# haoosz/FFR-Net

Hardware: AMD Instinct MI355X
Metric: face embeddings/sec (IR-SE50 + RecNet forward, 112x112 fp32) at batch 256 per GPU (higher is better)
Workload: dtype f32; 1 GPU; configs[2]: IR-SE50 + RecBlock (spatial+channel) forward, batch 256 per GPU, 112x112x3 fp32 -> f_new,f [512]; + all-gather of embeddings and pair cosine scores (112x96 of the BASELINE label cannot be embedded by the reference: BASELINE.md); batch_per_gpu=256, global_batch=256, parallelism=image-sharded x1, RCCL all-gather of embeddings

## Files before the change

### ffr-net_amd/csrc/conv.cpp

```cpp
#include "engine_internal.h"

namespace ffr_eng {

#ifdef FFR_TRACE
static int trace_igemm(ffr_handle* h, IgemmArgs& a, int tile, int nblocks, long long units, hipStream_t st) {
    unsigned long long* dbuf = nullptr;
    HIPCK(h, hipMalloc((void**)&dbuf, (size_t)nblocks * 8 * sizeof(unsigned long long)));
    a.trace = dbuf;
    HIPCK(h, launch_igemm(a, tile, nblocks, st));
    HIPCK(h, hipStreamSynchronize(st));
    std::vector<unsigned long long> t((size_t)nblocks * 8);
    HIPCK(h, hipMemcpy(t.data(), dbuf, t.size() * 8, hipMemcpyDeviceToHost));
    HIPCK(h, hipFree(dbuf));
    a.trace = nullptr;
    double acc[4] = {0, 0, 0, 0}, segs = 0, e1 = 0, e2 = 0, ghz = 0;
    unsigned long long r0 = ~0ull, r1 = 0, smax = 0;
    for (int b = 0; b < nblocks; ++b) {
        const unsigned long long* q = &t[(size_t)b * 8];
        for (int k = 0; k < 4; ++k) acc[k] += (double)q[k];
        segs += (double)q[4];
        ghz += (double)(q[0] + q[1] + q[2] + q[3]) / ((double)(q[6] - q[5]) * 10.0);
        e1 += (double)(q[7] >> 32); e2 += (double)(q[7] & 0xffffffffull);
        if (q[5] < r0) r0 = q[5];
        if (q[5] > smax) smax = q[5];
        if (q[6] > r1) r1 = q[6];
    }
    fprintf(stderr, "[igemm trace] tile %d blocks %d units %lld nkt %d segs/blk %.2f | per segment: setup %.0f prologue %.0f "
                    "loop %.0f (%.0f per K-tile) epilogue %.0f (first barrier at %.0f, C in LDS at %.0f) cyc | span %.1f us, starts within %.1f us, shader clock %.2f GHz\n",
            tile, nblocks, units, a.nkt, segs / nblocks, acc[0] / segs, acc[1] / segs, acc[2] / segs,
            acc[2] / ((double)units), acc[3] / segs, e1 / segs, e2 / segs, (double)(r1 - r0) / 100.0, (double)(smax - r0) / 100.0, ghz / nblocks);
    return FFR_OK;
}

static int trace_wino_mixed(ffr_handle* h, WinoMixedArgs& f, const ConvW& L, const ConvCall& c, hipStream_t st) {
    const int nbm = wino_mixed_blocks_launched(c.N, c.H, c.W, L.cout_pad, f.xcd_pairs);
    unsigned long long* dbuf = nullptr;
    HIPCK(h, hipMalloc((void**)&dbuf, (size_t)nbm * 12 * sizeof(unsigned long long)));
    HIPCK(h, hipMemsetAsync(dbuf, 0, (size_t)nbm * 12 * sizeof(unsigned long long), st));
    f.trace = dbuf;
    hipEvent_t e0, e1;
    HIPCK(h, hipEventCreate(&e0)); HIPCK(h, hipEventCreate(&e1));
    HIPCK(h, hipEventRecord(e0, st));
    HIPCK(h, launch_wino_fused_mixed(f, st));
    HIPCK(h, hipEventRecord(e1, st));
    HIPCK(h, hipStreamSynchronize(st));
    float ev_ms = 0.f;
    HIPCK(h, hipEventElapsedTime(&ev_ms, e0, e1));
    hipEventDestroy(e0); hipEventDestroy(e1);
    std::vector<unsigned long long> tr((size_t)nbm * 12);
    HIPCK(h, hipMemcpy(tr.data(), dbuf, tr.size() * 8, hipMemcpyDeviceToHost));
    HIPCK(h, hipFree(dbuf));
    double pro[4] = {0, 0, 0, 0}, loop[4] = {0, 0, 0, 0}, ep1[4] = {0, 0, 0, 0}, ep2[4] = {0, 0, 0, 0}, clk[4] = {0, 0, 0, 0};
    int cnt[4] = {0, 0, 0, 0};
    unsigned long long r_first = ~0ull, r_last = 0;
    struct Run { unsigned long long start, end; int tau; };
    std::map<unsigned long long, std::vector<Run>> per_cu;
    for (int b = 0; b < nbm; ++b) {
        const unsigned long long* q = &tr[(size_t)b * 12];
        if (!q[9]) continue;
        const int tau = (int)q[8];
        pro[tau] += (double)(q[1] - q[0]); loop[tau] += (double)(q[2] - q[1]); ep1[tau] += (double)(q[3] - q[2]); ep2[tau] += (double)(q[4] - q[3]);
        clk[tau] += (double)(q[4] - q[0]) / (double)(q[6] - q[5]) * 0.1;
        ++cnt[tau];
        if (q[5] < r_first) r_first = q[5];
        if (q[6] > r_last) r_last = q[6];
        per_cu[q[7]].push_back(Run{q[5], q[6], tau});
    }
    static const char* tname[4] = {"(4,4)", "(4,3)", "(3,4)", "(3,3)"};
    fprintf(stderr, "[wf trace] mixed %dx%d cin %d cout %d, %d images: hipEvent %.1f us, first block start to last block end %.1f us\n",
            c.H, c.W, L.cin_pad, L.cout_pad, c.N, ev_ms * 1e3, (double)(r_last - r_first) / 100.0);
    for (int tau = 0; tau < 4; ++tau) {
        if (!cnt[tau]) continue;
        const int S = wino_mixed_xp(tau) / 4;
        fprintf(stderr, "[wf trace]   type %s: %d blocks of %d slots | per block (wave 0): prologue %.0f loop %.0f (%.0f per K chunk, floor %d) "
                        "epilogue %.0f + %.0f = block %.0f cyc at %.2f GHz = %.1f us\n", tname[tau], cnt[tau], S, pro[tau] / cnt[tau], loop[tau] / cnt[tau],
                loop[tau] / cnt[tau] / f.nkc, S * 8 * 64, ep1[tau] / cnt[tau], ep2[tau] / cnt[tau],
                (pro[tau] + loop[tau] + ep1[tau] + ep2[tau]) / cnt[tau], clk[tau] / cnt[tau],
                (pro[tau] + loop[tau] + ep1[tau] + ep2[tau]) / cnt[tau] / (clk[tau] / cnt[tau]) * 1e-3);
    }
    std::map<std::string, int> hist;
    double busy = 0, gap = 0, tail = 0, lead = 0;
    for (auto& kv : per_cu) {
        auto& v = kv.second;
        std::sort(v.begin(), v.end(), [](const Run& x, const Run& y) { return x.start < y.start; });
        std::string key;
        for (size_t i = 0; i < v.size(); ++i) {
            key += tname[v[i].tau];
            busy += (double)(v[i].end - v[i].start);
            if (i) gap += (double)(v[i].start - v[i - 1].end);
        }
        lead += (double)(v.front().start - r_first);
        tail += (double)(r_last - v.back().end);
        ++hist[key];
    }
    const double ncu = (double)per_cu.size();
    fprintf(stderr, "[wf trace]   %d CUs ran blocks; per CU: busy %.1f us, idle before its first block %.1f, between blocks %.1f, after its last block %.1f us | sequences:",
            (int)per_cu.size(), busy / ncu / 100.0, lead / ncu / 100.0, gap / ncu / 100.0, tail / ncu / 100.0);
    for (auto& kv : hist) fprintf(stderr, "  %s x %d", kv.first.c_str(), kv.second);
    fprintf(stderr, "\n");
    return FFR_OK;
}

static int trace_wino_fused(ffr_handle* h, WinoFusedArgs& f, const ConvW& L, const ConvCall& c, const ConvPlan& p, hipStream_t st) {
    const int nb = wino_fused_blocks(f);
    unsigned long long* dbuf = nullptr;
    HIPCK(h, hipMalloc((void**)&dbuf, (size_t)nb * 40 * sizeof(unsigned long long)));
    HIPCK(h, hipMemsetAsync(dbuf, 0, (size_t)nb * 40 * sizeof(unsigned long long), st));
    f.trace = dbuf;
    HIPCK(h, launch_wino_fused(f, st));
    HIPCK(h, hipStreamSynchronize(st));
    std::vector<unsigned long long> tr((size_t)nb * 40);
    HIPCK(h, hipMemcpy(tr.data(), dbuf, tr.size() * 8, hipMemcpyDeviceToHost));
    HIPCK(h, hipFree(dbuf));
    double pro = 0, loop = 0, epi = 0, ep[5] = {0, 0, 0, 0, 0}; int cnt = 0;
    unsigned long long r0 = ~0ull, r1 = 0;
    for (int b = 0; b < nb; ++b) {
        const unsigned long long* q = &tr[(size_t)b * 40];
        if (!q[3]) continue;
        ep[0] += (double)(q[6] - q[2]); ep[1] += (double)(q[7] - q[6]); ep[2] += (double)(q[8] - q[7]);
        ep[3] += (double)(q[9] - q[8]); ep[4] += (double)(q[3] - q[9]);
        pro += (double)(q[1] - q[0]); loop += (double)(q[2] - q[1]); epi += (double)(q[3] - q[2]); ++cnt;
        if (q[4] > r1) r1 = q[4];
        if (q[4] < r0) r0 = q[4];
    }
    if (p.phased) {
        const int cpp = 4, nph = f.nkc / cpp;
        fprintf(stderr, "[wf trace] %dx%d cin %d cout %d (input transform in the kernel, %d-channel blocks%s): %d live blocks of %d | per block (wave 0): "
                        "prologue %.0f loop %.0f = %d phases x (transform %.0f + barrier %.0f + %d K chunks of %.0f) epilogue %.0f cyc | "
                        "block ends spread over %.1f us\n", c.H, c.W, L.cin_pad, L.cout_pad, p.half_n ? 32 : 64, "", cnt, nb,
                pro / cnt, loop / cnt, nph, ep[0] / cnt, ep[1] / cnt, cpp, (loop / cnt / nph - ep[0] / cnt - ep[1] / cnt) / cpp, epi / cnt,
                (double)(r1 - r0) / 100.0);
    }
    else
        fprintf(stderr, "[wf trace] %dx%d cin %d cout %d: %d live blocks of %d | per block (wave 0): prologue %.0f loop %.0f (%.0f per K chunk) "
                        "epilogue %.0f cyc (to LDS %.0f, transform+store %.0f, barrier+to LDS %.0f, transform+store %.0f, end %.0f) | block ends spread over %.1f us\n",
                c.H, c.W, L.cin_pad, L.cout_pad, cnt, nb, pro / cnt, loop / cnt, loop / cnt / f.nkc, epi / cnt, ep[0] / cnt, ep[1] / cnt,
                ep[2] / cnt, ep[3] / cnt, ep[4] / cnt, (double)(r1 - r0) / 100.0);
    return FFR_OK;
}
#endif

int run_gemm(ffr_handle* h, IgemmArgs& a, const ConvCall& c, double flops, double bytes, hipStream_t st, double fuse) {
    int tile, nblocks;
    int force = c.tile;
    if (force) {
        int fbm, fbn;
        igemm_tile_shape(force, &fbm, &fbn);
        if (a.cout_pad % fbn) return fail(h, FFR_ERR_ARG, "conv: forced tile %d (%d x %d) does not divide cout_pad %d", force, fbm, fbn, a.cout_pad);
    }
    plan_igemm(a.M, a.cout_pad, a.nkt, a.nbatch, force, h->opt.sk_minunits, &tile, &nblocks, &a.granule, a.w3 != nullptr);
    int bm, bn;
    igemm_tile_shape(tile, &bm, &bn);
    a.mtiles = (a.M + bm - 1) / bm;
    a.ntiles = a.cout_pad / bn;
    const long long units = (long long)a.nbatch * a.mtiles * a.ntiles * a.nkt;
    const bool cut = a.granule == 1 && ((units % nblocks) != 0 || ((units / nblocks) % a.nkt) != 0);
    if (cut && (size_t)nblocks * 2 * bm * bn > c.partial_cap) return fail(h, FFR_ERR_NOMEM, "stream-K workspace too small");
    a.partial = c.partial;
    a.tickets = c.tickets;
    if ((size_t)a.nbatch * a.mtiles * a.ntiles > c.tickets_cap) return fail(h, FFR_ERR_NOMEM, "stream-K ticket array too small");
#ifdef FFR_TRACE
    if (h->opt.igemm_trace) return trace_igemm(h, a, tile, nblocks, units, st);
#endif
    const double fexec = 2.0 * a.nbatch * (double)a.mtiles * bm * (double)a.cout_pad * a.KK;
    Scope s(h, st, FFR_KC_CONV_IGEMM, flops, bytes, fexec, fuse);
    HIPCK(h, launch_igemm(a, tile, nblocks, st));
    return FFR_OK;
}

static int conv_mixed(ffr_handle* h, const ConvW& L, const ConvCall& c, double flops, double bytes, hipStream_t st) {
    WinoMixedGeom g;
    wino_mixed_geom(c.H, c.W, &g);
    if (c.wino_stage == 0) {
        Scope s(h, st, FFR_KC_WINO, 0, 4.0 * ((double)c.N * c.H * c.W * L.cin + (double)wino_mixed_v_floats(g, c.N, L.cin_pad, nullptr)));
        HIPCK(h, launch_wino_in_mixed(c.x, c.winoV, c.N, c.H, c.W, c.in_pitch, L.cin_pad, st));
    }
    WinoMixedArgs f{};
    f.V[0] = c.winoV;
    for (int tau = 0; tau < 4; ++tau) f.U[tau] = L.wum[tau];
    f.bias = L.bias; f.slope = L.slope; f.resid = c.resid; f.out = c.out; f.tile_sums = c.tile_sums;
    f.N = c.N; f.H = c.H; f.W = c.W; f.nkc = L.cin_pad / 8;
    f.cout_pad = L.cout_pad; f.cout_store = c.cout_store; f.out_pitch = c.out_pitch; f.out_coff = c.out_coff;
    f.res_pitch = c.res_pitch; f.border_bias = L.border; f.flags = c.flags;
    f.xcd_pairs = 1;
    double fexec = 0.0, fuse = 0.0;
    for (int tau = 0; tau < 4; ++tau) {
        const int nr = tau >= 2 ? g.n3 : g.n4, nc = (tau & 1) ? g.n3 : g.n4;
        const double Tt = (double)c.N * nr * nc;
        fexec += 2.0 * wino_mixed_xp(tau) * std::ceil(Tt / 32.0) * 32.0 * L.cout_pad * L.cin_pad;
        fuse += 2.0 * wino_mixed_x(tau) * Tt * L.cout * L.cin;
    }
#ifdef FFR_TRACE
    if (h->opt.wf_trace) return trace_wino_mixed(h, f, L, c, st);
#endif
    Scope s(h, st, FFR_KC_WINO_FUSED, flops, bytes, fexec, fuse);
    HIPCK(h, launch_wino_fused_mixed(f, st));
    return FFR_OK;
}

static int conv_fused(ffr_handle* h, const ConvW& L, const ConvCall& c, const ConvPlan& p, double flops, double bytes, hipStream_t st) {
    const long long T = (long long)c.N * ((c.H + 3) / 4) * ((c.W + 3) / 4);
    if (!p.phased && c.wino_stage == 0) {
        Scope s(h, st, FFR_KC_WINO, 0, 4.0 * ((double)c.N * c.H * c.W * L.cin + 36.0 * T * L.cin_pad));
        HIPCK(h, launch_wino_in_chunked(c.x, c.winoV, c.N, c.H, c.W, c.in_pitch, L.cin_pad, L.pad_mode, st));
    }
    WinoFusedArgs f{};
    f.Vc = p.phased ? nullptr : c.winoV; f.x = c.x; f.in_pitch = c.in_pitch; f.pad_mode = L.pad_mode;
    f.x_bytes = p.phased ? (unsigned)(4.0 * c.N * c.H * c.W * c.in_pitch) : 0u;
    f.map_v = p.phased ? 2 : 1; f.half_n = p.half_n ? 1 : 0;
    f.Uc = L.wuc; f.bias = L.bias; f.slope = L.slope; f.resid = c.resid; f.out = c.out; f.tile_sums = c.tile_sums;
    f.N = c.N; f.H = c.H; f.W = c.W; f.nkc = L.cin_pad / 8;
    f.cout_pad = L.cout_pad; f.cout_store = c.cout_store; f.out_pitch = c.out_pitch; f.out_coff = c.out_coff;
    f.res_pitch = c.res_pitch; f.border_bias = L.border; f.flags = c.flags;
    const double fexec = 2.0 * 36.0 * (double)((T + 31) / 32 * 32) * (double)L.cout_pad * L.cin_pad;
#ifdef FFR_TRACE
    if (h->opt.wf_trace) return trace_wino_fused(h, f, L, c, p, st);
#endif
    Scope s(h, st, FFR_KC_WINO_FUSED, flops, bytes, fexec, flops / 4.0);
    HIPCK(h, launch_wino_fused(f, st));
    return FFR_OK;
}

static int igemm_batched(ffr_handle* h, const ConvCall& c, const float* A, long long a_bstride, int K_pad, const float* W,
                         long long w_bstride, int N_pad, float* out, int out_pitch, long long out_bstride, int M, int nbatch,
                         double flops, double bytes, double fuse, hipStream_t st) {
    IgemmArgs g{};
    g.x = A; g.w = W; g.bias = h->zero; g.slope = nullptr; g.resid = nullptr; g.out = out; g.zero = h->zero;
    g.N = 1; g.H = 1; g.W = M; g.Ho = 1; g.Wo = M;
    g.in_pitch = K_pad; g.cin_pad = K_pad; g.R = 1; g.S = 1; g.stride = 1; g.pad = 0; g.pad_mode = 0;
    g.M = M; g.KK = K_pad; g.nkt = K_pad / 32;
    g.cout_pad = N_pad; g.cout_store = N_pad; g.out_pitch = out_pitch; g.out_coff = 0; g.res_pitch = 0;
    g.border_bias = 0; g.flags = 0;
    g.nbatch = nbatch; g.x_bstride = a_bstride; g.w_bstride = w_bstride; g.out_bstride = out_bstride;
    return run_gemm(h, g, c, flops, bytes, st, fuse);
}

static int conv_unfused(ffr_handle* h, const ConvW& L, const ConvCall& c, long long M, double flops, double bytes, hipStream_t st) {
    const long long T = (long long)c.N * ((c.H + 3) / 4) * ((c.W + 3) / 4);
    if (c.wino_stage != 2) {
        Scope s(h, st, FFR_KC_WINO, 0, 4.0 * ((double)c.N * c.H * c.W * L.cin + 36.0 * T * L.cin_pad));
        HIPCK(h, launch_wino_in(c.x, c.winoV, c.N, c.H, c.W, c.in_pitch, L.cin_pad, L.pad_mode, st));
    }
    if (h->opt.gemm_stream) {
        int gtile = IGEMM_TILE_128x64, gblocks = 768;
        double best = 1e300;
        for (int tt = IGEMM_TILE_128x128; tt <= IGEMM_TILE_128x64; ++tt) {
            int bm, bn;
            igemm_tile_shape(tt, &bm, &bn);
            if (L.cout_pad % bn) continue;
            const long long tiles = 36LL * ((T + bm - 1) / bm) * (L.cout_pad / bn);
            const long long pmax = 256LL * igemm_resident_blocks(tt);
            const long long p = pmax > tiles ? tiles : pmax;
            const double rounds = (double)((tiles + p - 1) / p);
            const double share = (double)((p + 255) / 256);
            const double cost = rounds * bm * bn * share / (tt == IGEMM_TILE_128x128 ? 1.0 : 0.92);
            if (cost < best) { best = cost; gtile = tt; gblocks = (int)p; }
        }
        GemmStreamArgs g{};
        g.A = c.winoV; g.W = L.wu; g.C = c.winoM; g.M = (int)T; g.K = L.cin_pad; g.Npad = L.cout_pad; g.nbatch = 36;
        int bm, bn;
        igemm_tile_shape(gtile, &bm, &bn);
        const double fexec = 2.0 * 36.0 * (double)((T + bm - 1) / bm) * bm * (double)L.cout_pad * L.cin_pad;
        Scope s(h, st, FFR_KC_CONV_IGEMM, flops, bytes, fexec, flops / 4.0);
        HIPCK(h, launch_gemm_stream(g, gtile, gblocks, st));
    } else {
        RC(igemm_batched(h, c, c.winoV, T * L.cin_pad, L.cin_pad, L.wu, (long long)L.cout_pad * L.cin_pad, L.cout_pad, c.winoM, L.cout_pad,
                         T * L.cout_pad, (int)T, 36, flops, bytes, flops / 4.0, st));
    }
    if (c.wino_stage == 1) return FFR_OK;
    Scope s(h, st, FFR_KC_WINO, 0, 4.0 * (36.0 * T * L.cout_pad + (double)M * L.cout));
    HIPCK(h, launch_wino_out(c.winoM, L.bias, L.slope, c.resid, c.res_pitch, c.out, c.out_pitch, c.out_coff,
                             c.cout_store, L.cout_pad, c.N, c.H, c.W, L.border, c.flags, st, c.tile_sums));
    return FFR_OK;
}

int run_conv(ffr_handle* h, const ConvW& L, const ConvCall& c, hipStream_t st) {
    const int Ho = (c.H + 2 * L.pad - L.R) / L.stride + 1, Wo = (c.W + 2 * L.pad - L.S) / L.stride + 1;
    const long long M = (long long)c.N * Ho * Wo;
    if (M <= 0 || M > 0x7fffffffLL) return fail(h, FFR_ERR_ARG, "conv: bad M");
    if (L.pad_mode == 1 && (c.H < 2 || c.W < 2)) return fail(h, FFR_ERR_UNSUPPORTED, "reflect pad needs H,W >= 2");
    if (L.border && (c.H < 2 || c.W < 2)) return fail(h, FFR_ERR_UNSUPPORTED, "border-class bias needs H,W >= 2");
    const double flops = 2.0 * M * L.cout * (double)L.R * L.S * L.cin;
    const double bytes = 4.0 * ((double)c.N * c.H * c.W * L.cin + (double)M * L.cout + (double)L.cout * L.R * L.S * L.cin);
    const ConvPlan p = plan_conv(h, L, c);
    if (p.refused) return fail(h, FFR_ERR_STATE, "%s", p.refused);
    if (p.path == ConvPlan::Mixed) return conv_mixed(h, L, c, flops, bytes, st);
    if (p.path == ConvPlan::Unfused) return conv_unfused(h, L, c, M, flops, bytes, st);
    if (p.path == ConvPlan::Fused && !p.n_main) return conv_fused(h, L, c, p, flops, bytes, st);
    if (p.path == ConvPlan::Fused) {
        ConvCall c1 = c, c2 = c;
        c1.N = p.n_main; c1.force = p.half_n ? ConvForce::FusedHalf : ConvForce::Fused;
        c2.N = c.N - p.n_main; c2.force = ConvForce::Unfused;
        const size_t px = (size_t)p.n_main * c.H * c.W;
        c2.x = c.x + px * c.in_pitch;
        c2.out = c.out + px * c.out_pitch;
        if (c.resid) c2.resid = c.resid + px * c.res_pitch;
        if (c.tile_sums) c2.tile_sums = c.tile_sums + (size_t)p.n_main * ((c.H + 3) / 4) * ((c.W + 3) / 4) * L.cout_pad;
        if (p.side) {
            HIPCK(h, hipEventRecord(h->ev_fork, st));
            HIPCK(h, hipStreamWaitEvent(p.side, h->ev_fork, 0));
            RC(run_conv(h, L, c2, p.side));
            HIPCK(h, hipEventRecord(h->ev_join, p.side));
            RC(run_conv(h, L, c1, st));
            HIPCK(h, hipStreamWaitEvent(st, h->ev_join, 0));
            return FFR_OK;
        }
        RC(run_conv(h, L, c1, st));
        return run_conv(h, L, c2, st);
    }
    IgemmArgs a{};
    a.x = c.x; a.w = L.w; a.bias = L.bias; a.slope = L.slope; a.resid = c.resid; a.out = c.out; a.zero = h->zero;
    a.N = c.N; a.H = c.H; a.W = c.W; a.Ho = Ho; a.Wo = Wo;
    a.in_pitch = c.in_pitch; a.cin_pad = L.cin_pad; a.R = L.R; a.S = L.S; a.stride = L.stride; a.pad = L.pad; a.pad_mode = L.pad_mode;
    a.M = (int)M; a.KK = L.R * L.S * L.cin_pad; a.nkt = a.KK / 32; a.nbatch = 1;
    a.cout_pad = L.cout_pad; a.cout_store = c.cout_store; a.out_pitch = c.out_pitch; a.out_coff = c.out_coff;
    a.res_pitch = c.res_pitch; a.border_bias = L.border; a.flags = c.flags;
    if (L.w3 && h->opt.igemm_split) { a.w3 = L.w3; a.w3_pstride = (long long)L.cout_pad * a.KK; }
    return run_gemm(h, a, c, flops, bytes, st);
}

int gemm_rows(ffr_handle* h, const Work& w, const float* A, int a_pitch, int K_pad, const float* W, const float* bias,
              int N_pad, float* out, int out_pitch, long long rows, const float* resid, int res_pitch, int flags,
              hipStream_t st) {
    ConvW cw;
    cw.cin = K_pad; cw.cin_pad = K_pad; cw.cout = N_pad; cw.cout_pad = N_pad; cw.R = 1; cw.S = 1; cw.stride = 1; cw.pad = 0;
    cw.pad_mode = 0; cw.border = 0; cw.w = const_cast<float*>(W); cw.bias = bias ? const_cast<float*>(bias) : h->zero;
    cw.slope = nullptr; cw.wu = nullptr;
    ConvCall c = conv_call(w, ConvForce::Direct);
    c.x = A; c.N = 1; c.H = 1; c.W = (int)rows; c.in_pitch = a_pitch; c.resid = resid; c.res_pitch = res_pitch;
    c.out = out; c.out_pitch = out_pitch; c.out_coff = 0; c.cout_store = N_pad; c.flags = flags;
    return run_conv(h, cw, c, st);
}

int gemm_batched(ffr_handle* h, const Work& w, const float* A, long long a_bstride, int K_pad, const float* W,
                 long long w_bstride, int N_pad, float* out, int out_pitch, long long out_bstride, int M, int nbatch,
                 hipStream_t st) {
    const double fl = 2.0 * nbatch * (double)M * N_pad * K_pad;
    return igemm_batched(h, conv_call(w, ConvForce::Direct), A, a_bstride, K_pad, W, w_bstride, N_pad, out, out_pitch, out_bstride, M,
                         nbatch, fl, 4.0 * nbatch * ((double)M * K_pad + (double)N_pad * K_pad + (double)M * N_pad), fl, st);
}

}
```

### ffr-net_amd/csrc/engine.cpp

```cpp
#include "engine_internal.h"

using namespace ffr;
using namespace ffr_eng;

namespace ffr_eng {

std::string g_err = "";

int fail(ffr_handle* h, int code, const char* fmt, ...) {
    char buf[512];
    va_list ap;
    va_start(ap, fmt);
    vsnprintf(buf, sizeof buf, fmt, ap);
    va_end(ap);
    if (h) h->err = buf; else g_err = buf;
    return code;
}

struct PlanLayer { ConvW* L; std::string name; int net; };

std::vector<PlanLayer> plan_layers(const ffr_handle* hc) {
    ffr_handle* h = const_cast<ffr_handle*>(hc);
    std::vector<PlanLayer> v;
    if (h->enc_loaded)
        for (size_t i = 0; i < h->blocks.size(); ++i) {
            Block& b = h->blocks[i];
            const std::string p = "body." + std::to_string(i) + ".res_layer.";
            if (b.c1.wu) v.push_back({&b.c1, p + "1", 0});
            if (b.c2.wu) v.push_back({&b.c2, p + "3", 0});
        }
    if (h->rec_loaded)
        for (int i = 0; i < 15; ++i)
            if (rec_conv(h, i).wu) v.push_back({&rec_conv(h, i), std::string(REC_LAYERS[i].prefix) + ".conv2d", 1});
    return v;
}

void plan_changed(ffr_handle* h) { ++h->generation; h->mixed_ready_n = 0; }
}

extern "C" {

const char* ffr_version(void) { return "ffrnet-hip 0.1 (gfx950)"; }

const char* ffr_last_error(const ffr_handle* h) { return h ? h->err.c_str() : g_err.c_str(); }

int ffr_create(ffr_handle** out, int device) {
    if (!out) return fail(nullptr, FFR_ERR_ARG, "ffr_create: out is null");
    *out = nullptr;
    int count = 0;
    if (hipGetDeviceCount(&count) != hipSuccess || count <= 0)
        return fail(nullptr, FFR_ERR_HIP, "no HIP device available (this library has no CPU fallback)");
    if (device < 0 || device >= count) return fail(nullptr, FFR_ERR_ARG, "device %d out of range (%d devices)", device, count);
    DeviceScope scope(device);
    if (!scope.ok) return fail(nullptr, FFR_ERR_HIP, "hipSetDevice(%d) failed", device);
    hipDeviceProp_t prop;
    if (hipGetDeviceProperties(&prop, device) != hipSuccess) return fail(nullptr, FFR_ERR_HIP, "hipGetDeviceProperties failed");
    if (strncmp(prop.gcnArchName, "gfx950", 6) != 0)
        return fail(nullptr, FFR_ERR_UNSUPPORTED, "device %d is %s; this library is built for gfx950 (MI355X) only", device,
                    prop.gcnArchName);
    ffr_handle* h = new ffr_handle();
    h->device = device;
    h->num_cus = prop.multiProcessorCount > 0 ? prop.multiProcessorCount : 256;
    void* z = nullptr;
    if (hipMalloc(&z, 131072) != hipSuccess) { delete h; return fail(nullptr, FFR_ERR_NOMEM, "hipMalloc failed"); }
    hipMemset(z, 0, 131072);
    h->zero = (float*)z;
    hipError_t e = igemm_init();
    if (e == hipSuccess) e = gemm_stream_init();
    if (e == hipSuccess) e = wino_fused_init();
    if (e == hipSuccess) e = wino_mixed_init();
    if (e == hipSuccess) e = hipStreamCreateWithFlags(&h->side, hipStreamNonBlocking);
    if (e == hipSuccess) e = hipEventCreateWithFlags(&h->ev_fork, hipEventDisableTiming);
    if (e == hipSuccess) e = hipEventCreateWithFlags(&h->ev_join, hipEventDisableTiming);
    if (e != hipSuccess) {
        if (h->ev_fork) hipEventDestroy(h->ev_fork);
        if (h->ev_join) hipEventDestroy(h->ev_join);
        if (h->side) hipStreamDestroy(h->side);
        hipFree(z); delete h;
        return fail(nullptr, FFR_ERR_HIP, "ffr_create: %s", hipGetErrorString(e));
    }
    *out = h;
    return FFR_OK;
}

void ffr_destroy(ffr_handle* h) {
    if (!h) return;
    FFR_DEVICE_SCOPE(h);
    hipDeviceSynchronize();
    train_free(h);
    free_list(h->enc_allocs);
    free_list(h->rec_allocs);
    if (h->ev_fork) hipEventDestroy(h->ev_fork);
    if (h->ev_join) hipEventDestroy(h->ev_join);
    if (h->side) hipStreamDestroy(h->side);
    if (h->arena) hipFree(h->arena);
    if (h->tickets) hipFree(h->tickets);
    if (h->search_buf) hipFree(h->search_buf);
    if (h->align_buf) hipFree(h->align_buf);
    if (h->zero) hipFree(h->zero);
    for (auto& r : h->prof_log) { hipEventDestroy(r.e0); hipEventDestroy(r.e1); }
    for (auto e : h->ev_pool) hipEventDestroy(e);
    delete h;
}

int ffr_memory_stats(const ffr_handle* h, ffr_mem_stats* out) {
    if (!h || !out) return fail(nullptr, FFR_ERR_ARG, "ffr_memory_stats: null argument");
    out->encoder_weight_bytes = h->enc_weight_bytes;
    out->recnet_weight_bytes = h->rec_weight_bytes;
    out->mixed_tile_weight_bytes = h->mixed_weight_bytes;
    out->workspace_bytes = h->arena_bytes;
    out->encoder_load_seconds = h->enc_load_s;
    out->recnet_load_seconds = h->rec_load_s;
    out->mixed_tile_pack_seconds = h->mixed_pack_s;
    out->split_weight_bytes = h->split_weight_bytes;
    return FFR_OK;
}

size_t ffr_workspace_bytes(const ffr_handle* h, int N, int H, int W) {
    if (N <= 0 || H <= 0 || W <= 0) return 0;
    return layout(h ? h->opt : Options(), nullptr, N, H, W).total;
}

int ffr_reserve(ffr_handle* h, int N, int H, int W) {
    FFR_DEVICE_SCOPE(h); RC(check_fwd(h, false, false, N));
    Work w;
    return ensure_arena_encoder(h, N, H, W, &w);
}

static int encoder_forward(ffr_handle* h, const float* x, const U8In* u8, int N, int H, int W, float* featmap_nchw, float* f,
                           void* stream) {
    FFR_DEVICE_SCOPE(h); RC(check_fwd(h, true, false, N));
    if (u8 ? !u8->img : !x) return fail(h, FFR_ERR_ARG, u8 ? "img is null" : "x is null");
    if (H < 32 || W < 32 || (H & 15) || (W & 15)) return fail(h, FFR_ERR_ARG, "H and W must be multiples of 16, >= 32");
    if (f && (H != 112 || W != 112)) return fail(h, FFR_ERR_UNSUPPORTED, "f needs a 112x112 input (Linear(512*7*7,512))");
    hipStream_t st = (hipStream_t)stream;
    Work w;
    RC(ensure_arena_encoder(h, N, H, W, &w));
    RC(run_encoder(h, w, x, N, H, W, featmap_nchw ? w.trunk_bn : nullptr, f, st, u8));
    if (featmap_nchw) {
        Scope s(h, st, FFR_KC_LAYOUT, 0, 8.0 * N * (H / 16) * (W / 16) * 512);
        HIPCK(h, launch_nhwc_to_nchw(w.trunk_bn, 512, featmap_nchw, N, (H / 16) * (W / 16), 512, st));
    }
    return FFR_OK;
}

int ffr_encoder_forward(ffr_handle* h, const float* x, int N, int H, int W, float* featmap_nchw, float* f, void* stream) {
    return encoder_forward(h, x, nullptr, N, H, W, featmap_nchw, f, stream);
}

int ffr_encoder_forward_u8(ffr_handle* h, const uint8_t* img_hwc_rgb, const uint8_t* flip, int N, int H, int W,
                           float* featmap_nchw, float* f, void* stream) {
    const U8In u8{img_hwc_rgb, flip};
    return encoder_forward(h, nullptr, &u8, N, H, W, featmap_nchw, f, stream);
}

int ffr_recnet_forward(ffr_handle* h, const float* featmap_nchw, int N, float* f_new, float* feat_new_nchw, void* stream) {
    FFR_DEVICE_SCOPE(h); RC(check_fwd(h, false, true, N));
    if (!featmap_nchw) return fail(h, FFR_ERR_ARG, "featmap is null");
    hipStream_t st = (hipStream_t)stream;
    Work w;
    RC(ensure_arena(h, N, 112, 112, &w));
    {
        Scope s(h, st, FFR_KC_LAYOUT, 0, 8.0 * N * 49 * 512);
        HIPCK(h, launch_nchw_to_nhwc(featmap_nchw, w.X, 512, N, 49, 512, st));
    }
    RC(run_recnet(h, w, N, f_new, nullptr, st));
    if (feat_new_nchw) {
        Scope s(h, st, FFR_KC_LAYOUT, 0, 8.0 * N * 49 * 512);
        HIPCK(h, launch_nhwc_to_nchw(w.m512c, 512, feat_new_nchw, N, 49, 512, st));
    }
    return FFR_OK;
}

int ffr_embed(ffr_handle* h, const float* x, int N, float* f_new, float* f, void* stream) {
    FFR_DEVICE_SCOPE(h); RC(check_fwd(h, true, true, N));
    if (!x || !f_new) return fail(h, FFR_ERR_ARG, "x / f_new is null");
    hipStream_t st = (hipStream_t)stream;
    Work w;
    RC(ensure_arena_encoder(h, N, 112, 112, &w));
    RC(run_encoder(h, w, x, N, 112, 112, w.X, f, st));
    return run_recnet(h, w, N, f_new, nullptr, st);
}

int ffr_embed_u8(ffr_handle* h, const uint8_t* img_hwc_rgb, const uint8_t* flip, int N, float* f_new, float* f,
                 void* stream) {
    FFR_DEVICE_SCOPE(h); RC(check_fwd(h, true, true, N));
    if (!img_hwc_rgb || !f_new) return fail(h, FFR_ERR_ARG, "img / f_new is null");
    hipStream_t st = (hipStream_t)stream;
    Work w;
    RC(ensure_arena_encoder(h, N, 112, 112, &w));
    U8In u8{img_hwc_rgb, flip};
    RC(run_encoder(h, w, nullptr, N, 112, 112, w.X, f, st, &u8));
    return run_recnet(h, w, N, f_new, nullptr, st);
}

int ffr_cosine_scores(ffr_handle* h, const float* a, const float* b, int n, int dim, float* score, void* stream) {
    FFR_DEVICE_SCOPE(h); RC(check_fwd(h, false, false, n));
    if (!a || !b || !score || dim <= 0) return fail(h, FFR_ERR_ARG, "ffr_cosine_scores: bad arguments");
    hipStream_t st = (hipStream_t)stream;
    Scope s(h, st, FFR_KC_SCORE, 6.0 * n * dim, 8.0 * n * dim);
    HIPCK(h, launch_cosine(a, b, n, dim, score, st));
    return FFR_OK;
}

int ffr_lfw_fold_accuracy(ffr_handle* h, const float* score, const int32_t* label, int n, int n_folds, double* best_thr,
                          double* test_acc, void* stream) {
    FFR_DEVICE_SCOPE(h); RC(check_fwd(h, false, false, n));
    if (!score || !label || !best_thr || !test_acc || n_folds < 1 || n_folds > 32 || n < n_folds)
        return fail(h, FFR_ERR_ARG, "ffr_lfw_fold_accuracy: bad arguments");
    hipStream_t st = (hipStream_t)stream;
    Work w;
    RC(ensure_arena(h, 8, 112, 112, &w));
    Scope s(h, st, FFR_KC_SCORE, 400.0 * n, 8.0 * 400 * n);
    HIPCK(h, launch_fold_protocol(score, (const int*)label, n, n_folds, (int*)w.partial, best_thr, test_acc, st));
    return FFR_OK;
}

unsigned long long ffr_generation(const ffr_handle* h) { return h ? h->generation : 0; }

static bool misaligned16(const void* p) { return ((uintptr_t)p & 15) != 0; }

int ffr_row_norms(ffr_handle* h, const float* x, long long n, int dim, float* norms, void* stream) {
    FFR_DEVICE_SCOPE(h); RC(check_fwd(h, false, false, 1));
    if (dim != 512) return fail(h, FFR_ERR_UNSUPPORTED, "ffr_row_norms: dim must be 512, got %d", dim);
    if (!x || !norms || n < 1) return fail(h, FFR_ERR_ARG, "ffr_row_norms: bad arguments");
    hipStream_t st = (hipStream_t)stream;
    Scope s(h, st, FFR_KC_SCORE, 2.0 * n * dim, 4.0 * n * (dim + 1));
    HIPCK(h, launch_row_norms(x, n, norms, st));
    return FFR_OK;
}

int ffr_search_topk(ffr_handle* h, const float* query, int Q, const float* gallery, const float* gallery_norms, long long G,
                    int dim, int k, long long index_base, float* top_score, int64_t* top_index, void* stream) {
    FFR_DEVICE_SCOPE(h); RC(check_fwd(h, false, false, 1));
    if (dim != 512) return fail(h, FFR_ERR_UNSUPPORTED, "ffr_search_topk: dim must be 512, got %d", dim);
    if (!query || !top_score || !top_index || Q < 1 || k < 1 || k > 128 || G < 0 || (G > 0 && (!gallery || !gallery_norms)))
        return fail(h, FFR_ERR_ARG, "ffr_search_topk: bad arguments (Q >= 1, 1 <= k <= 128, G >= 0, non-null pointers)");
    if (misaligned16(query) || (G > 0 && misaligned16(gallery)))
        return fail(h, FFR_ERR_ARG, "ffr_search_topk: query and gallery rows must be 16-byte aligned");
    hipStream_t st = (hipStream_t)stream;
    if (G == 0) {
        Scope s(h, st, FFR_KC_SCORE, 0.0, 12.0 * Q * k);
        HIPCK(h, launch_topk_merge(nullptr, nullptr, 0, Q, k, top_score, top_index, st));
        return FFR_OK;
    }
    int T = 0, S = 0;
    long long chunk_rows = 0;
    search_plan(Q, G, h->num_cus, &T, &S, &chunk_rows);
    const size_t norm_bytes = ((size_t)Q * 4 + 255) & ~(size_t)255;
    const size_t list_s = S > 1 ? (((size_t)S * Q * k * 4 + 255) & ~(size_t)255) : 0;
    const size_t need = norm_bytes + list_s + (S > 1 ? (size_t)S * Q * k * 8 : 0);
    if (need > h->search_bytes) {
        if (h->search_buf) { hipDeviceSynchronize(); hipFree(h->search_buf); h->search_buf = nullptr; h->search_bytes = 0; }
        void* p = nullptr;
        if (hipMalloc(&p, need) != hipSuccess) return fail(h, FFR_ERR_NOMEM, "hipMalloc of %zu search bytes failed", need);
        h->search_buf = (char*)p;
        h->search_bytes = need;
        ++h->generation;
    }
    float* qnorm = (float*)h->search_buf;
    float* part_s = S > 1 ? (float*)(h->search_buf + norm_bytes) : top_score;
    int64_t* part_i = S > 1 ? (int64_t*)(h->search_buf + norm_bytes + list_s) : top_index;
    Scope s(h, st, FFR_KC_SCORE, 2.0 * Q * (double)G * dim, 4.0 * (double)G * (dim + 1) + 4.0 * Q * dim + 12.0 * Q * k);
    HIPCK(h, launch_row_norms(query, Q, qnorm, st));
    HIPCK(h, launch_search_topk(query, qnorm, Q, gallery, gallery_norms, G, k, index_base, T, S, chunk_rows, part_s, part_i,
                                st));
    if (S > 1) HIPCK(h, launch_topk_merge(part_s, part_i, S, Q, k, top_score, top_index, st));
// ... 108 lines not shown
    out->arith = v[i].L->direct ? FFR_ARITH_DIRECT : FFR_ARITH_WINOGRAD;
    out->sensitivity = v[i].L->sensitivity;
    return FFR_OK;
}

int ffr_layer_set_arith(ffr_handle* h, int i, int arith) {
    if (!h) return fail(nullptr, FFR_ERR_ARG, "null handle");
    if (arith != FFR_ARITH_DIRECT && arith != FFR_ARITH_WINOGRAD) return fail(h, FFR_ERR_ARG, "ffr_layer_set_arith: arith %d is neither 0 (direct) nor 1 (Winograd)", arith);
    const std::vector<PlanLayer> v = plan_layers(h);
    if (i < 0 || i >= (int)v.size()) return fail(h, FFR_ERR_ARG, "ffr_layer_set_arith: index %d outside [0, %d)", i, (int)v.size());
    const bool direct = arith == FFR_ARITH_DIRECT;
    if (v[i].L->direct != direct) { v[i].L->direct = direct; plan_changed(h); }
    return FFR_OK;
}

int ffr_calibrate(ffr_handle* h, const float* x, const float* featmap, int N, int H, int W, double tol, double* achieved,
                  void* stream) {
    if (!h) return fail(nullptr, FFR_ERR_ARG, "null handle");
    hipStream_t st = (hipStream_t)stream;
    {
        FFR_DEVICE_SCOPE(h);
        hipStreamCaptureStatus cs = hipStreamCaptureStatusNone;
        HIPCK(h, hipStreamIsCapturing(st, &cs));
        if (cs != hipStreamCaptureStatusNone) return fail(h, FFR_ERR_ARG, "ffr_calibrate: the stream is capturing (the call synchronises)");
    }
    if (!(tol > 0.0)) return fail(h, FFR_ERR_ARG, "ffr_calibrate: tol must be > 0 (got %g)", tol);
    if ((x != nullptr) == (featmap != nullptr)) return fail(h, FFR_ERR_ARG, "ffr_calibrate: pass images (x) or a featmap, exactly one of them");
    const bool enc = x != nullptr;
    FFR_DEVICE_SCOPE(h); RC(check_fwd(h, enc, !enc, N));
    if (enc && (H < 32 || W < 32 || (H & 15) || (W & 15))) return fail(h, FFR_ERR_ARG, "H and W must be multiples of 16, >= 32");
    if (!enc && (H != 7 || W != 7)) return fail(h, FFR_ERR_ARG, "ffr_calibrate: a featmap is [N,512,7,7] (H = W = 7)");
    const bool is112 = enc && H == 112 && W == 112;
    const bool rec = !enc || (h->rec_loaded && is112);
    const int P = enc ? (H / 16) * (W / 16) : 49;

    std::vector<ConvW*> cand;
    for (const PlanLayer& pl : plan_layers(h))
        if ((pl.net == 0 && enc) || (pl.net == 1 && rec)) cand.push_back(pl.L);
    const int L = (int)cand.size();
    struct Saved {
        ffr_handle* h; std::vector<std::pair<ConvW*, bool>> plan; bool prof; void* buf = nullptr; bool keep = false;
        ~Saved() {
            if (buf) { hipDeviceSynchronize(); hipFree(buf); }
            h->prof = prof;
            if (!keep) for (auto& p : plan) p.first->direct = p.second;
        }
    } sv{h, {}, h->prof};
    for (ConvW* c : cand) sv.plan.push_back({c, c->direct});
    h->prof = false;

    for (ConvW* c : cand) c->direct = false;
    h->mixed_ready_n = 0;
    Work w;
    if (enc) RC(ensure_arena_encoder(h, N, H, W, &w));
    else RC(ensure_arena(h, N, 112, 112, &w));

    const bool have[4] = {is112, enc, rec, rec};
    const size_t rows[4] = {(size_t)N, (size_t)N * P, (size_t)N, (size_t)N * 49};
    float* featmap_nhwc = rec ? w.X : w.trunk_bn;
    const int max_trials = 2 * L + 4;
    const size_t scratch = (size_t)absdiff_scratch_floats();
    size_t floats = scratch + (size_t)max_trials * 4 * 2 + 2 * (size_t)N * 512;
    size_t off_anchor[4];
    for (int t = 0; t < 4; ++t) { off_anchor[t] = floats; floats += have[t] ? rows[t] * 512 : 0; }
    HIPCK(h, hipMalloc(&sv.buf, floats * sizeof(float)));
    float* base = (float*)sv.buf;
    float* part = base;
    float* table = base + scratch;
    float* f_cur = table + (size_t)max_trials * 8;
    float* fnew_cur = f_cur + (size_t)N * 512;
    const float* cur[4] = {f_cur, featmap_nhwc, fnew_cur, w.m512c};
    float* anchor[4];
    for (int t = 0; t < 4; ++t) anchor[t] = base + off_anchor[t];
    HIPCK(h, hipMemsetAsync(table, 0, (size_t)max_trials * 8 * sizeof(float), st));

    auto forward = [&]() -> int {
        if (enc) {
            RC(run_encoder(h, w, x, N, H, W, featmap_nhwc, is112 ? f_cur : nullptr, st));
        } else {
            HIPCK(h, launch_nchw_to_nhwc(featmap, w.X, 512, N, 49, 512, st));
        }
        if (rec) RC(run_recnet(h, w, N, fnew_cur, nullptr, st));
        return FFR_OK;
    };
    auto compare = [&](int slot) -> int {
        for (int t = 0; t < 4; ++t)
            if (have[t]) HIPCK(h, launch_absdiff_max(cur[t], 512, anchor[t], 512, (int)rows[t], 512, part, table + ((size_t)slot * 4 + t) * 2, st));
        return FFR_OK;
    };
    std::vector<float> host((size_t)max_trials * 8);
    auto read = [&]() -> int {
        HIPCK(h, hipMemcpyAsync(host.data(), table, host.size() * sizeof(float), hipMemcpyDeviceToHost, st));
        HIPCK(h, hipStreamSynchronize(st));
        return FFR_OK;
    };
    auto rel = [&](int slot, int t) { const float* q = &host[((size_t)slot * 4 + t) * 2]; return q[1] > 0.f ? (double)q[0] / q[1] : (double)q[0]; };
    auto err = [&](int slot) { double e = 0.0; for (int t = 0; t < 4; ++t) if (have[t]) e = std::max(e, rel(slot, t)); return e; };
    auto set_plan = [&](const std::vector<char>& wino) { for (int k = 0; k < L; ++k) cand[k]->direct = !wino[k]; };

    set_plan(std::vector<char>(L, 0));
    RC(forward());
    for (int t = 0; t < 4; ++t)
        if (have[t]) HIPCK(h, hipMemcpyAsync(anchor[t], cur[t], rows[t] * 512 * sizeof(float), hipMemcpyDeviceToDevice, st));
    set_plan(std::vector<char>(L, 1));
    RC(forward()); RC(compare(0));
    for (int k = 0; k < L; ++k) {
        std::vector<char> one(L, 0);
        one[k] = 1;
        set_plan(one);
        RC(forward()); RC(compare(1 + k));
    }
    RC(read());
    const double half = 0.5 * tol;
    for (int k = 0; k < L; ++k) cand[k]->sensitivity = err(1 + k);
    std::vector<int> order(L);
    for (int k = 0; k < L; ++k) order[k] = k;
    std::stable_sort(order.begin(), order.end(), [&](int a, int b) { return cand[a]->sensitivity < cand[b]->sensitivity; });
    auto prefix_plan = [&](int p) { std::vector<char> v(L, 0); for (int i = 0; i < p; ++i) v[order[i]] = 1; return v; };

    std::vector<int> passing;
    if (err(0) <= half) passing.push_back(L);
    else if (L > 1) {
        for (int p = 1; p < L; ++p) { set_plan(prefix_plan(p)); RC(forward()); RC(compare(p)); }
        RC(read());
        int pmax = 0;
        while (pmax + 1 < L && err(pmax + 1) <= half) ++pmax;
        for (int p = pmax; p >= 1; --p) passing.push_back(p);
    }
    passing.push_back(0);

    for (int p : passing) {
        set_plan(prefix_plan(p));
        RC(forward()); RC(compare(0));
        RC(read());
        if (err(0) <= half || p == 0) break;
    }
    if (achieved) for (int t = 0; t < 4; ++t) achieved[t] = have[t] ? rel(0, t) : -1.0;
    sv.keep = true;
    bool changed = false;
    for (auto& pr : sv.plan) changed |= pr.first->direct != pr.second;
    if (changed) plan_changed(h);
    else h->mixed_ready_n = 0;
    return FFR_OK;
}

namespace {
struct OptEntry { const char* name; int ffr_eng::Options::*i; long long ffr_eng::Options::*l; long long lo, hi; };
const OptEntry OPTIONS[] = {
    {"wino", &Options::wino, nullptr, 0, 1}, {"wino_mincin", &Options::wino_mincin, nullptr, 0, 1 << 20},
    {"wino_fused", &Options::wino_fused, nullptr, 0, 1},
    {"wf_phased_maxk", &Options::wf_phased_maxk, nullptr, 0, 1 << 20}, {"wf_minblocks", nullptr, &Options::wf_minblocks, 0, 1LL << 40},
    {"se_maxtiles", &Options::se_maxtiles, nullptr, 0, 1 << 20}, {"wf_tailsplit", &Options::wf_tailsplit, nullptr, 0, 1},
    {"gemm_stream", &Options::gemm_stream, nullptr, 0, 1}, {"sk_minunits", &Options::sk_minunits, nullptr, 1, 1 << 20},
    {"combine_v", &Options::combine_v, nullptr, 0, 1}, {"wf_mixed", &Options::wf_mixed, nullptr, 0, 1},
    {"channel_rows", &Options::channel_rows, nullptr, 0, 4}, {"igemm_split", &Options::igemm_split, nullptr, 0, 1},
    {"wf_trace", &Options::wf_trace, nullptr, 0, 1}, {"igemm_trace", &Options::igemm_trace, nullptr, 0, 1},
};
const OptEntry* find_option(const char* name) {
    if (name) for (const OptEntry& e : OPTIONS) if (!strcmp(e.name, name)) return &e;
    return nullptr;
}
}

int ffr_set_option(ffr_handle* h, const char* name, long long value) {
    if (!h) return fail(nullptr, FFR_ERR_ARG, "null handle");
    const OptEntry* e = find_option(name);
    if (!e) return fail(h, FFR_ERR_ARG, "ffr_set_option: unknown option '%s'", name ? name : "(null)");
    if (value < e->lo || value > e->hi) return fail(h, FFR_ERR_ARG, "ffr_set_option: %s = %lld is outside [%lld, %lld]", name, value, e->lo, e->hi);
    if (e->i == &Options::channel_rows && value == 3) return fail(h, FFR_ERR_ARG, "ffr_set_option: channel_rows is 0 (auto), 1, 2 or 4");
#ifndef FFR_TRACE
    if ((e->i == &Options::wf_trace || e->i == &Options::igemm_trace) && value)
        return fail(h, FFR_ERR_UNSUPPORTED, "ffr_set_option: %s needs a -DFFR_TRACE build of the library (tools/trace_build.py)", name);
#endif
    const long long old = e->i ? (long long)(h->opt.*(e->i)) : h->opt.*(e->l);
    if (old != value) ++h->generation;
    if (e->i) h->opt.*(e->i) = (int)value; else h->opt.*(e->l) = value;
    return FFR_OK;
}

int ffr_get_option(const ffr_handle* h, const char* name, long long* value) {
    if (!h || !value) return fail(nullptr, FFR_ERR_ARG, "ffr_get_option: bad arguments");
    const OptEntry* e = find_option(name);
    if (!e) return fail(const_cast<ffr_handle*>(h), FFR_ERR_ARG, "ffr_get_option: unknown option '%s'", name ? name : "(null)");
    *value = e->i ? (long long)(h->opt.*(e->i)) : h->opt.*(e->l);
    return FFR_OK;
}

int ffr_probe_mfma_peak(ffr_handle* h, int iters, double* tflops, double* clock_ghz, void* stream) {
    FFR_DEVICE_SCOPE(h); RC(check_fwd(h, false, false, 1));
    if (iters <= 0 || !tflops) return fail(h, FFR_ERR_ARG, "ffr_probe_mfma_peak: bad arguments");
    hipStream_t st = (hipStream_t)stream;
    const int blocks = h->num_cus * 2;
    struct Res {
        unsigned long long* stamps = nullptr; float* sink = nullptr; hipEvent_t e0 = nullptr, e1 = nullptr;
        ~Res() { if (e0) hipEventDestroy(e0); if (e1) hipEventDestroy(e1); if (stamps) hipFree(stamps); if (sink) hipFree(sink); }
    } r;
    HIPCK(h, hipMalloc((void**)&r.stamps, (size_t)blocks * 4 * sizeof(unsigned long long)));
    HIPCK(h, hipMalloc((void**)&r.sink, (size_t)blocks * 256 * sizeof(float)));
    HIPCK(h, hipEventCreate(&r.e0)); HIPCK(h, hipEventCreate(&r.e1));
    for (int rep = 0; rep < 3; ++rep) HIPCK(h, launch_mfma_probe(iters, blocks, r.stamps, r.sink, st));
    HIPCK(h, hipEventRecord(r.e0, st));
    HIPCK(h, launch_mfma_probe(iters, blocks, r.stamps, r.sink, st));
    HIPCK(h, hipEventRecord(r.e1, st));
    HIPCK(h, hipEventSynchronize(r.e1));
    float ms = 0.f;
    HIPCK(h, hipEventElapsedTime(&ms, r.e0, r.e1));
    std::vector<unsigned long long> sv((size_t)blocks * 4);
    HIPCK(h, hipMemcpy(sv.data(), r.stamps, sv.size() * 8, hipMemcpyDeviceToHost));
    double ghz = 0;
    for (int b = 0; b < blocks; ++b) ghz += (double)(sv[b * 4 + 1] - sv[b * 4 + 0]) / ((double)(sv[b * 4 + 3] - sv[b * 4 + 2]) * 10.0);
    *tflops = (double)blocks * 4.0 * iters * 16.0 * 4096.0 / ((double)ms * 1e-3) / 1e12;
    if (clock_ghz) *clock_ghz = ghz / blocks;
    return FFR_OK;
}

int ffr_profile_enable(ffr_handle* h, int on) {
    if (!h) return fail(nullptr, FFR_ERR_ARG, "null handle");
    h->prof = on != 0;
    return FFR_OK;
}

int ffr_profile_read(ffr_handle* h, ffr_kclass_stat* out) {
    if (!h || !out) return fail(h, FFR_ERR_ARG, "ffr_profile_read: bad arguments");
    for (int i = 0; i < FFR_KC_COUNT; ++i) out[i] = ffr_kclass_stat{0, 0.0, 0.0, 0.0, 0.0, 0.0};
    for (auto& r : h->prof_log) {
        HIPCK(h, hipEventSynchronize(r.e1));
        float ms = 0.f;
        HIPCK(h, hipEventElapsedTime(&ms, r.e0, r.e1));
        out[r.kc].launches += 1;
        if (!r.side) {
            out[r.kc].ms += ms;
            out[r.kc].flops += r.flops;
            out[r.kc].bytes += r.bytes;
            out[r.kc].flops_executed += r.fexec;
            out[r.kc].flops_useful += r.fuse;
        }
        h->ev_pool.push_back(r.e0);
        h->ev_pool.push_back(r.e1);
    }
    h->prof_log.clear();
    return FFR_OK;
}

int ffr_op_conv(ffr_handle* h, const ffr_conv_desc* d, void* stream) {
    if (!d) return fail(h, FFR_ERR_ARG, "desc is null");
    FFR_DEVICE_SCOPE(h); RC(check_fwd(h, false, false, d->N));
    if (!d->x || !d->w || !d->bias || !d->out) return fail(h, FFR_ERR_ARG, "ffr_op_conv: null tensor");
    if (d->cin_pad % 32 || d->cout_pad % 64 || d->cin_pad <= 0) return fail(h, FFR_ERR_ARG, "ffr_op_conv: bad padding");
    Work w;
    RC(ensure_arena(h, d->N > 8 ? d->N : 8, 112, 112, &w));
    ConvW L;
    L.cin = L.cin_pad = d->cin_pad; L.cout = d->cout_store; L.cout_pad = d->cout_pad; L.R = d->R; L.S = d->S;
    L.stride = d->stride; L.pad = d->pad; L.pad_mode = d->pad_mode; L.border = d->border_bias;
    L.w = (float*)d->w; L.bias = (float*)d->bias; L.slope = (float*)d->slope;
    struct Planes { void* p = nullptr; ~Planes() { if (p) hipFree(p); } } planes;
    if (d->flags & 2) {
        if (!h->opt.igemm_split) return fail(h, FFR_ERR_STATE, "ffr_op_conv: flags bit1 asks for the split form, but option igemm_split is 0");
        const size_t nw = (size_t)d->cout_pad * d->R * d->S * d->cin_pad;
        HIPCK(h, hipMalloc(&planes.p, nw * 3 * sizeof(unsigned short)));
        HIPCK(h, launch_split_weights(d->w, (unsigned short*)planes.p, nw, (hipStream_t)stream));
        L.w3 = (unsigned short*)planes.p;
    }
    ConvCall c = conv_call(w);
    c.x = d->x; c.N = d->N; c.H = d->H; c.W = d->W; c.in_pitch = d->in_pitch; c.resid = d->resid; c.res_pitch = d->res_pitch;
    c.out = d->out; c.out_pitch = d->out_pitch; c.out_coff = d->out_coff; c.cout_store = d->cout_store; c.flags = d->flags & 1;
    c.tile = d->tile;
    const int rc = run_conv(h, L, c, (hipStream_t)stream);
    if (planes.p) hipStreamSynchronize((hipStream_t)stream);
    return rc;
}

int ffr_op_conv3x3(ffr_handle* h, const float* x, int N, int H, int W, int cin, const float* w_host,
                   const float* bias_host, const float* slope_host, int cout, int pad_mode, int use_wino,
                   const float* resid, float* out, void* stream) {
    FFR_DEVICE_SCOPE(h); RC(check_fwd(h, false, false, N));
    if (!x || !w_host || !bias_host || !out || cin % 32 || cout % 4 || cin <= 0 || cout <= 0)
        return fail(h, FFR_ERR_ARG, "ffr_op_conv3x3: bad arguments (cin %% 32, cout %% 4)");
    if (use_wino < 0 || use_wino > 4) return fail(h, FFR_ERR_ARG, "ffr_op_conv3x3: use_wino must be 0..4");
    hipStream_t st = (hipStream_t)stream;
    Work w;
    RC(ensure_arena(h, N > 8 ? N : 8, 112, 112, &w));
    std::vector<void*> own;
    BNFold ob;
    ob.s.assign(cout, 1.0);
    ob.t.assign(bias_host, bias_host + cout);
    ConvW L;
    int rc = pack_conv(h, own, w_host, cout, cin, 3, 3, nullptr, &ob, slope_host, 1, 1, pad_mode, &L);
    if (rc == FFR_OK && use_wino && !L.wu) rc = fail(h, FFR_ERR_UNSUPPORTED, "layer not eligible for the Winograd path (cin < FFR_WINO_MINCIN)");
    if (rc == FFR_OK && use_wino == 4) {
        if (!wino_mixed_eligible(h, L, N, H, W, cin, w.wino_cap, ConvForce::Mixed)) rc = fail(h, FFR_ERR_UNSUPPORTED, "layer / map not eligible for the mixed-tile path");
        else rc = ensure_mixed_weights(h, L, own, true);
    }
    if (rc == FFR_OK) {
        ConvCall c = conv_call(w, (ConvForce)use_wino);
        c.x = x; c.N = N; c.H = H; c.W = W; c.in_pitch = cin; c.resid = resid; c.res_pitch = cout;
        c.out = out; c.out_pitch = cout; c.out_coff = 0; c.cout_store = cout;
        rc = run_conv(h, L, c, st);
        if (rc == FFR_OK && use_wino && (size_t)36 * N * ((H + 3) / 4) * ((W + 3) / 4) * (L.cin_pad > L.cout_pad ? L.cin_pad : L.cout_pad) > w.wino_cap)
            rc = fail(h, FFR_ERR_NOMEM, "Winograd scratch too small for this test shape");
    }
    hipStreamSynchronize(st);
    free_list(own);
    return rc;
}

int ffr_encoder_trunk_nhwc(ffr_handle* h, const float* x, int N, int H, int W, int n_blocks, float* out, void* stream) {
    FFR_DEVICE_SCOPE(h); RC(check_fwd(h, true, false, N));
    if (!x || !out || n_blocks < 0 || n_blocks > (int)h->blocks.size()) return fail(h, FFR_ERR_ARG, "ffr_encoder_trunk_nhwc: bad arguments");
    if (H < 32 || W < 32 || (H & 15) || (W & 15)) return fail(h, FFR_ERR_ARG, "H and W must be multiples of 16, >= 32");
    hipStream_t st = (hipStream_t)stream;
    Work w;
    RC(ensure_arena_encoder(h, N, H, W, &w));
    float* t; int oh, ow, oc;
    RC(run_trunk(h, w, x, N, H, W, n_blocks, st, &t, &oh, &ow, &oc));
    HIPCK(h, hipMemcpyAsync(out, t, (size_t)N * oh * ow * oc * sizeof(float), hipMemcpyDeviceToDevice, st));
    return FFR_OK;
}

int ffr_recnet_debug(ffr_handle* h, const float* featmap_nchw, int N, float* ss_space, float* M_space, float* feat_space,
                     float* feat_channel_raw, float* feat_channel, float* ss_channel0, float* M_channel0, void* stream) {
    FFR_DEVICE_SCOPE(h); RC(check_fwd(h, false, true, N));
    if (!featmap_nchw) return fail(h, FFR_ERR_ARG, "featmap is null");
    hipStream_t st = (hipStream_t)stream;
    Work w;
    RC(ensure_arena(h, N, 112, 112, &w));
    HIPCK(h, launch_nchw_to_nhwc(featmap_nchw, w.X, 512, N, 49, 512, st));
    RecDebug d{ss_space, M_space, feat_space, feat_channel_raw, feat_channel, ss_channel0, M_channel0};
    return run_recnet(h, w, N, nullptr, &d, st);
}

}
```

### ffr-net_amd/csrc/engine_internal.h

```cpp
#pragma once
#include <hip/hip_runtime.h>

#include <algorithm>
#include <chrono>
#include <cmath>
#include <cstdarg>
#include <cstdio>
#include <cstdlib>
#include <cstring>
#include <initializer_list>
#include <map>
#include <string>
#include <vector>

#include "../../include/ffrnet.h"
#include "../../include/ffrnet_train.h"
#include "ffr_kernels.h"

namespace ffr_eng {

using namespace ffr;

struct TrainState;

struct ConvW {
    int cin = 0, cin_pad = 0, cout = 0, cout_pad = 0, R = 1, S = 1, stride = 1, pad = 0, pad_mode = 0, border = 0;
    float* w = nullptr;
    float* bias = nullptr;
    float* slope = nullptr;
    float* wu = nullptr;
    float* wum[4] = {nullptr, nullptr, nullptr, nullptr};
    bool wum_gave_up = false;
    unsigned short* w3 = nullptr;
    float* wuc = nullptr;
    bool direct = false;
    double sensitivity = -1.0;
};

struct Block {
    int cin = 0, depth = 0, stride = 1;
    bool has_sc = false;
    ConvW c1, c2, sc;
    float* fc1 = nullptr;
    float* fc2 = nullptr;
};

struct Options {
    int wino = 1;
    int wino_mincin = 64;
    int wino_fused = 1;
    int wf_phased_maxk = 128;
    long long wf_minblocks = 200;
    int se_maxtiles = 256;
    int wf_tailsplit = 1;
    int gemm_stream = 1;
    int sk_minunits = 18;
    int wf_mixed = 1;
    int channel_rows = 0;
    int igemm_split = 1;
    int combine_v = 1;
    int wf_trace = 0, igemm_trace = 0;
};

struct ProfRec {
    hipEvent_t e0, e1;
    int kc;
    double flops, bytes, fexec, fuse;
    bool side;
};

}

struct ffr_handle {
    int device = 0;
    int num_cus = 256;
    hipStream_t side = nullptr;
    hipEvent_t ev_fork = nullptr, ev_join = nullptr;
    std::string err;
    float* zero = nullptr;
    std::vector<void*> enc_allocs, rec_allocs;
    bool enc_loaded = false, rec_loaded = false;
    size_t enc_weight_bytes = 0, rec_weight_bytes = 0;
    size_t mixed_weight_bytes = 0;
    double enc_load_s = 0.0, rec_load_s = 0.0, mixed_pack_s = 0.0;
    size_t split_weight_bytes = 0;
    bool mixed_gave_up_logged = false, split_gave_up_logged = false;
    int mixed_ready_n = 0, mixed_ready_h = 0, mixed_ready_w = 0;
    float *stem_w = nullptr, *stem_b = nullptr, *stem_s = nullptr;
    std::vector<ffr_eng::Block> blocks;
    float *bn_s = nullptr, *bn_t = nullptr;
    ffr_eng::ConvW fc;
    ffr_eng::ConvW sp[9], fm[3], mg[3];
    ffr::ChannelPathWeights cw{};
    char* arena = nullptr;
    size_t arena_bytes = 0;
    int* tickets = nullptr;
    size_t tickets_cap = 0;
    ffr_eng::Options opt;
    bool prof = false;
    std::vector<ffr_eng::ProfRec> prof_log;
    std::vector<hipEvent_t> ev_pool;
    ffr_eng::TrainState* train = nullptr;
    std::vector<ffr_wgrad_launch> wgrad_log;
    char* search_buf = nullptr;
    size_t search_bytes = 0;
    char* align_buf = nullptr;
    size_t align_bytes = 0;
    unsigned long long generation = 1;
};

namespace ffr_eng {

int fail(ffr_handle* h, int code, const char* fmt, ...);

#define HIPCK(h, expr)                                                                          \
    do {                                                                                        \
        hipError_t _e = (expr);                                                                 \
        if (_e != hipSuccess)                                                                   \
            return fail(h, FFR_ERR_HIP, "%s failed: %s (%s:%d)", #expr, hipGetErrorString(_e), __FILE__, __LINE__); \
    } while (0)

#define RC(expr)                  \
    do {                          \
        int _rc = (expr);         \
        if (_rc != FFR_OK) return _rc; \
    } while (0)

inline int round_up(int v, int m) { return (v + m - 1) / m * m; }

struct DeviceScope {
    int prev = -1;
    bool switched = false, ok = true;
    explicit DeviceScope(int dev) {
        if (dev < 0) return;
        if (hipGetDevice(&prev) != hipSuccess) prev = -1;
        if (prev != dev) { ok = hipSetDevice(dev) == hipSuccess; switched = ok && prev >= 0; }
    }
    ~DeviceScope() { if (switched) hipSetDevice(prev); }
};
#define FFR_DEVICE_SCOPE(h) ffr_eng::DeviceScope _dev_scope((h) ? (h)->device : -1)

struct Scope {
    ffr_handle* h;
    hipStream_t st;
    ProfRec r;
    bool on;
    Scope(ffr_handle* h_, hipStream_t st_, int kc, double flops, double bytes, double fexec = -1.0, double fuse = -1.0)
        : h(h_), st(st_), on(h_->prof) {
        if (!on) return;
        auto get = [&]() {
            hipEvent_t e;
            if (!h->ev_pool.empty()) { e = h->ev_pool.back(); h->ev_pool.pop_back(); }
            else hipEventCreate(&e);
            return e;
        };
        r.e0 = get(); r.e1 = get(); r.kc = kc; r.flops = flops; r.bytes = bytes; r.fexec = fexec < 0 ? flops : fexec; r.fuse = fuse < 0 ? flops : fuse;
        r.side = h->side && st == h->side;
        hipEventRecord(r.e0, st);
    }
    ~Scope() {
        if (!on) return;
        hipEventRecord(r.e1, st);
        h->prof_log.push_back(r);
    }
};

struct SD {
    std::map<std::string, const ffr_tensor_desc*> m;
    ffr_handle* h;
    int rc = FFR_OK;
    const float* get(const std::string& name, std::initializer_list<int64_t> shape) {
        auto it = m.find(name);
        if (it == m.end()) { rc = fail(h, FFR_ERR_KEY, "state_dict entry '%s' is missing", name.c_str()); return nullptr; }
        const ffr_tensor_desc* d = it->second;
        bool ok = d->data && d->ndim == (int)shape.size();
        int i = 0;
        for (int64_t s : shape) { if (ok && d->shape[i] != s) ok = false; ++i; }
        if (!ok) { rc = fail(h, FFR_ERR_KEY, "state_dict entry '%s' has an unexpected shape", name.c_str()); return nullptr; }
        return d->data;
    }
};

struct BNFold { std::vector<double> s, t; };
bool bn_fold(SD& sd, const std::string& p, int C, BNFold& o);
int upload(ffr_handle* h, std::vector<void*>& owner, const std::vector<float>& v, float** out);
int pack_conv(ffr_handle* h, std::vector<void*>& owner, const float* W, int cout, int cin, int R, int S,
              const BNFold* in_bn, const BNFold* out_bn, const float* slope, int stride, int pad, int pad_mode, ConvW* L);
void free_list(std::vector<void*>& v);
int ensure_mixed_weights(ffr_handle* h, ConvW& L, std::vector<void*>& owner, bool strict);
int prepare_mixed_weights(ffr_handle* h, int N, int H, int W, size_t wino_cap);
struct RecLayer { const char* prefix; int cin, cout; };
extern const RecLayer REC_LAYERS[15];
inline ConvW& rec_conv(ffr_handle* h, int i) { return i < 9 ? h->sp[i] : i < 12 ? h->fm[i - 9] : h->mg[i - 12]; }

enum class ConvForce { Auto = -1, Direct = 0, Fused = 1, Unfused = 2, FusedHalf = 3, Mixed = 4 };

struct ConvCall {
    const float* x; int N, H, W, in_pitch;
    const float* resid; int res_pitch;
    float* out; int out_pitch, out_coff, cout_store;
    int flags; int tile;
    float* partial; size_t partial_cap;
    int* tickets; size_t tickets_cap;
    float* winoV; float* winoM; size_t wino_cap;
    ConvForce force = ConvForce::Auto;
    int wino_stage = 0;
    bool v_mixed = false;
    bool v_chunked = false;
    float* tile_sums = nullptr;
};

struct ConvPlan {
    enum Path { Direct, Mixed, Fused, Unfused } path = Direct;
    bool half_n = false;
    bool phased = false;
    int n_main = 0;
    hipStream_t side = nullptr;
    bool takes_v = false;
    const char* refused = nullptr;
};

inline bool layer_wino(const ffr_handle* h, const ConvW& L) { return h->opt.wino != 0 && !L.direct; }
ConvForce wino_fused_form(const ffr_handle* h, int cin_pad, int cout_pad, long long T, double x_bytes, ConvForce ask);
bool wino_mixed_eligible(const ffr_handle* h, const ConvW& L, int N, int H, int W, int in_pitch, size_t wino_cap, ConvForce force);
ConvPlan plan_conv(const ffr_handle* h, const ConvW& L, const ConvCall& c);
void plan_igemm(long long M, int cout_pad, int nkt, int nbatch, int force_tile, int min_units, int* tile, int* nblocks, int* granule,
                bool split = false);
int run_gemm(ffr_handle* h, IgemmArgs& a, const ConvCall& c, double flops, double bytes, hipStream_t st, double fuse = -1.0);
int run_conv(ffr_handle* h, const ConvW& L, const ConvCall& c, hipStream_t st);

struct Arena {
    char* base; size_t off = 0, cap;
    Arena(char* b, size_t c) : base(b), cap(c) {}
    float* take(size_t floats) {
        size_t bytes = (floats * 4 + 255) & ~(size_t)255;
        float* p = base ? (float*)(base + off) : nullptr;
        off += bytes;
        return p;
    }
};

struct Work {
    float *bufA, *bufB, *t1, *res, *sc, *scale, *se_part, *trunk_bn;
    float* partial; size_t partial_cap;
    int* tickets; size_t tickets_cap;
    float *winoV, *winoM; size_t wino_cap;
    float *X, *bufS, *bufF, *bufM, *s256a, *s256b, *s256c, *ms, *m512a, *m512b, *m512c, *dbg;
    size_t total;
};

Work layout(const Options& opt, char* base, int N, int H, int W);
inline ConvCall conv_call(const Work& w, ConvForce force = ConvForce::Auto) {
    ConvCall c{};
    c.partial = w.partial; c.partial_cap = w.partial_cap; c.tickets = w.tickets; c.tickets_cap = w.tickets_cap;
    c.winoV = w.winoV; c.winoM = w.winoM; c.wino_cap = w.wino_cap; c.force = force;
    return c;
}
int ensure_arena(ffr_handle* h, int N, int H, int W, Work* w);
int ensure_arena_encoder(ffr_handle* h, int N, int H, int W, Work* w);
struct U8In { const unsigned char* img; const unsigned char* flip; const unsigned char* img2 = nullptr; };
int run_trunk(ffr_handle* h, const Work& w, const float* x_nchw, int N, int H, int W, int n_blocks, hipStream_t st,
              float** out_ptr, int* oh, int* ow, int* oc, const U8In* u8 = nullptr, const float* x2 = nullptr, int n_split = 0);
int run_encoder(ffr_handle* h, const Work& w, const float* x, int N, int H, int W, float* featmap_nhwc, float* f,
                hipStream_t st, const U8In* u8 = nullptr, const float* x2 = nullptr, int n_split = 0);
struct RecDebug { float *ss_space, *M_space, *feat_space, *feat_channel_raw, *feat_channel, *ss_channel0, *M_channel0; };
int conv_rec(ffr_handle* h, const Work& w, const ConvW& L, const float* x, int in_pitch, const float* resid,
             int res_pitch, float* out, int out_pitch, int out_coff, int flags, int N, hipStream_t st);
int run_recnet(ffr_handle* h, const Work& w, int N, float* f_new, const RecDebug* dbg, hipStream_t st);
int check_fwd(ffr_handle* h, bool need_enc, bool need_rec, int N);
int gemm_rows(ffr_handle* h, const Work& w, const float* A, int a_pitch, int K_pad, const float* W, const float* bias,
              int N_pad, float* out, int out_pitch, long long rows, const float* resid, int res_pitch, int flags,
              hipStream_t st);
int gemm_batched(ffr_handle* h, const Work& w, const float* A, long long a_bstride, int K_pad, const float* W,
                 long long w_bstride, int N_pad, float* out, int out_pitch, long long out_bstride, int M, int nbatch,
                 hipStream_t st);
void train_free(ffr_handle* h);

}
```

### ffr-net_amd/csrc/ffr_kernels.h

```cpp
#pragma once
#include <hip/hip_runtime.h>
#include <stdint.h>

#ifdef FFR_TRACE
#define FFR_TRACE_ON(p) ((p) != nullptr)
#else
#define FFR_TRACE_ON(p) false
#endif

namespace ffr {

struct IgemmArgs {
    const float* x;
    const float* w;
    const float* bias;
    const float* slope;
    const float* resid;
    float* out;
    const float* zero;
    float* partial;
    int* tickets;
    unsigned long long* trace;
    int N, H, W, Ho, Wo, in_pitch, cin_pad, R, S, stride, pad, pad_mode;
    int M, KK, nkt, granule;
    int nbatch;
    long long x_bstride, w_bstride, out_bstride;
    int cout_pad, cout_store, out_pitch, out_coff, res_pitch;
    int border_bias, flags;
    int mtiles, ntiles;
    const unsigned short* w3;
    long long w3_pstride;
};
enum { IGEMM_TILE_128x128 = 1, IGEMM_TILE_128x64 = 2, IGEMM_TILE_64x64 = 3, IGEMM_TILE_256x64 = 4,
       IGEMM_NTILES = 4 };
void igemm_tile_shape(int tile, int* bm, int* bn);
hipError_t igemm_init();
int igemm_resident_blocks(int tile, bool split = false);
hipError_t launch_split_weights(const float* w, unsigned short* planes, size_t n, hipStream_t stream);
hipError_t launch_igemm(const IgemmArgs& a, int tile, int nblocks, hipStream_t stream);

struct GemmStreamArgs {
    const float* A; const float* W; float* C;
    int M, K, Npad, nbatch;
    int mtiles, ntiles;
};
hipError_t gemm_stream_init();
hipError_t launch_gemm_stream(GemmStreamArgs a, int tile, int nblocks, hipStream_t stream);

hipError_t launch_wino_in(const float* x, float* V, int N, int H, int W, int pitch, int cin_pad, int pad_mode,
                          hipStream_t stream);
hipError_t launch_wino_weights(const float* W, float* U, int out_pad, int in_pad, hipStream_t stream, int chunked = 0);
hipError_t launch_wino_dout(const float* dy, float* dM, int N, int H, int W, int Cp, hipStream_t stream);
hipError_t launch_wino_dweights(const float* dU, float* grad, int out_pad, int in_pad, int accumulate, hipStream_t stream);
bool wino_out_in_supported(int H, int W, int C);
hipError_t launch_wino_out_in(const float* M, const float* bias, const float* slope, float* V, int N, int H, int W, int C,
                              int border_bias, hipStream_t stream);
hipError_t launch_wino_out(const float* M, const float* bias, const float* slope, const float* resid, int res_pitch,
                           float* out, int out_pitch, int out_coff, int cout_store, int cout_pad, int N, int H, int W,
                           int border_bias, int flags, hipStream_t stream, float* tile_sums = nullptr);

hipError_t launch_wino_in_chunked(const float* x, float* Vc, int N, int H, int W, int pitch, int cin_pad, int pad_mode,
                                  hipStream_t stream);
struct WinoFusedArgs {
    const float* Vc; const float* Uc;
    const float* x;
    unsigned x_bytes;
    int in_pitch, pad_mode;
    const float* bias; const float* slope; const float* resid; float* out; float* tile_sums;
    int N, H, W, nkc;
    int cout_pad, cout_store, out_pitch, out_coff, res_pitch, border_bias, flags;
    int half_n;
    int map_v;
    int th, tw, mbn, nbn;
    long long T;
    unsigned long long* trace;
};
bool combine_in_c_supported(int H, int W, int C);
hipError_t launch_combine_in_c(const float* res, const float* scale, const float* sh, float* out, float* Vc, int N, int H,
                               int W, int C, hipStream_t stream);
int wino_fused_blocks(const WinoFusedArgs& a);
hipError_t wino_fused_init();
hipError_t launch_wino_fused(WinoFusedArgs a, hipStream_t stream);
inline size_t wino_chunked_floats(long long T, int cin_pad) { return (size_t)((T + 31) / 32) * 32 * 36 * cin_pad; }

struct WinoMixedGeom { int n4, o4[2], n3, o3[2]; };
struct WinoInMixedArgs {
    const float* x; float* V[4];
    int N, H, W, pitch, nkc;
    WinoMixedGeom g;
    int goff[4];
    long long T[4];
};
struct WinoMixedArgs {
    const float* V[4];
    const float* U[4];
    const float* bias; const float* slope; const float* resid; float* out; float* tile_sums;
    int N, H, W, nkc;
    int cout_pad, cout_store, out_pitch, out_coff, res_pitch, border_bias, flags;
    WinoMixedGeom g;
    int xcd_pairs;
    int mbn[4], boff[4], nbn, tpi_off[4], tpi_total;
    long long T[4];
    unsigned long long* trace;
};
bool wino_mixed_geom(int H, int W, WinoMixedGeom* g);
int wino_mixed_x(int tau);
int wino_mixed_xp(int tau);
size_t wino_mixed_v_floats(const WinoMixedGeom& g, int N, int cin_pad, size_t off[4]);
int wino_mixed_blocks(int N, int H, int W, int cout_pad);
size_t wino_mixed_u_floats(int tau, int cout_pad, int cin_pad);
int wino_mixed_blocks_launched(int N, int H, int W, int cout_pad, int xcd_pairs);
hipError_t launch_wino_weights_mixed(const float* w, float* um, int cout_pad, int cin_pad, int tau, hipStream_t stream);
hipError_t wino_mixed_init();
hipError_t launch_wino_in_mixed(const float* x, float* V, int N, int H, int W, int pitch, int cin_pad, hipStream_t stream);
hipError_t launch_wino_fused_mixed(WinoMixedArgs a, hipStream_t stream);
hipError_t launch_combine_in_mixed(const float* res, const float* scale, const float* sh, float* out, float* V, int N, int H, int W,
                                   int C, hipStream_t stream);

hipError_t launch_mfma_probe(int iters, int blocks, unsigned long long* stamps, float* sink, hipStream_t stream);

hipError_t launch_stem(const float* x_nchw, const unsigned char* xu8, const unsigned char* flip, const float* w27x64,
                       const float* bias, const float* slope, float* out, int N, int H, int W, hipStream_t stream,
                       const float* x2 = nullptr, int n_split = 0, const unsigned char* xu8b = nullptr);
int se_slices(int N, int HW);
hipError_t launch_se(const float* res, int N, int HW, int C, const float* fc1, const float* fc2,
                     float* scale, float* part, hipStream_t stream);
hipError_t launch_se_fc(const float* part, int N, int S, int HW, int C, const float* fc1, const float* fc2, float* scale,
                        hipStream_t stream);
hipError_t launch_combine(const float* res, const float* scale, const float* sc, const float* x,
                          float* out, int N, int Ho, int Wo, int C, int stride, hipStream_t stream);
hipError_t launch_affine(const float* x, const float* s, const float* t, float* y, int M, int C,
                         hipStream_t stream);
hipError_t launch_head_finish(const float* partial, int splits, int N, int C, const float* bias,
                              float* f, hipStream_t stream);
hipError_t launch_nhwc_to_nchw(const float* in, int in_pitch, float* out, int N, int P, int C,
                               hipStream_t stream);
hipError_t launch_nchw_to_nhwc(const float* in, float* out, int out_pitch, int N, int P, int C,
                               hipStream_t stream);
hipError_t launch_copy_slice(const float* in, float* out, int M, int C, int pitch, int coff,
                             hipStream_t stream);
hipError_t launch_cosine(const float* a, const float* b, int n, int dim, float* score,
                         hipStream_t stream);
int absdiff_scratch_floats();
hipError_t launch_absdiff_max(const float* a, int a_pitch, const float* b, int b_pitch, int rows, int cols, float* part,
                              float* out, hipStream_t stream);

hipError_t launch_row_norms(const float* x, long long n, float* norms, hipStream_t stream);
long long search_max_chunk_rows();
void search_plan(int Q, long long G, int num_cus, int* ntiles, int* nchunks, long long* chunk_rows);
hipError_t launch_search_topk(const float* query, const float* qnorm, int Q, const float* gallery, const float* gnorm,
                              long long G, int k, long long index_base, int ntiles, int nchunks, long long chunk_rows,
                              float* out_s, int64_t* out_i, hipStream_t stream);
hipError_t launch_topk_merge(const float* score, const int64_t* index, int S, int Q, int k, float* out_s, int64_t* out_i,
                             hipStream_t stream);

hipError_t launch_align_tfm(const float* landmarks, const float* tmpl, int N, int K, const int* frame_index, int F, double* A,
                            uint8_t* valid, hipStream_t stream);
hipError_t launch_align_warp(const uint8_t* frames, int F, int H, int W, int pitch, const int* frame_index, const double* A,
                             const uint8_t* valid, int N, int oh, int ow, uint8_t* crop, hipStream_t stream);

hipError_t launch_fold_protocol(const float* score, const int* label, int n, int nf, int* scratch, double* best_thr,
                                double* test_acc, hipStream_t stream);

hipError_t launch_selfsim_space(const float* X, float* bufS, int pitchS, float* ss_out, int N,
                                hipStream_t stream);
struct ChannelPathWeights {
    const float* w1a;
    const float* w1b;
    const float* b1;
    const float* a1;
    const float* A2;
    const float* d2;
    const float* a4;
    const float* A3;
    const float* d3;
    const float* a7;
    const float* w8;
    const float* b8;
    const float* w8a;
    const float* b8a;
};
hipError_t launch_channel_path(const float* X, const ChannelPathWeights& w, float* bufF, int pitchF, int N, hipStream_t stream,
                               float* dbg_ss, float* dbg_M, int num_cus, int row_blocks ,
                               unsigned long long* trace = nullptr , int* row_blocks_used = nullptr);
hipError_t launch_space_apply(const float* X, const float* ms, int ms_pitch, float* out, int out_pitch,
                              int out_coff, int N, hipStream_t stream);
hipError_t launch_avgpool49(const float* feat, float* f_new, int N, int C, hipStream_t stream);

}
```

### ffr-net_amd/csrc/igemm.hip

```cpp
#include "ffr_kernels.h"

#include <utility>

namespace ffr {

typedef float f32x16 __attribute__((ext_vector_type(16)));
typedef float f32x4 __attribute__((ext_vector_type(4)));
typedef unsigned u32x4 __attribute__((ext_vector_type(4)));
typedef __bf16 bf16x8 __attribute__((ext_vector_type(8)));

#define LDS_PTR(p) ((__attribute__((address_space(3))) void*)(p))
#define GLB_PTR(p) ((const __attribute__((address_space(1))) void*)(p))

__device__ __forceinline__ unsigned cvt_pk_bf16(float lo, float hi) {
    unsigned r;
    asm("v_cvt_pk_bf16_f32 %0, %1, %2" : "=v"(r) : "v"(lo), "v"(hi));
    return r;
}

template <int BM, int BN, int WARPS_M, int WARPS_N, int PAD_MODE, bool SPLIT = false>
__global__ __launch_bounds__(256) void k_igemm(const IgemmArgs a) {
    constexpr int WM = BM / WARPS_M, WN = BN / WARPS_N;
    constexpr int TM = WM / 32, TN = WN / 32;
    constexpr int A_PT = BM / 32;
    constexpr int B_PT = SPLIT ? 3 * (BN / 64) : BN / 32;
    constexpr int STAGE_FLOATS = SPLIT ? BM * 32 + BN * 48 : (BM + BN) * 32;
    static_assert(WARPS_M * WARPS_N == 4, "4 waves");
    extern __shared__ __attribute__((aligned(16))) float smem[];
    constexpr int MAIN_FLOATS = (2 * STAGE_FLOATS > BM * (BN + 4)) ? 2 * STAGE_FLOATS : BM * (BN + 4);
    int* s_cls = reinterpret_cast<int*>(smem + MAIN_FLOATS);
    float* s_bias = smem + MAIN_FLOATS + BM + 4;

    const int wave = __builtin_amdgcn_readfirstlane(threadIdx.x >> 6);
    const int wm = wave / WARPS_N, wn = wave % WARPS_N;
    const int HoWo = a.Ho * a.Wo;

    const long long U = (long long)a.nbatch * a.mtiles * a.ntiles * a.nkt;
    const long long G = U / a.granule;
    long long u = (long long)blockIdx.x * G / gridDim.x * a.granule;
    const long long uend = (long long)(blockIdx.x + 1) * G / gridDim.x * a.granule;
    unsigned long long tr_acc[6] = {0, 0, 0, 0, 0, 0}, tr_seg = 0, tr_t = 0, tr_rt0 = 0;
    if (FFR_TRACE_ON(a.trace)) tr_rt0 = __builtin_amdgcn_s_memrealtime();
    while (u < uend) {
    const int tile_id = (int)(u / a.nkt);
    const int kb = (int)(u - (long long)tile_id * a.nkt);
    const int nk = (uend - u < (long long)(a.nkt - kb)) ? (int)(uend - u) : a.nkt - kb;
    u += nk;
    const int tpb = a.mtiles * a.ntiles;
    const int batch = tile_id / tpb;
    const int tile_b = tile_id - batch * tpb;
    const int nt = tile_b % a.ntiles, mt = tile_b / a.ntiles;
    const float* const xb = a.x + (long long)batch * a.x_bstride;
    const float* const wb = a.w + (long long)batch * a.w_bstride;
    float* const ob = a.out + (long long)batch * a.out_bstride;
    const int m0 = mt * BM, n0 = nt * BN;
    __syncthreads();
    __builtin_amdgcn_s_setprio(2);
    int tid = threadIdx.x;
    asm volatile("" : "+v"(tid));
    if (FFR_TRACE_ON(a.trace)) { tr_t = __builtin_amdgcn_s_memtime(); ++tr_seg; }
    const int lane = tid & 63;

    const int srow = tid >> 3;
    const int lch = (tid & 7) ^ ((srow >> 1) & 7);
    int a_pix[A_PT], a_h0[A_PT], a_w0[A_PT];
#pragma unroll
    for (int i = 0; i < A_PT; ++i) {
        int m = m0 + srow + 32 * i;
        if (m >= a.M) m = 0;
        if (a.H == 1 && a.N == 1) {
            a_pix[i] = 0;
            a_h0[i] = -a.pad;
            a_w0[i] = m * a.stride - a.pad;
        } else {
            const int n = m / HoWo;
            const int rem = m - n * HoWo;
            const int ho = rem / a.Wo;
            const int wo = rem - ho * a.Wo;
            a_pix[i] = n * a.H * a.W;
            a_h0[i] = ho * a.stride - a.pad;
            a_w0[i] = wo * a.stride - a.pad;
        }
    }
    if (a.border_bias && tid < BM) {
        int m = m0 + tid;
        if (m >= a.M) m = 0;
        const int n = m / HoWo;
        const int rem = m - n * HoWo;
        const int ho = rem / a.Wo;
        const int wo = rem - ho * a.Wo;
        const int h0 = ho * a.stride - a.pad, w0 = wo * a.stride - a.pad;
        const int rc = (h0 < 0) ? 0 : ((h0 + a.R - 1 >= a.H) ? 2 : 1);
        const int cc = (w0 < 0) ? 0 : ((w0 + a.S - 1 >= a.W) ? 2 : 1);
        s_cls[tid] = rc * 3 + cc;
    }
    if (a.border_bias) {
        for (int idx = tid; idx < 9 * BN; idx += 256) s_bias[idx] = a.bias[(idx / BN) * a.cout_pad + n0 + (idx % BN)];
    }

    const int kbase0 = kb * 32;
    int tap = kbase0 / a.cin_pad;
    int c0 = kbase0 - tap * a.cin_pad;
    int tr = tap / a.S, ts = tap - tr * a.S;

    const float* a_ptr[A_PT];
    const float* b_ptr[B_PT];
#pragma unroll
    for (int i = 0; i < B_PT; ++i) {
        if constexpr (SPLIT) {
            const int brow = tid >> 2, bch = (tid & 3) ^ ((brow >> 2) & 3);
            const int plane = i / (BN / 64), piece = i % (BN / 64);
            b_ptr[i] = reinterpret_cast<const float*>(a.w3 + (size_t)plane * a.w3_pstride + (size_t)(n0 + brow + 64 * piece) * a.KK + kbase0 + bch * 8);
        } else {
            b_ptr[i] = wb + (size_t)(n0 + srow + 32 * i) * a.KK + kbase0 + lch * 4;
        }
    }

    auto set_tap = [&]() {
#pragma unroll
        for (int i = 0; i < A_PT; ++i) {
            int hi = a_h0[i] + tr, wi = a_w0[i] + ts;
            bool ok = true;
            if (PAD_MODE == 1) {
                hi = hi < 0 ? -hi : (hi >= a.H ? 2 * a.H - 2 - hi : hi);
                wi = wi < 0 ? -wi : (wi >= a.W ? 2 * a.W - 2 - wi : wi);
            } else {
                ok = ((unsigned)hi < (unsigned)a.H) && ((unsigned)wi < (unsigned)a.W);
            }
            const float* src = xb + (size_t)(a_pix[i] + hi * a.W + wi) * a.in_pitch;
            a_ptr[i] = (ok ? src : a.zero) + c0 + lch * 4;
        }
    };
    set_tap();

    auto dma_piece = [&](int buf, int d) {
        float* sA = smem + buf * STAGE_FLOATS;
        if (d < A_PT) {
            __builtin_amdgcn_global_load_lds(GLB_PTR(a_ptr[d]), LDS_PTR(sA + (32 * d + 8 * wave) * 32), 16, 0, 0);
            a_ptr[d] += 32;
        } else {
            const int i = d - A_PT;
            if constexpr (SPLIT) {
                __builtin_amdgcn_global_load_lds(GLB_PTR(b_ptr[i]), LDS_PTR(sA + BM * 32 + (i / (BN / 64)) * BN * 16 + (64 * (i % (BN / 64)) + 16 * wave) * 16), 16, 0, 0);
                b_ptr[i] += 16;
            } else {
                __builtin_amdgcn_global_load_lds(GLB_PTR(b_ptr[i]), LDS_PTR(sA + (BM + 32 * i + 8 * wave) * 32), 16, 0, 0);
                b_ptr[i] += 32;
            }
        }
    };
    auto advance_tile = [&]() {
        c0 += 32;
        if (c0 == a.cin_pad) {
            c0 = 0;
            if (++ts == a.S) { ts = 0; ++tr; }
            set_tap();
        }
    };

    f32x16 acc[TM][TN];
#pragma unroll
    for (int i = 0; i < TM; ++i)
#pragma unroll
        for (int j = 0; j < TN; ++j)
#pragma unroll
            for (int r = 0; r < 16; ++r) acc[i][j][r] = 0.f;

    const int frow = lane & 31;
    const int fh = lane >> 5;
    const int fswz = (lane >> 1) & 7;
    int pc[4];
// ... 411 lines not shown
```

### ffr-net_amd/csrc/pack.cpp

```cpp
#include "engine_internal.h"

using namespace ffr_eng;

namespace ffr_eng {

const double BN_EPS = 1e-5;


bool bn_fold(SD& sd, const std::string& p, int C, BNFold& o) {
    const float* g = sd.get(p + ".weight", {C});
    const float* b = sd.get(p + ".bias", {C});
    const float* mu = sd.get(p + ".running_mean", {C});
    const float* var = sd.get(p + ".running_var", {C});
    if (!g || !b || !mu || !var) return false;
    o.s.resize(C); o.t.resize(C);
    for (int c = 0; c < C; ++c) {
        o.s[c] = (double)g[c] / std::sqrt((double)var[c] + BN_EPS);
        o.t[c] = (double)b[c] - (double)mu[c] * o.s[c];
    }
    return true;
}

int upload(ffr_handle* h, std::vector<void*>& owner, const std::vector<float>& v, float** out) {
    void* p = nullptr;
    if (hipMalloc(&p, v.size() * sizeof(float)) != hipSuccess)
        return fail(h, FFR_ERR_NOMEM, "hipMalloc of %zu weight bytes failed", v.size() * sizeof(float));
    owner.push_back(p);
    if (h && &owner == &h->enc_allocs) h->enc_weight_bytes += v.size() * sizeof(float);
    if (h && &owner == &h->rec_allocs) h->rec_weight_bytes += v.size() * sizeof(float);
    HIPCK(h, hipMemcpy(p, v.data(), v.size() * sizeof(float), hipMemcpyHostToDevice));
    *out = (float*)p;
    return FFR_OK;
}

static double round_bf16(double d) {
    if (d == 0.0 || !std::isfinite(d)) return d;
    if (std::fabs(d) >= 1.2e-38) {
        unsigned long long u;
        memcpy(&u, &d, 8);
        u += 0x00000fffffffffffull + ((u >> 45) & 1);
        u &= ~((1ull << 45) - 1);
        memcpy(&d, &u, 8);
        return d;
    }
    int e;
    std::frexp(d, &e);
    int q = e - 8;
    if (q < -133) q = -133;
    return std::nearbyint(std::ldexp(d, -q)) * std::ldexp(1.0, q);
}

int upload_split(ffr_handle* h, std::vector<void*>& owner, const std::vector<double>& wd, unsigned short** out) {
    *out = nullptr;
    const size_t n = wd.size();
    std::vector<unsigned short> pl(3 * n);
    for (size_t i = 0; i < n; ++i) {
        double r = wd[i];
        for (int p = 0; p < 3; ++p) {
            const double b = round_bf16(r);
            const float bf = (float)b;
            unsigned u;
            memcpy(&u, &bf, 4);
            pl[(size_t)p * n + i] = (unsigned short)(u >> 16);
            r -= b;
        }
    }
    void* p = nullptr;
    const size_t bytes = pl.size() * sizeof(unsigned short);
    hipError_t e = hipMalloc(&p, bytes);
    if (e == hipSuccess) e = hipMemcpy(p, pl.data(), bytes, hipMemcpyHostToDevice);
    if (e != hipSuccess) {
        if (p) hipFree(p);
        (void)hipGetLastError();
        if (!h->split_gave_up_logged) {
            h->split_gave_up_logged = true;
            fprintf(stderr, "ffrnet: no room for the split-operand weight planes (%zu bytes: %s); the layers concerned keep the fp32 kernel\n",
                    bytes, hipGetErrorString(e));
        }
        return FFR_OK;
    }
    owner.push_back(p);
    if (&owner == &h->enc_allocs) { h->enc_weight_bytes += bytes; h->split_weight_bytes += bytes; }
    if (&owner == &h->rec_allocs) h->rec_weight_bytes += bytes;
    *out = (unsigned short*)p;
    return FFR_OK;
}

int pack_conv(ffr_handle* h, std::vector<void*>& owner, const float* W, int cout, int cin, int R, int S,
              const BNFold* in_bn, const BNFold* out_bn, const float* slope, int stride, int pad, int pad_mode,
              ConvW* L) {
    L->cin = cin; L->cout = cout; L->R = R; L->S = S; L->stride = stride; L->pad = pad; L->pad_mode = pad_mode;
    L->cin_pad = round_up(cin, 32);
    L->cout_pad = round_up(cout, 64);
    L->border = in_bn ? 1 : 0;
    const int KK = R * S * L->cin_pad;
    std::vector<float> wp((size_t)L->cout_pad * KK, 0.f);
    const int wino_min_cin = h->opt.wino_mincin;
    const bool wino = R == 3 && S == 3 && stride == 1 && pad == 1 && L->cin_pad >= wino_min_cin && wino_min_cin > 0;
    std::vector<double> wd;
    if (!wino) wd.assign(wp.size(), 0.0);
    const int ncls = L->border ? 9 : 1;
    std::vector<float> bias((size_t)ncls * L->cout_pad, 0.f);
    std::vector<double> tap(R * S);
    for (int co = 0; co < cout; ++co) {
        const double g = out_bn ? out_bn->s[co] : 1.0;
        const double b = out_bn ? out_bn->t[co] : 0.0;
        for (int r = 0; r < R; ++r)
            for (int s = 0; s < S; ++s) {
                double tsum = 0.0;
                for (int ci = 0; ci < cin; ++ci) {
                    const double wv = W[(((size_t)co * cin + ci) * R + r) * S + s];
                    const double si = in_bn ? in_bn->s[ci] : 1.0;
                    wp[(size_t)co * KK + (size_t)(r * S + s) * L->cin_pad + ci] = (float)(wv * si * g);
                    if (!wino) wd[(size_t)co * KK + (size_t)(r * S + s) * L->cin_pad + ci] = wv * si * g;
                    if (in_bn) tsum += wv * in_bn->t[ci];
                }
                tap[r * S + s] = tsum;
            }
        if (L->border) {
            for (int rc = 0; rc < 3; ++rc)
                for (int cc = 0; cc < 3; ++cc) {
                    double acc = 0.0;
                    for (int r = 0; r < R; ++r) {
                        if ((rc == 0 && r == 0) || (rc == 2 && r == R - 1)) continue;
                        for (int s = 0; s < S; ++s) {
                            if ((cc == 0 && s == 0) || (cc == 2 && s == S - 1)) continue;
                            acc += tap[r * S + s];
                        }
                    }
                    bias[(size_t)(rc * 3 + cc) * L->cout_pad + co] = (float)(g * acc + b);
                }
        } else {
            bias[co] = (float)b;
        }
    }
    RC(upload(h, owner, wp, &L->w));
    RC(upload(h, owner, bias, &L->bias));
    L->w3 = nullptr;
    if (!wino) RC(upload_split(h, owner, wd, &L->w3));
    L->wu = nullptr;
    L->wuc = nullptr;
    for (int tau = 0; tau < 4; ++tau) L->wum[tau] = nullptr;
    L->direct = false;
    L->sensitivity = -1.0;
    if (wino) {
        static const double G[6][3] = {{0.25, 0, 0}, {-1.0 / 6, -1.0 / 6, -1.0 / 6}, {-1.0 / 6, 1.0 / 6, -1.0 / 6},
                                       {1.0 / 24, 1.0 / 12, 1.0 / 6}, {1.0 / 24, -1.0 / 12, 1.0 / 6}, {0, 0, 1}};
        std::vector<float> wu((size_t)36 * L->cout_pad * L->cin_pad, 0.f);
        for (int co = 0; co < cout; ++co) {
            const double g = out_bn ? out_bn->s[co] : 1.0;
            for (int ci = 0; ci < cin; ++ci) {
                const float* gk = W + ((size_t)co * cin + ci) * 9;
                const double sc = (in_bn ? in_bn->s[ci] : 1.0) * g;
                double tmp[6][3];
                for (int i = 0; i < 6; ++i)
                    for (int c = 0; c < 3; ++c) tmp[i][c] = G[i][0] * gk[0 * 3 + c] + G[i][1] * gk[1 * 3 + c] + G[i][2] * gk[2 * 3 + c];
                for (int i = 0; i < 6; ++i)
                    for (int j = 0; j < 6; ++j) {
                        const double u = tmp[i][0] * G[j][0] + tmp[i][1] * G[j][1] + tmp[i][2] * G[j][2];
                        wu[((size_t)(i * 6 + j) * L->cout_pad + co) * L->cin_pad + ci] = (float)(u * sc);
                    }
            }
        }
        RC(upload(h, owner, wu, &L->wu));
        const int nkc = L->cin_pad / 8, nbn = L->cout_pad / 64;
        std::vector<float> wuc(wu.size());
        for (int nb = 0; nb < nbn; ++nb)
            for (int kc = 0; kc < nkc; ++kc)
                for (int xi = 0; xi < 36; ++xi)
                    for (int nl = 0; nl < 64; ++nl)
                        for (int hf = 0; hf < 2; ++hf) {
                            const int piece = (nl >> 5) * 64 + hf * 32 + (nl & 31);
                            float* dst = &wuc[((((size_t)nb * nkc + kc) * 36 + xi) * 128 + piece) * 4];
                            const float* src = &wu[((size_t)xi * L->cout_pad + nb * 64 + nl) * L->cin_pad + kc * 8 + 4 * hf];
                            for (int e = 0; e < 4; ++e) dst[e] = src[e];
                        }
        RC(upload(h, owner, wuc, &L->wuc));
    }
    L->slope = nullptr;
    if (slope) {
        std::vector<float> sl(L->cout_pad, 0.f);
        for (int co = 0; co < cout; ++co) sl[co] = slope[co];
        RC(upload(h, owner, sl, &L->slope));
    }
    return FFR_OK;
}

void free_list(std::vector<void*>& v) {
    for (void* p : v) hipFree(p);
    v.clear();
}

const int STAGE_CH[4][2] = {{64, 64}, {64, 128}, {128, 256}, {256, 512}};
const int UNITS[3][4] = {{3, 4, 14, 3}, {3, 13, 30, 3}, {3, 8, 36, 3}};

static bool block_table(int n_blocks, std::vector<int>& cin, std::vector<int>& depth, std::vector<int>& stride) {
    for (auto& units : UNITS) {
        if (units[0] + units[1] + units[2] + units[3] != n_blocks) continue;
        for (int s = 0; s < 4; ++s)
            for (int u = 0; u < units[s]; ++u) {
                cin.push_back(u == 0 ? STAGE_CH[s][0] : STAGE_CH[s][1]);
                depth.push_back(STAGE_CH[s][1]);
                stride.push_back(u == 0 ? 2 : 1);
            }
        return true;
    }
    return false;
}

const RecLayer REC_LAYERS[15] = {
    {"Conv4Space.0", 561, 256}, {"Conv4Space.1.conv1", 256, 256}, {"Conv4Space.1.conv2", 256, 256}, {"Conv4Space.2", 256, 128},
    {"Conv4Space.3.conv1", 128, 128}, {"Conv4Space.3.conv2", 128, 128}, {"Conv4Space.4", 128, 49}, {"Conv4Space.5.conv1", 49, 49},
    {"Conv4Space.5.conv2", 49, 49}, {"ChannelFlipMerge.0", 1024, 512}, {"ChannelFlipMerge.1.conv1", 512, 512},
    {"ChannelFlipMerge.1.conv2", 512, 512}, {"Conv4Merge.0", 1536, 512}, {"Conv4Merge.1.conv1", 512, 512}, {"Conv4Merge.1.conv2", 512, 512}};

int ensure_mixed_weights(ffr_handle* h, ConvW& L, std::vector<void*>& owner, bool strict) {
    if (L.wum[1]) return FFR_OK;
    if (L.wum_gave_up && !strict) return FFR_OK;
    if (!L.wuc || !L.w) return fail(h, FFR_ERR_STATE, "mixed-tile weights asked for a layer without Winograd weights");
    float* um[4] = {L.wuc, nullptr, nullptr, nullptr};
    const auto t0 = std::chrono::steady_clock::now();
    size_t total = 0;
    for (int tau = 1; tau < 4; ++tau) {
        void* p = nullptr;
        const size_t bytes = wino_mixed_u_floats(tau, L.cout_pad, L.cin_pad) * sizeof(float);
        hipError_t e = hipMalloc(&p, bytes);
        if (e == hipSuccess) {
            um[tau] = (float*)p;
            e = launch_wino_weights_mixed(L.w, um[tau], L.cout_pad, L.cin_pad, tau, nullptr);
        }
        if (e != hipSuccess) {
            hipDeviceSynchronize();
            for (int k = 1; k <= tau; ++k) if (um[k]) hipFree(um[k]);
            (void)hipGetLastError();
            if (strict) return fail(h, e == hipErrorOutOfMemory ? FFR_ERR_NOMEM : FFR_ERR_HIP, "mixed-tile weights (%zu bytes): %s", bytes, hipGetErrorString(e));
            L.wum_gave_up = true;
            if (!h->mixed_gave_up_logged) {
                h->mixed_gave_up_logged = true;
                fprintf(stderr, "ffrnet: no room for the exact-tiling weight sets (%zu bytes: %s); the layers concerned stay on padded F(4x4) tiles\n",
                        bytes, hipGetErrorString(e));
            }
            return FFR_OK;
        }
        total += bytes;
    }
    HIPCK(h, hipDeviceSynchronize());
    for (int tau = 1; tau < 4; ++tau) owner.push_back(um[tau]);
    if (&owner == &h->enc_allocs) { h->mixed_weight_bytes += total; h->enc_weight_bytes += total; }
    h->mixed_pack_s += std::chrono::duration<double>(std::chrono::steady_clock::now() - t0).count();
    for (int tau = 0; tau < 4; ++tau) L.wum[tau] = um[tau];
    return FFR_OK;
}

int prepare_mixed_weights(ffr_handle* h, int N, int H, int W, size_t wino_cap) {
    if (!h->enc_loaded || !h->opt.wf_mixed || !h->opt.wino || !h->opt.wino_fused) return FFR_OK;
    if (h->mixed_ready_n >= N && h->mixed_ready_h == H && h->mixed_ready_w == W) return FFR_OK;
    int ch = H, cw = W;
    for (Block& b : h->blocks) {
        if (wino_mixed_eligible(h, b.c1, N, ch, cw, b.cin, wino_cap, ConvForce::Auto)) RC(ensure_mixed_weights(h, b.c1, h->enc_allocs, false));
        if (b.stride == 1 && wino_mixed_eligible(h, b.c2, N, ch, cw, b.depth, wino_cap, ConvForce::Auto)) RC(ensure_mixed_weights(h, b.c2, h->enc_allocs, false));
        ch /= b.stride; cw /= b.stride;
    }
    h->mixed_ready_n = N; h->mixed_ready_h = H; h->mixed_ready_w = W;
    return FFR_OK;
}

}

extern "C" {

int ffr_load_encoder(ffr_handle* h, const ffr_tensor_desc* t, int n) {
    if (!h || !t || n <= 0) return fail(h, FFR_ERR_ARG, "ffr_load_encoder: bad arguments");
    FFR_DEVICE_SCOPE(h); RC(check_fwd(h, false, false, 1));
    hipDeviceSynchronize();
    free_list(h->enc_allocs);
    ++h->generation;
    h->enc_loaded = false;
    h->mixed_ready_n = 0; h->mixed_weight_bytes = 0; h->enc_weight_bytes = 0; h->mixed_pack_s = 0.0; h->split_weight_bytes = 0;
    const auto load_t0 = std::chrono::steady_clock::now();
    SD sd; sd.h = h;
    for (int i = 0; i < n; ++i) if (t[i].name) sd.m[t[i].name] = &t[i];
    auto& own = h->enc_allocs;

    {
        const float* W = sd.get("input_layer.0.weight", {64, 3, 3, 3});
        BNFold bn;
        if (!W || !bn_fold(sd, "input_layer.1", 64, bn)) return sd.rc;
        const float* sl = sd.get("input_layer.2.weight", {64});
        if (!sl) return sd.rc;
        std::vector<float> w(27 * 64), b(64), s(64);
        for (int co = 0; co < 64; ++co) {
            for (int k = 0; k < 27; ++k) w[k * 64 + co] = (float)((double)W[co * 27 + k] * bn.s[co]);
            b[co] = (float)bn.t[co];
            s[co] = sl[co];
        }
        RC(upload(h, own, w, &h->stem_w));
        RC(upload(h, own, b, &h->stem_b));
        RC(upload(h, own, s, &h->stem_s));
    }
    int n_blocks = 0;
    while (sd.m.count("body." + std::to_string(n_blocks) + ".res_layer.1.weight")) ++n_blocks;
    std::vector<int> cin, depth, stride;
    if (!block_table(n_blocks, cin, depth, stride))
        return fail(h, FFR_ERR_KEY, "the state_dict holds %d bottlenecks; Backbone has 24, 49 or 50 (num_layers 50, 100, 152)", n_blocks);
    const bool has_se = sd.m.count("body.0.res_layer.5.fc1.weight") != 0;
    h->blocks.assign(n_blocks, Block());
    for (int i = 0; i < n_blocks; ++i) {
        Block& b = h->blocks[i];
        b.cin = cin[i]; b.depth = depth[i]; b.stride = stride[i];
        const std::string p = "body." + std::to_string(i);
        BNFold bn1, bn2;
        if (!bn_fold(sd, p + ".res_layer.0", b.cin, bn1) || !bn_fold(sd, p + ".res_layer.4", b.depth, bn2)) return sd.rc;
        const float* W1 = sd.get(p + ".res_layer.1.weight", {b.depth, b.cin, 3, 3});
        const float* sl = sd.get(p + ".res_layer.2.weight", {b.depth});
        const float* W2 = sd.get(p + ".res_layer.3.weight", {b.depth, b.depth, 3, 3});
        const float* f1 = has_se ? sd.get(p + ".res_layer.5.fc1.weight", {b.depth / 16, b.depth, 1, 1}) : nullptr;
        const float* f2 = has_se ? sd.get(p + ".res_layer.5.fc2.weight", {b.depth, b.depth / 16, 1, 1}) : nullptr;
        if (!W1 || !sl || !W2 || (has_se && (!f1 || !f2))) return sd.rc;
        RC(pack_conv(h, own, W1, b.depth, b.cin, 3, 3, &bn1, nullptr, sl, 1, 1, 0, &b.c1));
        RC(pack_conv(h, own, W2, b.depth, b.depth, 3, 3, nullptr, &bn2, nullptr, b.stride, 1, 0, &b.c2));
        if (has_se) {
            RC(upload(h, own, std::vector<float>(f1, f1 + (size_t)b.depth / 16 * b.depth), &b.fc1));
            RC(upload(h, own, std::vector<float>(f2, f2 + (size_t)b.depth / 16 * b.depth), &b.fc2));
        }
        b.has_sc = b.cin != b.depth;
        if (b.has_sc) {
            BNFold bns;
            const float* Ws = sd.get(p + ".shortcut_layer.0.weight", {b.depth, b.cin, 1, 1});
            if (!Ws || !bn_fold(sd, p + ".shortcut_layer.1", b.depth, bns)) return sd.rc;
            RC(pack_conv(h, own, Ws, b.depth, b.cin, 1, 1, nullptr, &bns, nullptr, b.stride, 0, 0, &b.sc));
        }
    }
    {
        BNFold bn;
        if (!bn_fold(sd, "bn", 512, bn)) return sd.rc;
        std::vector<float> s(512), tt(512);
        for (int c = 0; c < 512; ++c) { s[c] = (float)bn.s[c]; tt[c] = (float)bn.t[c]; }
        RC(upload(h, own, s, &h->bn_s));
        RC(upload(h, own, tt, &h->bn_t));
    }
    {
        BNFold b0, b4;
        if (!bn_fold(sd, "output_layer.0", 512, b0) || !bn_fold(sd, "output_layer.4", 512, b4)) return sd.rc;
        const float* W = sd.get("output_layer.3.weight", {512, 25088});
        const float* bias = sd.get("output_layer.3.bias", {512});
        if (!W || !bias) return sd.rc;
        ConvW& L = h->fc;
        L = ConvW();
        L.cin = L.cin_pad = 25088; L.cout = L.cout_pad = 512; L.R = L.S = 1; L.stride = 1; L.pad = 0;
        std::vector<float> wp((size_t)512 * 25088), bb(512);
        std::vector<double> wd(wp.size());
        for (int o = 0; o < 512; ++o) {
            double acc = bias[o];
            for (int c = 0; c < 512; ++c)
                for (int p = 0; p < 49; ++p) {
                    const double wv = W[(size_t)o * 25088 + c * 49 + p];
                    wp[(size_t)o * 25088 + p * 512 + c] = (float)(wv * b0.s[c] * b4.s[o]);
                    wd[(size_t)o * 25088 + p * 512 + c] = wv * b0.s[c] * b4.s[o];
                    acc += wv * b0.t[c];
                }
            bb[o] = (float)(b4.s[o] * acc + b4.t[o]);
        }
        RC(upload(h, own, wp, &L.w));
        RC(upload(h, own, bb, &L.bias));
        RC(upload_split(h, own, wd, &L.w3));
    }
    h->enc_loaded = true;
    h->enc_load_s = std::chrono::duration<double>(std::chrono::steady_clock::now() - load_t0).count();
    return FFR_OK;
}

int ffr_load_recnet(ffr_handle* h, const ffr_tensor_desc* t, int n) {
    if (!h || !t || n <= 0) return fail(h, FFR_ERR_ARG, "ffr_load_recnet: bad arguments");
    FFR_DEVICE_SCOPE(h); RC(check_fwd(h, false, false, 1));
    hipDeviceSynchronize();
    free_list(h->rec_allocs);
    ++h->generation;
    h->rec_loaded = false;
    h->rec_weight_bytes = 0;
    const auto load_t0 = std::chrono::steady_clock::now();
    SD sd; sd.h = h;
    for (int i = 0; i < n; ++i) if (t[i].name) sd.m[t[i].name] = &t[i];
    auto& own = h->rec_allocs;

    auto conv_layer = [&](const std::string& p, int cin, int cout, ConvW* L) -> int {
        const float* W = sd.get(p + ".conv2d.weight", {cout, cin, 3, 3});
        const float* sl = sd.get(p + ".relu.func.weight", {cout});
        BNFold bn;
        if (!W || !sl || !bn_fold(sd, p + ".norm.norm", cout, bn)) return sd.rc;
        return pack_conv(h, own, W, cout, cin, 3, 3, nullptr, &bn, sl, 1, 1, 1, L);
    };
    for (int i = 0; i < 15; ++i) RC(conv_layer(REC_LAYERS[i].prefix, REC_LAYERS[i].cin, REC_LAYERS[i].cout, &rec_conv(h, i)));

    const float* W1 = sd.get("Conv4Channel.0.weight", {32, 561});
    const float* b1 = sd.get("Conv4Channel.0.bias", {32});
    const float* a1 = sd.get("Conv4Channel.1.func.weight", {512});
    const float* W2 = sd.get("Conv4Channel.2.weight", {512, 32});
    const float* b2 = sd.get("Conv4Channel.2.bias", {512});
    const float* W3 = sd.get("Conv4Channel.3.weight", {32, 512});
    const float* b3 = sd.get("Conv4Channel.3.bias", {32});
    const float* a4 = sd.get("Conv4Channel.4.func.weight", {512});
    const float* W5 = sd.get("Conv4Channel.5.weight", {512, 32});
    const float* b5 = sd.get("Conv4Channel.5.bias", {512});
    const float* W6 = sd.get("Conv4Channel.6.weight", {32, 512});
    const float* b6 = sd.get("Conv4Channel.6.bias", {32});
    const float* a7 = sd.get("Conv4Channel.7.func.weight", {512});
    const float* W8 = sd.get("Conv4Channel.8.weight", {512, 32});
    const float* b8 = sd.get("Conv4Channel.8.bias", {512});
    if (!W1 || !b1 || !a1 || !W2 || !b2 || !W3 || !b3 || !a4 || !W5 || !b5 || !W6 || !b6 || !a7 || !W8 || !b8) return sd.rc;
    std::vector<float> w1a(32 * 49), w1bT(512 * 32);
    for (int j = 0; j < 32; ++j) {
        for (int p = 0; p < 49; ++p) w1a[j * 49 + p] = W1[j * 561 + p];
        for (int c = 0; c < 512; ++c) w1bT[c * 32 + j] = W1[j * 561 + 49 + c];
    }
    auto fold = [](const float* Wb , const float* bb, const float* Wa , const float* ba,
                   std::vector<float>& A, std::vector<float>& d) {
        A.assign(32 * 32, 0.f); d.assign(32, 0.f);
        for (int j = 0; j < 32; ++j) {
            double dd = bb[j];
            for (int k = 0; k < 512; ++k) dd += (double)Wb[j * 512 + k] * ba[k];
            d[j] = (float)dd;
            for (int i = 0; i < 32; ++i) {
                double s = 0;
                for (int k = 0; k < 512; ++k) s += (double)Wb[j * 512 + k] * Wa[k * 32 + i];
                A[j * 32 + i] = (float)s;
            }
        }
    };
    std::vector<float> A2, d2, A3, d3;
    fold(W3, b3, W2, b2, A2, d2);
    fold(W6, b6, W5, b5, A3, d3);
// ... 33 lines not shown
```

### ffr-net_amd/csrc/plan.cpp

```cpp
#include "engine_internal.h"

namespace ffr_eng {

static bool wino_phased(const ffr_handle* h, int cin_pad, double x_bytes) {
    return cin_pad <= h->opt.wf_phased_maxk && x_bytes <= 1073741824.0;
}

static bool short_last_round(const ffr_handle* h, long long block_tiles) {
    const long long full = block_tiles / h->num_cus * h->num_cus, rem = block_tiles - full;
    return h->opt.wf_tailsplit != 0 && !h->opt.wf_trace && full > 0 && rem > 0 && rem * 4 <= h->num_cus;
}

ConvForce wino_fused_form(const ffr_handle* h, int cin_pad, int cout_pad, long long T, double x_bytes, ConvForce ask) {
    if (!h->opt.wino_fused || ask == ConvForce::Direct || ask == ConvForce::Unfused) return ConvForce::Unfused;
    if (ask == ConvForce::Fused || ask == ConvForce::FusedHalf) return ask;
    const long long min_blocks = h->opt.wf_minblocks;
    const long long mbn = (T + 31) / 32;
    const long long bt_full = mbn * (cout_pad / 64);
    auto fit = [&](long long bt) {
        const long long full = bt / h->num_cus * h->num_cus, rem = bt - full;
        if (rem == 0 || short_last_round(h, bt)) return 1.0;
        return (double)bt / (double)(full + h->num_cus);
    };
    bool half_n = false;
    if (!wino_phased(h, cin_pad, x_bytes)) {
        if (bt_full < min_blocks) half_n = 2 * bt_full >= min_blocks;
        else half_n = 0.92 * fit(2 * bt_full) > fit(bt_full);
    }
    if (mbn * (cout_pad / (half_n ? 32 : 64)) < min_blocks) return ConvForce::Unfused;
    return half_n ? ConvForce::FusedHalf : ConvForce::Fused;
}

bool wino_mixed_eligible(const ffr_handle* h, const ConvW& L, int N, int H, int W, int in_pitch, size_t wino_cap, ConvForce force) {
    if (!L.wuc || !L.w || L.R != 3 || L.S != 3 || L.stride != 1 || L.pad_mode != 0 || in_pitch != L.cin_pad) return false;
    if (!(H == 14 && W == 14) && !(force == ConvForce::Mixed && H == 7 && W == 7)) return false;
    WinoMixedGeom g;
    if (!wino_mixed_geom(H, W, &g) || wino_mixed_v_floats(g, N, L.cin_pad, nullptr) > wino_cap) return false;
    if (force == ConvForce::Mixed) return true;
    if (force != ConvForce::Auto || !layer_wino(h, L) || !h->opt.wino_fused || !h->opt.wf_mixed) return false;
    return wino_mixed_blocks(N, H, W, L.cout_pad) >= 2 * h->num_cus;
}

ConvPlan plan_conv(const ffr_handle* h, const ConvW& L, const ConvCall& c) {
    ConvPlan p;
    if (c.wino_stage == 2 && c.v_chunked) {
        ConvCall whole = c;
        whole.wino_stage = 0; whole.v_chunked = false;
        p = plan_conv(h, L, whole);
        if (!p.takes_v) { p = ConvPlan{}; p.refused = "a ready V was announced for a convolution that cannot take it"; }
        return p;
    }
    const ConvForce f = c.force;
    if (L.wum[1] && wino_mixed_eligible(h, L, c.N, c.H, c.W, c.in_pitch, c.wino_cap, f) && c.winoV && c.tile == 0 &&
        (c.wino_stage == 0 || (c.wino_stage == 2 && c.v_mixed)) && ((c.out_pitch | c.out_coff | c.res_pitch | c.cout_store) & 3) == 0)
        { p.path = ConvPlan::Mixed; return p; }
    if (!L.wu || !c.winoV || c.tile != 0 || (f == ConvForce::Auto ? !layer_wino(h, L) : f == ConvForce::Direct)) return p;
    const int tiles_img = ((c.H + 3) / 4) * ((c.W + 3) / 4);
    const long long T = (long long)c.N * tiles_img;
    const double x_bytes = 4.0 * c.N * c.H * c.W * c.in_pitch;
    const bool phased = wino_phased(h, L.cin_pad, x_bytes);
    const ConvForce form = wino_fused_form(h, L.cin_pad, L.cout_pad, T, x_bytes, f);
    if (form != ConvForce::Unfused && L.wuc && c.wino_stage == 0 && (phased || wino_chunked_floats(T, L.cin_pad) <= c.wino_cap) &&
        T < 0x7fffffffLL) {
        p.path = ConvPlan::Fused;
        p.phased = phased;
        p.half_n = form == ConvForce::FusedHalf;
        const int nbn = L.cout_pad / (p.half_n ? 32 : 64);
        const long long block_tiles = (T + 31) / 32 * nbn;
        if (f == ConvForce::Auto && short_last_round(h, block_tiles)) {
            const long long full = block_tiles / h->num_cus * h->num_cus;
            const int n_main = (int)((full / nbn) * 32 / tiles_img);
            const size_t rem_floats = (size_t)36 * (c.N - n_main) * tiles_img * (L.cin_pad > L.cout_pad ? L.cin_pad : L.cout_pad);
            if (n_main >= 1 && n_main < c.N && rem_floats <= c.wino_cap) {
                p.n_main = n_main;
                p.side = phased ? h->side : nullptr;
            }
        }
        p.takes_v = !phased && p.n_main == 0 && L.pad_mode == 0 && c.in_pitch == L.cin_pad;
        return p;
    }
    if (L.wu == L.wuc) p.refused = "Winograd weights exist in the fused kernel's order only, but this launch cannot run fused";
    else if ((size_t)36 * T * L.cin_pad <= c.wino_cap && (size_t)36 * T * L.cout_pad <= c.wino_cap && T < 0x7fffffffLL) p.path = ConvPlan::Unfused;
    return p;
}

void plan_igemm(long long M, int cout_pad, int nkt, int nbatch, int force_tile, int min_units, int* tile, int* nblocks, int* granule, bool split) {
    auto ntiles = [&](int t) {
        int bm, bn;
        igemm_tile_shape(t, &bm, &bn);
        return ((M + bm - 1) / bm) * (long long)(cout_pad / bn) * nbatch;
    };
    int best = (cout_pad % 128 == 0) ? IGEMM_TILE_128x128 : IGEMM_TILE_128x64;
    if (split && nkt < 16) best = IGEMM_TILE_128x64;
    const long long big_units = ntiles(best) * nkt;
    const bool large = big_units / (256LL * igemm_resident_blocks(best, split)) >= (nkt + 3) / 4 && M * nbatch >= 1024;
    if (!large) best = IGEMM_TILE_64x64;
    bool exact = false;
    if (large) {
        for (int t = IGEMM_TILE_128x128; t <= IGEMM_TILE_128x64; ++t) {
            int bm, bn;
            igemm_tile_shape(t, &bm, &bn);
            if (cout_pad % bn || (split && nkt < 16 && t == IGEMM_TILE_128x128)) continue;
            if (ntiles(t) % (256LL * igemm_resident_blocks(t, split)) == 0) { best = t; exact = true; break; }
        }
    }
    if (force_tile >= 1 && force_tile <= IGEMM_NTILES) { best = force_tile; exact = false; }
    const long long tiles = ntiles(best);
    const long long units = tiles * (long long)nkt;
    const long long pmax = 256LL * igemm_resident_blocks(best, split);
    long long p;
    *granule = 1;
    if (exact || (nkt < 16 && tiles >= pmax && (nkt <= 4 || tiles >= pmax * 8))) {
        *granule = nkt;
        p = pmax;
    } else if (large) {
        p = pmax;
        if (p > units / 4) p = units / 4;
    } else if (tiles >= 160 && tiles <= pmax) {
        *granule = nkt;
        p = tiles;
    } else {
        p = units / min_units;
        if (p > pmax) p = pmax;
    }
    if (p < 1) p = 1;
    *tile = best;
    *nblocks = (int)p;
}

}
```

### ffr-net_amd/csrc/wino_fused.hip

```cpp
#include "ffr_kernels.h"
#include "wino_math.h"

namespace ffr {

template <int PAD_MODE>
__global__ __launch_bounds__(256) void k_wino_in_c(const float* __restrict__ x, float* __restrict__ Vc, int H, int W, int pitch,
                                                  int nkc, int th, int tw, long long T) {
    const int lane = threadIdx.x & 63, wave = threadIdx.x >> 6;
    const int mb = blockIdx.x, kc = blockIdx.y * 4 + wave;
    const int tl = lane >> 1;
    const int hh = lane & 1;
    const long long t = (long long)mb * 32 + tl;
    const int c4 = kc * 8 + hh * 4;
    float* vout = Vc + (((size_t)mb * nkc + kc) * 36) * 256 + (hh * 32 + tl) * 4;
    if (t >= T) {
#pragma unroll
        for (int xi = 0; xi < 36; ++xi) *reinterpret_cast<f32x4*>(vout + xi * 256) = (f32x4){0.f, 0.f, 0.f, 0.f};
        return;
    }
    const unsigned tu = (unsigned)t, tpi = (unsigned)(tw * th);
    const int n = (int)(tu / tpi);
    const unsigned tr = tu - (unsigned)n * tpi;
    const int ty = (int)(tr / (unsigned)tw);
    const int tx = (int)(tr - (unsigned)ty * (unsigned)tw);
    const int h0 = ty * 4 - 1, w0 = tx * 4 - 1;
    const float* xn = x + (size_t)n * H * W * pitch + c4;
    f32x4 tmp[6][6];
#pragma unroll
    for (int j = 0; j < 6; ++j) {
        f32x4 d[6], v[6];
        int wi = w0 + j;
        bool okw = true;
        if (PAD_MODE == 1) wi = wi < 0 ? -wi : (wi >= W ? 2 * W - 2 - wi : wi);
        else okw = (unsigned)wi < (unsigned)W;
        if (PAD_MODE == 1 && wi < 0) wi = 0;
#pragma unroll
        for (int i = 0; i < 6; ++i) {
            int hi = h0 + i;
            bool ok = okw;
            if (PAD_MODE == 1) { hi = hi < 0 ? -hi : (hi >= H ? 2 * H - 2 - hi : hi); if (hi < 0) hi = 0; }
            else ok = ok && ((unsigned)hi < (unsigned)H);
            d[i] = (f32x4){0.f, 0.f, 0.f, 0.f};
            if (ok) d[i] = *reinterpret_cast<const f32x4*>(xn + ((size_t)hi * W + wi) * pitch);
        }
        bt6v(d, v);
#pragma unroll
        for (int i = 0; i < 6; ++i) tmp[i][j] = v[i];
    }
#pragma unroll
    for (int i = 0; i < 6; ++i) {
        f32x4 v[6];
        bt6v(tmp[i], v);
#pragma unroll
        for (int j = 0; j < 6; ++j) *reinterpret_cast<f32x4*>(vout + (i * 6 + j) * 256) = v[j];
    }
}

hipError_t launch_wino_in_chunked(const float* x, float* Vc, int N, int H, int W, int pitch, int cin_pad, int pad_mode,
                                  hipStream_t stream) {
    if (cin_pad % 32) return hipErrorInvalidValue;
    const int th = (H + 3) / 4, tw = (W + 3) / 4;
    const long long T = (long long)N * th * tw;
    const int mbn = (int)((T + 31) / 32);
    const dim3 grid(mbn, cin_pad / 32);
    if (pad_mode == 1) hipLaunchKernelGGL(k_wino_in_c<1>, grid, dim3(256), 0, stream, x, Vc, H, W, pitch, cin_pad / 8, th, tw, T);
    else hipLaunchKernelGGL(k_wino_in_c<0>, grid, dim3(256), 0, stream, x, Vc, H, W, pitch, cin_pad / 8, th, tw, T);
    return hipGetLastError();
}

constexpr int CIC_MAXPX = 392;
__global__ __launch_bounds__(256) void k_combine_in_c(const float* __restrict__ res, const float* __restrict__ scale,
                                                     const float* __restrict__ sh, float* __restrict__ out,
                                                     float* __restrict__ Vc, int N, int H, int W, int C, int nkc, int th, int tw) {
    __shared__ __attribute__((aligned(16))) float s_x[CIC_MAXPX * 32];
    const int tid = threadIdx.x, lane = tid & 63, wave = tid >> 6;
    const int mb = blockIdx.x;
    const int tiles_img = th * tw, ipg = 32 / tiles_img, HW = H * W;
    const int n_first = mb * ipg;
    const int n_imgs = N - n_first < ipg ? N - n_first : ipg;
    const int cb = blockIdx.y * 32;
    {
        const int q4 = (tid & 7) * 4;
        const int npx = n_imgs * HW;
        for (int p = tid >> 3; p < npx; p += 32) {
            const int il = p / HW;
            const size_t off = ((size_t)n_first * HW + p) * C + cb + q4;
            const f32x4 sv = scale ? *reinterpret_cast<const f32x4*>(scale + (size_t)(n_first + il) * C + cb + q4) : (f32x4){1.f, 1.f, 1.f, 1.f};
            const f32x4 x = *reinterpret_cast<const f32x4*>(res + off) * sv + *reinterpret_cast<const f32x4*>(sh + off);
            *reinterpret_cast<f32x4*>(out + off) = x;
            *reinterpret_cast<f32x4*>(s_x + p * 32 + q4) = x;
        }
    }
    __syncthreads();
    const int tl = 8 * wave + (lane >> 3), quad = lane & 7;
    const int kc = blockIdx.y * 4 + (quad >> 1), hf = quad & 1;
    float* vout = Vc + (((size_t)mb * nkc + kc) * 36) * 256 + (hf * 32 + tl) * 4;
    const int il = tl / tiles_img, tr = tl - il * tiles_img;
    const f32x4 zero4 = {0.f, 0.f, 0.f, 0.f};
    if (il >= n_imgs) {
#pragma unroll
        for (int xi = 0; xi < 36; ++xi) *reinterpret_cast<f32x4*>(vout + xi * 256) = zero4;
        return;
    }
    const int ty = tr / tw, tx = tr - ty * tw;
    const int h0 = ty * 4 - 1, w0 = tx * 4 - 1;
    const float* xi_base = s_x + il * HW * 32 + quad * 4;
    f32x4 d[6][6];
#pragma unroll
    for (int i = 0; i < 6; ++i) {
        const int hi = h0 + i;
        const bool okh = (unsigned)hi < (unsigned)H;
#pragma unroll
        for (int j = 0; j < 6; ++j) {
            const int wi = w0 + j;
            d[i][j] = zero4;
            if (okh && (unsigned)wi < (unsigned)W) d[i][j] = *reinterpret_cast<const f32x4*>(xi_base + (hi * W + wi) * 32);
        }
    }
#pragma unroll
    for (int j = 0; j < 6; ++j) {
        f32x4 col[6], v[6];
#pragma unroll
        for (int i = 0; i < 6; ++i) col[i] = d[i][j];
        bt6v(col, v);
#pragma unroll
        for (int i = 0; i < 6; ++i) d[i][j] = v[i];
    }
#pragma unroll
    for (int i = 0; i < 6; ++i) {
        f32x4 v[6];
        bt6v(d[i], v);
#pragma unroll
        for (int j = 0; j < 6; ++j) *reinterpret_cast<f32x4*>(vout + (i * 6 + j) * 256) = v[j];
    }
}

bool combine_in_c_supported(int H, int W, int C) {
    const int tiles_img = ((H + 3) / 4) * ((W + 3) / 4);
    return C % 32 == 0 && tiles_img <= 32 && 32 % tiles_img == 0 && (32 / tiles_img) * H * W <= CIC_MAXPX;
}

hipError_t launch_combine_in_c(const float* res, const float* scale, const float* sh, float* out, float* Vc, int N, int H,
                               int W, int C, hipStream_t stream) {
    if (!combine_in_c_supported(H, W, C)) return hipErrorInvalidValue;
    const int th = (H + 3) / 4, tw = (W + 3) / 4;
    const long long T = (long long)N * th * tw;
    const dim3 grid((unsigned)((T + 31) / 32), C / 32);
    hipLaunchKernelGGL(k_combine_in_c, grid, dim3(256), 0, stream, res, scale, sh, out, Vc, N, H, W, C, C / 8, th, tw);
    return hipGetLastError();
}

__device__ __forceinline__ void wait_vmcnt(int n) {
    switch (n) {
        case 0: asm volatile("s_waitcnt vmcnt(0)" ::: "memory"); break;
        case 3: asm volatile("s_waitcnt vmcnt(3)" ::: "memory"); break;
        case 6: asm volatile("s_waitcnt vmcnt(6)" ::: "memory"); break;
        case 9: asm volatile("s_waitcnt vmcnt(9)" ::: "memory"); break;
        case 12: asm volatile("s_waitcnt vmcnt(12)" ::: "memory"); break;
        case 15: asm volatile("s_waitcnt vmcnt(15)" ::: "memory"); break;
        case 18: asm volatile("s_waitcnt vmcnt(18)" ::: "memory"); break;
        case 21: asm volatile("s_waitcnt vmcnt(21)" ::: "memory"); break;
        default: asm volatile("s_waitcnt vmcnt(24)" ::: "memory"); break;
    }
}

constexpr int WF_EPI_FLOATS = 36 * 32 * 32;
constexpr int WF_LDS_BYTES = (WF_EPI_FLOATS + 9 * 64 + 32 * 8 + 32 * 12) * 4;

template <int MODE, int NT>
__global__ __launch_bounds__(256, 1) void k_wino_fused(const WinoFusedArgs a) {
    constexpr bool PHASED = MODE != 0;
    extern __shared__ __attribute__((aligned(16))) float smem[];
    const int wave = __builtin_amdgcn_readfirstlane(threadIdx.x >> 6);
    const int lane = threadIdx.x & 63;
    const int xcd = blockIdx.x & 7, idx = blockIdx.x >> 3;
    int nb, mb;
    if (a.map_v == 2) {
        nb = idx % a.nbn; mb = xcd * ((a.mbn + 7) >> 3) + idx / a.nbn;
        if (idx / a.nbn >= ((a.mbn + 7) >> 3)) return;
    } else if (a.map_v == 3) {
        const int hn = a.nbn >> 1;
        nb = (xcd >> 2) * hn + idx % hn; mb = (idx / hn) * 4 + (xcd & 3);
    } else if (a.map_v) {
        nb = idx % a.nbn; mb = (idx / a.nbn) * 8 + xcd;
    } else if (a.nbn % 8 == 0) {
        const int r = a.nbn >> 3;
        nb = xcd * r + idx % r; mb = idx / r;
    } else if (8 % a.nbn == 0) {
        const int per = 8 / a.nbn;
        nb = xcd % a.nbn; mb = xcd / a.nbn + per * idx;
    } else {
        nb = idx % a.nbn; mb = (idx / a.nbn) * 8 + xcd;
    }
    if (mb >= a.mbn) return;
    const int nkc = a.nkc;
    unsigned long long st0 = 0, st1 = 0, st2 = 0, se[4] = {0, 0, 0, 0};
    if (FFR_TRACE_ON(a.trace)) st0 = __builtin_amdgcn_s_memtime();
    const int tid = threadIdx.x;
    const int n0 = nb * (32 * NT);
    float* const s_bias = smem + WF_EPI_FLOATS;
    int* const s_tile = reinterpret_cast<int*>(s_bias + 9 * 64);
    for (int i = tid; i < (a.border_bias ? 9 : 1) * 64; i += 256)
        if ((i & 63) < 32 * NT) s_bias[i] = a.bias[(size_t)(i >> 6) * a.cout_pad + n0 + (i & 63)];
    if (tid < 32) {
        const long long t = (long long)mb * 32 + tid;
        int pix0 = 0, vrc = 0, br = 0, bc = 0, ibase = 0, h0 = 0, w0 = 0;
        if (t < a.T) {
            const unsigned tiles_img = (unsigned)(a.th * a.tw);
            const int n = (int)((unsigned)t / tiles_img);
            const int tr = (int)((unsigned)t - (unsigned)n * tiles_img);
            const int ty = (int)((unsigned)tr / (unsigned)a.tw), tx = tr - ty * a.tw;
            pix0 = (n * a.H + ty * 4) * a.W + tx * 4;
            ibase = n * a.H * a.W; h0 = ty * 4 - 1; w0 = tx * 4 - 1;
            const int vr = a.H - ty * 4 < 4 ? a.H - ty * 4 : 4, vc = a.W - tx * 4 < 4 ? a.W - tx * 4 : 4;
            vrc = vr | (vc << 8);
            br = (ty == 0 ? 1 : 0) | ((a.H - 1 - ty * 4) & 0xff) << 8;
            bc = (tx == 0 ? 1 : 0) | ((a.W - 1 - tx * 4) & 0xff) << 8;
        }
        s_tile[tid * 8 + 0] = pix0; s_tile[tid * 8 + 1] = vrc; s_tile[tid * 8 + 2] = br; s_tile[tid * 8 + 3] = bc;
        s_tile[tid * 8 + 4] = ibase; s_tile[tid * 8 + 5] = h0; s_tile[tid * 8 + 6] = w0;
        if constexpr (PHASED) {
            unsigned* const so = reinterpret_cast<unsigned*>(s_tile + 32 * 8) + tid * 12;
#pragma unroll
            for (int i = 0; i < 6; ++i) {
                int hi = h0 + i, wi = w0 + i;
                bool rok, cok;
                if (a.pad_mode == 1) {
                    hi = hi < 0 ? -hi : (hi >= a.H ? 2 * a.H - 2 - hi : hi); if (hi < 0) hi = 0;
                    wi = wi < 0 ? -wi : (wi >= a.W ? 2 * a.W - 2 - wi : wi); if (wi < 0) wi = 0;
                    rok = vrc != 0; cok = true;
                } else {
                    rok = vrc != 0 && (unsigned)hi < (unsigned)a.H;
                    cok = (unsigned)wi < (unsigned)a.W;
                }
                so[i] = rok ? (unsigned)((ibase + hi * a.W) * a.in_pitch) * 4u : 0x40000000u;
                so[6 + i] = cok ? (unsigned)(wi * a.in_pitch) * 4u : 0x40000000u;
            }
        }
    }

    const __amdgpu_buffer_rsrc_t vrs = __builtin_amdgcn_make_buffer_rsrc((void*)(PHASED ? a.Uc : a.Vc + (size_t)mb * nkc * 36 * 256), 0,
                                                                         PHASED ? 0u : (unsigned)nkc * 36u * 1024u, 0x00020000);
    const __amdgpu_buffer_rsrc_t urs = __builtin_amdgcn_make_buffer_rsrc((void*)a.Uc, 0, (unsigned)((size_t)a.cout_pad * nkc * 8 * 36 * 4), 0x00020000);
    const unsigned lane16 = (unsigned)lane * 16u;
    unsigned vp = (unsigned)(9 * wave) * 1024u;
    unsigned up = NT == 2 ? (unsigned)(nb * nkc * 36 + 9 * wave) * 2048u
                          : (unsigned)((nb >> 1) * nkc * 36 + 9 * wave) * 2048u + (unsigned)(nb & 1) * 1024u;
    auto ldfrag = [&](const __amdgpu_buffer_rsrc_t& rs, unsigned so) {
        return __builtin_bit_cast(f32x4, __builtin_amdgcn_raw_buffer_load_b128(rs, lane16, so, 0));
    };
    const int rowl = lane & 31;

    f32x16 acc[8][NT], accv[NT];
#pragma unroll
    for (int nt = 0; nt < NT; ++nt)
#pragma unroll
        for (int r = 0; r < 16; ++r) {
            accv[nt][r] = 0.f;
#pragma unroll
            for (int j = 0; j < 8; ++j) acc[j][nt][r] = 0.f;
        }

#define FFR_PIN __builtin_amdgcn_sched_barrier(0)
    if constexpr (MODE == 0) {
    f32x4 fv[9], fu[9][NT];
    auto load = [&](int j, int part, unsigned v, unsigned u) {
        if (part == 0) fv[j] = ldfrag(vrs, v + j * 1024u);
        else fu[j][part - 1] = ldfrag(urs, u + j * 2048u + (part - 1) * 1024u);
    };
#pragma unroll
    for (int j = 0; j < 8; ++j) {
#pragma unroll
        for (int part = 0; part <= NT; ++part) load(j, part, vp, up);
        FFR_PIN;
    }
    FFR_PIN;
    if (FFR_TRACE_ON(a.trace)) st1 = __builtin_amdgcn_s_memtime();

    auto chunk = [&]<bool LAST>() {
#pragma unroll
        for (int j = 0; j < 9; ++j) {
            const f32x4 av = fv[j], b0 = fu[j][0], b1 = fu[j][NT - 1];
#pragma unroll
            for (int g = 0; g < 4 * NT; ++g) {
                const int e = g / NT, nt = g % NT;
                if (j < 8) acc[j][nt] = __builtin_amdgcn_mfma_f32_32x32x2f32(nt ? b1[e] : b0[e], av[e], acc[j][nt], 0, 0, 0);
                else asm volatile("v_mfma_f32_32x32x2_f32 %0, %1, %2, %0" : "+v"(accv[nt]) : "v"(nt ? b1[e] : b0[e]), "v"(av[e]));
                if (g == 1) {
#pragma unroll
                    for (int part = 0; part <= NT; ++part) {
                        if (j == 0) load(8, part, vp, up);
                        else if (!LAST) load(j - 1, part, vp + 36 * 1024u, up + 36 * 2048u);
                    }
                }
                FFR_PIN;
            }
        }
    };
#pragma unroll 1
    for (int kc = 0; kc + 1 < nkc; ++kc) {
        chunk.template operator()<false>();
        vp += 36 * 1024u;
        up += 36 * 2048u;
    }
    chunk.template operator()<true>();
    } else if constexpr (MODE == 1) {
    f32x4 fu[9][NT];
    auto loadu = [&](int j, int part, unsigned u) {
        fu[j][part] = ldfrag(urs, u + j * 2048u + part * 1024u);
    };
    f32x4 af[2];
    int aoff[4];
#pragma unroll
    for (int c = 0; c < 4; ++c) aoff[c] = ((lane & 32) + (lane & 24) + ((lane + 2 * c + (lane >> 5)) & 7)) * 4;
    auto reada = [&](int buf, int c, int j) {
        af[buf] = *reinterpret_cast<const f32x4*>(smem + (c * 36 + 9 * wave + j) * 256 + aoff[c]);
    };
    __syncthreads();
    constexpr unsigned OOB = 0x40000000u;
    const __amdgpu_buffer_rsrc_t xrsrc = __builtin_amdgcn_make_buffer_rsrc((void*)a.x, 0, a.x_bytes, 0x00020000);
    const int nph = nkc >> 2;
    const int ttl = 8 * wave + (lane >> 3), tq = lane & 7;
    unsigned ro[6], co[6];
    const unsigned* const s_off = reinterpret_cast<const unsigned*>(s_tile + 32 * 8) + ttl * 12;
    auto offsets = [&]() {
#pragma unroll
        for (int i = 0; i < 6; ++i) {
            ro[i] = s_off[i] + (unsigned)tq * 16u;
            co[i] = s_off[6 + i];
        }
    };
    offsets();
    constexpr int NPRE = 16;
    f32x4 pre[NPRE];
    auto load_px = [&](int idx, unsigned so) {
        return __builtin_bit_cast(f32x4, __builtin_amdgcn_raw_buffer_load_b128(xrsrc, ro[idx % 6] + co[idx / 6], so, 0));
    };
#pragma unroll
    for (int k = 0; k < NPRE; ++k) pre[k] = load_px(k, 0u);
    if (FFR_TRACE_ON(a.trace)) st1 = __builtin_amdgcn_s_memtime();
#pragma unroll 1
    for (int ph = 0; ph < nph; ++ph) {
        unsigned long long tp0 = 0;
        if (FFR_TRACE_ON(a.trace)) tp0 = __builtin_amdgcn_s_memtime();
        const unsigned soff = (unsigned)(ph * 32) * 4u;
        const unsigned soff_next = ph + 1 < nph ? soff + 128u : soff;
        {
        f32x4 d[6][6];
#pragma unroll
        for (int j = 0; j < 6; ++j)
#pragma unroll
            for (int i = 0; i < 6; ++i) d[i][j] = j * 6 + i < NPRE ? pre[j * 6 + i] : load_px(j * 6 + i, soff);
#pragma unroll
        for (int j = 0; j < 6; ++j) {
            f32x4 col[6], v[6];
#pragma unroll
            for (int i = 0; i < 6; ++i) col[i] = d[i][j];
            bt6t(col, v);
#pragma unroll
            for (int i = 0; i < 6; ++i) d[i][j] = v[i];
        }
        float* vout = smem + (((tq >> 1) * 36) * 64 + (tq & 1) * 32 + (ttl & 24) + ((ttl + tq) & 7)) * 4;
#pragma unroll
        for (int i = 0; i < 6; ++i) {
            f32x4 v[6];
            bt6t(d[i], v);
#pragma unroll
            for (int j = 0; j < 6; ++j) *reinterpret_cast<f32x4*>(vout + (i * 6 + j) * 256) = v[j];
            if (i >= 2) {
#pragma unroll
                for (int q = 0; q < 2; ++q)
#pragma unroll
                    for (int part = 0; part < NT; ++part) loadu((i - 2) * 2 + q, part, up);
            }
        }
        }
        if (FFR_TRACE_ON(a.trace)) se[0] += __builtin_amdgcn_s_memtime() - tp0;
        __syncthreads();
        if (FFR_TRACE_ON(a.trace)) se[1] += __builtin_amdgcn_s_memtime() - tp0;
        reada(0, 0, 0);
#pragma unroll
        for (int c = 0; c < 4; ++c) {
#pragma unroll
            for (int j = 0; j < 9; ++j) {
                const int cur = (c * 9 + j) & 1;
                const f32x4 av = af[cur], b0 = fu[j][0], b1 = fu[j][NT - 1];
                const bool has_next = !(c == 3 && j == 8);
#pragma unroll
                for (int g = 0; g < 4 * NT; ++g) {
                    const int e = g / NT, nt = g % NT;
                    if (j < 8) acc[j][nt] = __builtin_amdgcn_mfma_f32_32x32x2f32(nt ? b1[e] : b0[e], av[e], acc[j][nt], 0, 0, 0);
                    else asm volatile("v_mfma_f32_32x32x2_f32 %0, %1, %2, %0" : "+v"(accv[nt]) : "v"(nt ? b1[e] : b0[e]), "v"(av[e]));
                    if (c == 3 && j == 0 && g == 0) offsets();
                    if (g == 1) {
#pragma unroll
                        for (int part = 0; part < NT; ++part) {
                            if (j == 0) loadu(8, part, up);
                            else if (c < 3) loadu(j - 1, part, up + 36 * 2048u);
                        }
                        if (c == 3 && j >= 1) {
#pragma unroll
                            for (int q = 0; q < NPRE / 8; ++q) pre[(NPRE / 8) * (j - 1) + q] = load_px((NPRE / 8) * (j - 1) + q, soff_next);
                        }
                    }
                    if (g == 2 * NT && has_next) reada(cur ^ 1, j == 8 ? c + 1 : c, j == 8 ? 0 : j + 1);
                    FFR_PIN;
                }
            }
            up += 36 * 2048u;
        }
        __syncthreads();
    }
    }
#undef FFR_PIN
    if (FFR_TRACE_ON(a.trace)) st2 = __builtin_amdgcn_s_memtime();

    asm volatile("s_nop 15\n\ts_nop 15" ::: "memory");
    const int hsel = lane >> 5;
    const int cq = lane & 7;
    const bool vec4 = ((a.out_pitch | a.out_coff | a.res_pitch) & 3) == 0;
#pragma unroll
    for (int nt = 0; nt < NT; ++nt) {
#pragma unroll
        for (int j = 0; j < 9; ++j)
#pragma unroll
            for (int q = 0; q < 4; ++q) {
                const f32x16& t16 = j < 8 ? acc[j < 8 ? j : 0][nt] : accv[nt];
                *reinterpret_cast<f32x4*>(smem + ((9 * wave + j) * 32 + rowl) * 32 + (((2 * q + hsel) ^ (rowl & 7)) * 4)) =
                    (f32x4){t16[4 * q], t16[4 * q + 1], t16[4 * q + 2], t16[4 * q + 3]};
            }
        __syncthreads();
        if (FFR_TRACE_ON(a.trace) && !PHASED) se[2 * nt] = __builtin_amdgcn_s_memtime();
        const int tl = (lane >> 3) + 8 * wave;
        const int vrc = s_tile[tl * 8 + 1];
        if (vrc != 0) {
            const int pix0 = s_tile[tl * 8 + 0];
            const int vr = vrc & 0xff, vc = vrc >> 8;
            const f32x4* e = reinterpret_cast<const f32x4*>(smem + tl * 32 + 4 * (cq ^ (tl & 7)));
            f32x4 y[4][4];
            {
                f32x4 tmp[4][6];
#pragma unroll
                for (int j = 0; j < 6; ++j) {
                    f32x4 mc[6], yc[4];
#pragma unroll
                    for (int i = 0; i < 6; ++i) mc[i] = e[(i * 6 + j) * 256];
                    at6q(mc, yc);
#pragma unroll
                    for (int i = 0; i < 4; ++i) tmp[i][j] = yc[i];
                }
#pragma unroll
                for (int i = 0; i < 4; ++i) at6q(tmp[i], y[i]);
            }
            const int cl = nt * 32 + 4 * cq;
            const int cg = n0 + cl;
            f32x4 slope = {1.f, 1.f, 1.f, 1.f};
            if (a.slope) slope = *reinterpret_cast<const f32x4*>(a.slope + cg);
            f32x4 bs[4][4];
            if (!a.border_bias) {
                const f32x4 b0 = *reinterpret_cast<const f32x4*>(s_bias + cl);
#pragma unroll
                for (int i = 0; i < 4; ++i)
#pragma unroll
                    for (int jj = 0; jj < 4; ++jj) bs[i][jj] = b0;
            } else {
                const int br = s_tile[tl * 8 + 2], bc = s_tile[tl * 8 + 3];
                int rc[4], cc[4];
#pragma unroll
                for (int i = 0; i < 4; ++i) {
                    rc[i] = ((i == 0 && (br & 1)) ? 0 : (i == (br >> 8) ? 2 : 1)) * 3 * 64;
                    cc[i] = ((i == 0 && (bc & 1)) ? 0 : (i == (bc >> 8) ? 2 : 1)) * 64;
                }
#pragma unroll
                for (int i = 0; i < 4; ++i)
#pragma unroll
                    for (int jj = 0; jj < 4; ++jj) bs[i][jj] = *reinterpret_cast<const f32x4*>(s_bias + rc[i] + cc[jj] + cl);
            }
            f32x4 psum = {0.f, 0.f, 0.f, 0.f};
            if (vec4 && cg + 3 < a.cout_store) {
                int ro[4], co[4];
#pragma unroll
                for (int i = 0; i < 4; ++i) {
                    ro[i] = (i < vr ? i : vr - 1) * a.W;
                    co[i] = i < vc ? i : vc - 1;
                }
                float* const ob = a.out + (size_t)pix0 * a.out_pitch + a.out_coff + cg;
                const float* const rb = a.resid ? a.resid + (size_t)pix0 * a.res_pitch + cg : nullptr;
                f32x4 rs[4][4];
                if (rb) {
#pragma unroll
                    for (int i = 0; i < 4; ++i)
#pragma unroll
                        for (int jj = 0; jj < 4; ++jj) rs[i][jj] = *reinterpret_cast<const f32x4*>(rb + (ro[i] + co[jj]) * a.res_pitch);
                }
                float mr[4], mc[4];
#pragma unroll
                for (int i = 0; i < 4; ++i) { mr[i] = i < vr ? 1.f : 0.f; mc[i] = i < vc ? 1.f : 0.f; }
#pragma unroll
                for (int i = 3; i >= 0; --i)
#pragma unroll
                    for (int jj = 3; jj >= 0; --jj) {
                        f32x4 v = y[i][jj] + bs[i][jj];
#pragma unroll
                        for (int c = 0; c < 4; ++c) v[c] = fmaxf(v[c], 0.f) + slope[c] * fminf(v[c], 0.f);
                        if (rb) v += rs[i][jj];
                        if (a.flags & 1) {
#pragma unroll
                            for (int c = 0; c < 4; ++c) v[c] = 1.0f / (1.0f + __expf(-v[c]));
                        }
                        *reinterpret_cast<f32x4*>(ob + (ro[i] + co[jj]) * a.out_pitch) = v;
                        if (a.tile_sums) psum += v * (mr[i] * mc[jj]);
                    }
            } else {
#pragma unroll
                for (int i = 0; i < 4; ++i)
#pragma unroll
                    for (int jj = 0; jj < 4; ++jj) {
                        if (!(i < vr && jj < vc)) continue;
                        const size_t m = (size_t)pix0 + i * a.W + jj;
#pragma unroll
                        for (int c = 0; c < 4; ++c) {
                            if (cg + c >= a.cout_store) continue;
                            float v = y[i][jj][c] + bs[i][jj][c];
                            v = fmaxf(v, 0.f) + slope[c] * fminf(v, 0.f);
                            if (a.resid) v += a.resid[m * a.res_pitch + cg + c];
                            if (a.flags & 1) v = 1.0f / (1.0f + __expf(-v));
                            a.out[m * a.out_pitch + a.out_coff + cg + c] = v;
                            psum[c] += v;
                        }
                    }
            }
            if (a.tile_sums) {
                const long long t = (long long)mb * 32 + tl;
                *reinterpret_cast<f32x4*>(a.tile_sums + (size_t)t * a.cout_pad + cg) = psum;
            }
        }
        if (FFR_TRACE_ON(a.trace) && !PHASED) se[2 * nt + 1] = __builtin_amdgcn_s_memtime();
        __syncthreads();
    }
    if (FFR_TRACE_ON(a.trace) && lane == 0) {
        unsigned long long* tr = a.trace + ((size_t)blockIdx.x * 4 + wave) * 10;
        tr[0] = st0; tr[1] = st1; tr[2] = st2; tr[3] = __builtin_amdgcn_s_memtime();
        tr[6] = se[0]; tr[7] = se[1];
        tr[8] = NT == 2 ? se[2] : se[1]; tr[9] = NT == 2 ? se[3] : se[1];
        if (PHASED) {
            tr[6] = st2 + se[0] / (nkc >> 2); tr[7] = tr[6] + (se[1] - se[0]) / (nkc >> 2); tr[8] = tr[7]; tr[9] = tr[7];
        }
        tr[4] = __builtin_amdgcn_s_memrealtime();
        unsigned xcc;
        asm volatile("s_getreg_b32 %0, hwreg(HW_REG_XCC_ID)" : "=s"(xcc));
        tr[5] = xcc & 0xf;
    }
}

hipError_t wino_fused_init() {
    const void* fns[4] = {(const void*)k_wino_fused<0, 2>, (const void*)k_wino_fused<1, 2>,
                          (const void*)k_wino_fused<0, 1>, (const void*)k_wino_fused<1, 1>};
    for (const void* f : fns) {
        hipError_t e = hipFuncSetAttribute(f, hipFuncAttributeMaxDynamicSharedMemorySize, WF_LDS_BYTES);
        if (e != hipSuccess) return e;
    }
    return hipSuccess;
}

static int wf_grid(int mbn, int nbn, int map_v) {
    if (map_v == 3) return (mbn + 3) / 4 * 8 * (nbn >> 1);
    if (map_v) return (mbn + 7) / 8 * 8 * nbn;
    if (nbn % 8 == 0) return mbn * nbn;
    if (8 % nbn == 0) { const int per = 8 / nbn; return 8 * ((mbn + per - 1) / per); }
    return (mbn + 7) / 8 * 8 * nbn;
}

int wino_fused_blocks(const WinoFusedArgs& a) {
    const long long T = (long long)a.N * ((a.H + 3) / 4) * ((a.W + 3) / 4);
    return wf_grid((int)((T + 31) / 32), a.cout_pad / (a.half_n ? 32 : 64), a.map_v);
}

hipError_t launch_wino_fused(WinoFusedArgs a, hipStream_t stream) {
    if (a.cout_pad % 64 || a.nkc < 2) return hipErrorInvalidValue;
    a.th = (a.H + 3) / 4; a.tw = (a.W + 3) / 4;
    a.T = (long long)a.N * a.th * a.tw;
    a.mbn = (int)((a.T + 31) / 32);
    a.nbn = a.cout_pad / (a.half_n ? 32 : 64);
    const dim3 grid(wf_grid(a.mbn, a.nbn, a.map_v));
    if (a.Vc) {
        if (a.half_n) hipLaunchKernelGGL((k_wino_fused<0, 1>), grid, dim3(256), WF_LDS_BYTES, stream, a);
        else hipLaunchKernelGGL((k_wino_fused<0, 2>), grid, dim3(256), WF_LDS_BYTES, stream, a);
    } else {
        if (!a.x || a.nkc % 4 || a.x_bytes == 0 || a.x_bytes > 0x40000000u) return hipErrorInvalidValue;
        if (a.half_n) hipLaunchKernelGGL((k_wino_fused<1, 1>), grid, dim3(256), WF_LDS_BYTES, stream, a);
        else hipLaunchKernelGGL((k_wino_fused<1, 2>), grid, dim3(256), WF_LDS_BYTES, stream, a);
    }
    return hipGetLastError();
}

}
```

### ffr-net_amd/native.py

```python
import ctypes as C
import os

import torch

from . import align as _align

_HERE = os.path.dirname(os.path.abspath(__file__))
_LIB = None

KCLASS_NAMES = ['conv_igemm', 'stem', 'se', 'combine', 'head', 'selfsim', 'channel',
                'space', 'layout', 'score', 'wino', 'wino_fused', 'wgrad',
                'train_bn', 'train_loss', 'train_optim', 'train_xform', 'train_elem']


class NativeLibraryMissing(RuntimeError):
    pass


class TensorDesc(C.Structure):
    _fields_ = [('name', C.c_char_p), ('data', C.c_void_p), ('ndim', C.c_int32),
                ('shape', C.c_int64 * 4)]


class MemStats(C.Structure):
    _fields_ = [('encoder_weight_bytes', C.c_size_t), ('recnet_weight_bytes', C.c_size_t), ('mixed_tile_weight_bytes', C.c_size_t),
                ('workspace_bytes', C.c_size_t), ('encoder_load_seconds', C.c_double), ('recnet_load_seconds', C.c_double),
                ('mixed_tile_pack_seconds', C.c_double), ('split_weight_bytes', C.c_size_t)]


class KClassStat(C.Structure):
    _fields_ = [('launches', C.c_int64), ('ms', C.c_double), ('flops', C.c_double),
                ('bytes', C.c_double), ('flops_executed', C.c_double), ('flops_useful', C.c_double)]


class ConvDesc(C.Structure):
    _fields_ = [('x', C.c_void_p), ('N', C.c_int), ('H', C.c_int), ('W', C.c_int),
                ('in_pitch', C.c_int), ('cin_pad', C.c_int),
                ('w', C.c_void_p), ('bias', C.c_void_p), ('slope', C.c_void_p),
                ('resid', C.c_void_p), ('res_pitch', C.c_int),
                ('out', C.c_void_p), ('out_pitch', C.c_int), ('out_coff', C.c_int),
                ('cout_store', C.c_int), ('cout_pad', C.c_int),
                ('R', C.c_int), ('S', C.c_int), ('stride', C.c_int), ('pad', C.c_int),
                ('pad_mode', C.c_int), ('border_bias', C.c_int), ('flags', C.c_int),
                ('tile', C.c_int), ('splitk', C.c_int)]


class LayerInfo(C.Structure):
    _fields_ = [('name', C.c_char * 64), ('net', C.c_int), ('arith', C.c_int), ('sensitivity', C.c_double)]


class WgradLaunch(C.Structure):
    _fields_ = [('name', C.c_char * 48)] + [(f, C.c_int) for f in (
        'path', 'rows', 'cout_pad', 'Ng', 'nbatch', 'nkt', 'splits', 'kt_per_split', 'full_tiles', 'tail_splits', 'tail_kt',
        'accumulate')]


WGRAD_PATHS = ('plain-taps9', 'plain-taps1', 'batched')
ARITH = {'direct': 0, 'winograd': 1}
CALIB_TENSORS = ('f', 'featmap', 'f_new', 'feat_new')


_LIB_PATH = os.path.join(_HERE, 'libffrnet_hip.so')


def lib_path():
    return _LIB_PATH


def set_library(path):
    global _LIB_PATH
    if _LIB is not None:
        raise RuntimeError('ffrnet_amd: the native library is already loaded')
    _LIB_PATH = os.path.abspath(path)


_P = C.c_void_p
SYMBOLS = [
    ('ffr_create', C.c_int, [C.POINTER(_P), C.c_int]),
    ('ffr_destroy', None, [_P]),
    ('ffr_last_error', C.c_char_p, [_P]),
    ('ffr_version', C.c_char_p, []),
    ('ffr_load_encoder', C.c_int, [_P, C.POINTER(TensorDesc), C.c_int]),
    ('ffr_load_recnet', C.c_int, [_P, C.POINTER(TensorDesc), C.c_int]),
    ('ffr_encoder_forward', C.c_int, [_P, _P, C.c_int, C.c_int, C.c_int, _P, _P, _P]),
    ('ffr_recnet_forward', C.c_int, [_P, _P, C.c_int, _P, _P, _P]),
    ('ffr_embed', C.c_int, [_P, _P, C.c_int, _P, _P, _P]),
    ('ffr_embed_u8', C.c_int, [_P, _P, _P, C.c_int, _P, _P, _P]),
    ('ffr_encoder_forward_u8', C.c_int, [_P, _P, _P, C.c_int, C.c_int, C.c_int, _P, _P, _P]),
    ('ffr_cosine_scores', C.c_int, [_P, _P, _P, C.c_int, C.c_int, _P, _P]),
    ('ffr_lfw_fold_accuracy', C.c_int, [_P, _P, _P, C.c_int, C.c_int, _P, _P, _P]),
    ('ffr_row_norms', C.c_int, [_P, _P, C.c_longlong, C.c_int, _P, _P]),
    ('ffr_search_topk', C.c_int, [_P, _P, C.c_int, _P, _P, C.c_longlong, C.c_int, C.c_int, C.c_longlong, _P, _P, _P]),
    ('ffr_topk_merge', C.c_int, [_P, _P, _P, C.c_int, C.c_int, C.c_int, _P, _P, _P]),
    ('ffr_align_transforms', C.c_int, [_P, _P, _P, C.c_int, C.c_int, _P, _P, _P]),
    ('ffr_align_warp', C.c_int, [_P, _P, C.c_int, C.c_int, C.c_int, C.c_longlong, _P, _P, _P, C.c_int, C.c_int, C.c_int, _P, _P]),
    ('ffr_embed_aligned', C.c_int, [_P, _P, C.c_int, C.c_int, C.c_int, C.c_longlong, _P, _P, _P, C.c_int, _P, C.c_int, _P, _P, _P,
                                    _P]),
    ('ffr_workspace_bytes', C.c_size_t, [_P, C.c_int, C.c_int, C.c_int]),
    ('ffr_reserve', C.c_int, [_P, C.c_int, C.c_int, C.c_int]),
    ('ffr_generation', C.c_ulonglong, [_P]),
    ('ffr_layer_count', C.c_int, [_P, C.POINTER(C.c_int)]),
    ('ffr_layer_get', C.c_int, [_P, C.c_int, C.POINTER(LayerInfo)]),
    ('ffr_layer_set_arith', C.c_int, [_P, C.c_int, C.c_int]),
    ('ffr_calibrate', C.c_int, [_P, _P, _P, C.c_int, C.c_int, C.c_int, C.c_double, C.POINTER(C.c_double), _P]),
    ('ffr_memory_stats', C.c_int, [_P, _P]),
    ('ffr_set_option', C.c_int, [_P, C.c_char_p, C.c_longlong]),
    ('ffr_get_option', C.c_int, [_P, C.c_char_p, C.POINTER(C.c_longlong)]),
    ('ffr_probe_mfma_peak', C.c_int, [_P, C.c_int, C.POINTER(C.c_double), C.POINTER(C.c_double), _P]),
    ('ffr_profile_enable', C.c_int, [_P, C.c_int]),
    ('ffr_profile_read', C.c_int, [_P, C.POINTER(KClassStat)]),
    ('ffr_op_conv', C.c_int, [_P, C.POINTER(ConvDesc), _P]),
    ('ffr_op_conv3x3', C.c_int, [_P, _P, C.c_int, C.c_int, C.c_int, C.c_int, _P, _P, _P, C.c_int, C.c_int, C.c_int, _P, _P, _P]),
    ('ffr_encoder_trunk_nhwc', C.c_int, [_P, _P, C.c_int, C.c_int, C.c_int, C.c_int, _P, _P]),
    ('ffr_recnet_debug', C.c_int, [_P, _P, C.c_int, _P, _P, _P, _P, _P, _P, _P, _P]),
    ('ffr_op_convlayer_train', C.c_int, [_P, _P, C.c_int, C.c_int, C.c_int, C.c_int, _P, _P, _P, _P, _P, _P, _P, _P, _P, _P, _P]),
    ('ffr_train_init', C.c_int, [_P, C.POINTER(TensorDesc), C.c_int]),
    ('ffr_train_info', C.c_int, [_P, C.POINTER(_P), C.POINTER(_P), C.POINTER(C.c_size_t), C.POINTER(C.c_longlong),
                                 C.POINTER(C.c_int)]),
    ('ffr_train_get', C.c_int, [_P, C.c_int, C.c_char_p, _P, C.c_size_t]),
    ('ffr_train_set', C.c_int, [_P, C.c_int, C.c_char_p, _P, C.c_size_t]),
    ('ffr_train_zero_grad', C.c_int, [_P, _P]),
    ('ffr_train_forward', C.c_int, [_P, C.c_int, _P, _P, C.c_int, C.c_int, _P, _P, _P, _P, _P, _P, _P, _P]),
    ('ffr_train_backward', C.c_int, [_P, C.c_int, _P, _P, _P, _P, _P, _P, _P, _P]),
    ('ffr_train_adam_step', C.c_int, [_P, C.c_double, C.c_double, C.c_double, C.c_double, C.c_double, C.c_double, _P]),
    ('ffr_train_debug_copy', C.c_int, [_P, C.c_int, C.c_char_p, _P, C.c_size_t]),
    ('ffr_train_option', C.c_int, [_P, C.c_char_p, C.c_int]),
    ('ffr_train_wgrad_plan', C.c_int, [_P, C.POINTER(WgradLaunch), C.c_int, C.POINTER(C.c_int)]),
    ('ffr_train_buckets', C.c_int, [_P, C.POINTER(C.c_int), C.POINTER(C.c_size_t), C.POINTER(C.c_int)]),
    ('ffr_train_bucket_wait', C.c_int, [_P, C.c_int, _P]),
    ('ffr_train_export', C.c_int, [_P, C.c_int, C.c_char_p, _P, _P]),
    ('ffr_train_import', C.c_int, [_P, C.c_int, C.c_char_p, _P, _P]),
    ('ffr_train_losses', C.c_int, [_P, C.c_int, _P, C.POINTER(C.c_double), _P, _P]),
    ('ffr_train_backward_losses', C.c_int, [_P, C.c_int, _P]),
    ('ffr_train_iteration', C.c_int, [_P, _P, _P, _P, C.c_int, C.POINTER(C.c_double), _P, _P]),
    ('ffr_train_iteration_u8', C.c_int, [_P, _P, _P, _P, _P, C.c_int, C.POINTER(C.c_double), _P, _P]),
]


def load_library():
    global _LIB
    if _LIB is not None:
        return _LIB
    path = lib_path()
    if not os.path.exists(path):
        raise NativeLibraryMissing(
            'ffrnet_amd: %s not found -- build it with `python -c "import __graft_entry__ as g; '
            'g.build()"` (hipcc --offload-arch=gfx950). There is no CPU fallback.' % path)
    lib = C.CDLL(path)
    for name, res, args in SYMBOLS:
        fn = getattr(lib, name)
        fn.restype = res
        fn.argtypes = args
    _LIB = lib
    return lib


def _ptr(t):
    return C.c_void_p(t.data_ptr()) if t is not None else C.c_void_p(0)


def _check_dev(t, name, shape_tail=None, device=None):
    if not isinstance(t, torch.Tensor):
        raise TypeError('%s must be a torch.Tensor' % name)
    if not t.is_cuda:
        raise RuntimeError('ffrnet_amd: %s is on %s; the native HIP path needs a ROCm device '
                           'tensor (there is no CPU fallback)' % (name, t.device))
    if device is not None and t.device.index != device.index:
        raise RuntimeError('ffrnet_amd: %s is on %s but this Engine lives on %s; move the tensor there (or create the '
                           'Engine on the tensor\'s device: one process per GPU calls torch.cuda.set_device(local_rank) '
                           'before anything else)' % (name, t.device, device))
    if t.dtype != torch.float32:
        raise RuntimeError('ffrnet_amd: %s must be float32, got %s' % (name, t.dtype))
    if shape_tail is not None and tuple(t.shape[1:]) != tuple(shape_tail):
        raise RuntimeError('ffrnet_amd: %s expected shape [N,%s], got %s'
                           % (name, ','.join(map(str, shape_tail)), list(t.shape)))


def _check_u8(t, name, device, hw=None):
    if not isinstance(t, torch.Tensor):
        raise TypeError('%s must be a torch.Tensor' % name)
    if not t.is_cuda:
        raise RuntimeError('ffrnet_amd: %s is on %s; the native HIP path needs a ROCm device tensor (there is no CPU '
                           'fallback)' % (name, t.device))
    if t.device.index != device.index:
        raise RuntimeError('ffrnet_amd: %s is on %s but this Engine lives on %s' % (name, t.device, device))
    if t.dtype != torch.uint8:
        raise RuntimeError('ffrnet_amd: %s must be uint8 images [N,H,W,3], got %s' % (name, t.dtype))
    if t.dim() != 4 or t.size(3) != 3 or (hw is not None and tuple(t.shape[1:3]) != tuple(hw)):
        raise RuntimeError('ffrnet_amd: %s expected shape [N,%s,3] (HWC, RGB), got %s'
                           % (name, '%d,%d' % tuple(hw) if hw is not None else 'H,W', list(t.shape)))


def _flip_flags(flip, n, device, name='flip'):
    if flip is None:
        return None
    if not isinstance(flip, torch.Tensor) or flip.dtype not in (torch.bool, torch.uint8):
        raise RuntimeError('ffrnet_amd: %s must be a bool or uint8 tensor, got %s'
                           % (name, flip.dtype if isinstance(flip, torch.Tensor) else type(flip)))
    if flip.numel() != n:
        raise RuntimeError('ffrnet_amd: %s must hold %d flags, got %d' % (name, n, flip.numel()))
    if flip.is_cuda and flip.device.index != device.index:
        raise RuntimeError('ffrnet_amd: %s is on %s but this Engine lives on %s' % (name, flip.device, device))
    return flip.reshape(-1).to(device, torch.uint8).contiguous()


class Engine(object):

    def __init__(self, device=0):
        self.lib = load_library()
        self.device = torch.device('cuda', device if isinstance(device, int) else
                                   (device.index or 0))
        self._h = C.c_void_p(0)
        self._ck(self.lib.ffr_create(C.byref(self._h), self.device.index), create=True)
        self.has_encoder = False
        self.has_recnet = False
        self._recnet_sig = None

    def _ck(self, rc, create=False):
        if rc != 0:
            msg = self.lib.ffr_last_error(None if create else self._h)
            raise RuntimeError('ffrnet native error %d: %s' % (rc, (msg or b'?').decode()))

    def close(self):
        if getattr(self, '_h', None) and self._h.value:
            self.lib.ffr_destroy(self._h)
            self._h = C.c_void_p(0)

    def __del__(self):
        try:
            self.close()
        except Exception:
            pass

    def _stream(self):
        return C.c_void_p(torch.cuda.current_stream(self.device).cuda_stream)

    @staticmethod
    def _descs(sd):
        keep, items = [], []
        for k, v in sd.items():
            if not torch.is_tensor(v) or not v.is_floating_point():
                continue
            t = v.detach().to('cpu', torch.float32).contiguous()
            if t.dim() < 1 or t.dim() > 4:
                continue
            keep.append(t)
            d = TensorDesc()
            d.name = k.encode()
            d.data = t.data_ptr()
            d.ndim = t.dim()
            for i, s in enumerate(t.shape):
                d.shape[i] = s
            items.append(d)
        arr = (TensorDesc * len(items))(*items)
        return arr, len(items), keep

    def load_encoder(self, state_dict):
        arr, n, keep = self._descs(state_dict)
# ... 652 lines not shown
```

### include/ffrnet.h

```cpp
#ifndef FFRNET_H
#define FFRNET_H

#include <stddef.h>
#include <stdint.h>

#ifdef __cplusplus
extern "C" {
#endif

typedef struct ffr_handle ffr_handle;

typedef enum {
    FFR_OK = 0,
    FFR_ERR_ARG = -1,
    FFR_ERR_STATE = -2,
    FFR_ERR_KEY = -3,
    FFR_ERR_HIP = -4,
    FFR_ERR_NOMEM = -5,
    FFR_ERR_UNSUPPORTED = -6
} ffr_status;

typedef struct {
    const char*  name;
    const float* data;
    int32_t      ndim;
    int64_t      shape[4];
} ffr_tensor_desc;

int  ffr_create(ffr_handle** out, int device);
void ffr_destroy(ffr_handle* h);
const char* ffr_last_error(const ffr_handle* h);
const char* ffr_version(void);

int ffr_load_encoder(ffr_handle* h, const ffr_tensor_desc* t, int n);
int ffr_load_recnet(ffr_handle* h, const ffr_tensor_desc* t, int n);

int ffr_encoder_forward(ffr_handle* h, const float* x_nchw, int N, int H, int W,
                        float* featmap_nchw, float* f, void* stream);
int ffr_encoder_forward_u8(ffr_handle* h, const uint8_t* img_hwc_rgb, const uint8_t* flip, int N, int H, int W,
                           float* featmap_nchw, float* f, void* stream);

int ffr_recnet_forward(ffr_handle* h, const float* featmap_nchw, int N,
                       float* f_new, float* feat_new_nchw, void* stream);

int ffr_embed(ffr_handle* h, const float* x_nchw, int N,
              float* f_new, float* f, void* stream);

int ffr_embed_u8(ffr_handle* h, const uint8_t* img_hwc_rgb, const uint8_t* flip, int N,
                 float* f_new, float* f, void* stream);

int ffr_cosine_scores(ffr_handle* h, const float* a, const float* b, int n, int dim,
                      float* score, void* stream);

int ffr_row_norms(ffr_handle* h, const float* x, long long n, int dim, float* norms, void* stream);
int ffr_search_topk(ffr_handle* h, const float* query, int Q, const float* gallery, const float* gallery_norms,
                    long long G, int dim, int k, long long index_base,
                    float* top_score, int64_t* top_index, void* stream);
int ffr_topk_merge(ffr_handle* h, const float* score, const int64_t* index, int S, int Q, int k,
                   float* out_score, int64_t* out_index, void* stream);

int ffr_align_transforms(ffr_handle* h, const float* landmarks, const float* tmpl, int N, int K,
                         double* A, uint8_t* valid, void* stream);
int ffr_align_warp(ffr_handle* h, const uint8_t* frames, int F, int H, int W, long long pitch_bytes,
                   const int32_t* frame_index, const double* A, const uint8_t* valid, int N,
                   int out_h, int out_w, uint8_t* crop, void* stream);
int ffr_embed_aligned(ffr_handle* h, const uint8_t* frames, int F, int H, int W, long long pitch_bytes,
                      const int32_t* frame_index, const float* landmarks, const float* tmpl, int K,
                      const uint8_t* flip, int N, float* f_new, float* f, uint8_t* valid, void* stream);

int ffr_lfw_fold_accuracy(ffr_handle* h, const float* score, const int32_t* label, int n, int n_folds,
                          double* best_thr, double* test_acc, void* stream);

size_t ffr_workspace_bytes(const ffr_handle* h, int N, int H, int W);
int    ffr_reserve(ffr_handle* h, int N, int H, int W);

enum {
    FFR_KC_CONV_IGEMM = 0,
    FFR_KC_STEM = 1,
    FFR_KC_SE = 2,
    FFR_KC_COMBINE = 3,
    FFR_KC_HEAD = 4,
    FFR_KC_SELFSIM = 5,
    FFR_KC_CHANNEL = 6,
    FFR_KC_SPACE = 7,
    FFR_KC_LAYOUT = 8,
    FFR_KC_SCORE = 9,
    FFR_KC_WINO = 10,
    FFR_KC_WINO_FUSED = 11,
    FFR_KC_WGRAD = 12,
    FFR_KC_TRAIN_BN = 13,
    FFR_KC_TRAIN_LOSS = 14,
    FFR_KC_TRAIN_OPTIM = 15,
    FFR_KC_TRAIN_XFORM = 16,
    FFR_KC_TRAIN_ELEM = 17,
    FFR_KC_COUNT = 18
};
typedef struct {
    int64_t launches;
    double  ms;
    double  flops;
    double  bytes;
    double  flops_executed;
    double  flops_useful;
} ffr_kclass_stat;
int ffr_profile_enable(ffr_handle* h, int on);
int ffr_set_option(ffr_handle* h, const char* name, long long value);
int ffr_get_option(const ffr_handle* h, const char* name, long long* value);
unsigned long long ffr_generation(const ffr_handle* h);

enum { FFR_ARITH_DIRECT = 0, FFR_ARITH_WINOGRAD = 1 };
typedef struct {
    char   name[64];
    int    net;
    int    arith;
    double sensitivity;
} ffr_layer_info;
int ffr_layer_count(const ffr_handle* h, int* n);
int ffr_layer_get(const ffr_handle* h, int i, ffr_layer_info* out);
int ffr_layer_set_arith(ffr_handle* h, int i, int arith);
int ffr_calibrate(ffr_handle* h, const float* x_nchw, const float* featmap_nchw, int N, int H, int W,
                  double tol, double* achieved, void* stream);
typedef struct ffr_mem_stats {
    size_t encoder_weight_bytes, recnet_weight_bytes, mixed_tile_weight_bytes, workspace_bytes;
    double encoder_load_seconds, recnet_load_seconds, mixed_tile_pack_seconds;
    size_t split_weight_bytes;
} ffr_mem_stats;
int ffr_memory_stats(const ffr_handle* h, ffr_mem_stats* out);
int ffr_probe_mfma_peak(ffr_handle* h, int iters, double* tflops, double* clock_ghz, void* stream);
int ffr_profile_read(ffr_handle* h, ffr_kclass_stat* out );

typedef struct {
    const float* x; int N, H, W, in_pitch, cin_pad;
    const float* w; const float* bias; const float* slope;
    const float* resid; int res_pitch;
    float* out; int out_pitch, out_coff, cout_store, cout_pad;
    int R, S, stride, pad, pad_mode, border_bias, flags;
    int tile, splitk;
} ffr_conv_desc;
int ffr_op_conv(ffr_handle* h, const ffr_conv_desc* d, void* stream);

int ffr_op_conv3x3(ffr_handle* h, const float* x_nhwc, int N, int H, int W, int cin,
                   const float* w_host, const float* bias_host, const float* slope_host, int cout,
                   int pad_mode, int use_wino, const float* resid_nhwc, float* out_nhwc, void* stream);

int ffr_encoder_trunk_nhwc(ffr_handle* h, const float* x_nchw, int N, int H, int W,
                           int n_blocks, float* out_nhwc, void* stream);

int ffr_recnet_debug(ffr_handle* h, const float* featmap_nchw, int N,
                     float* ss_space, float* M_space, float* feat_space,
                     float* feat_channel_raw, float* feat_channel, float* ss_channel0, float* M_channel0,
                     void* stream);

#ifdef __cplusplus
}
#endif
#endif
```

Baseline: 16570 embeddings/s.

## Add split-operand bf16x3 MFMA K loop to the phased fused Winograd kernel

```diff
diff --git a/ffr-net_amd/csrc/conv.cpp b/ffr-net_amd/csrc/conv.cpp
--- a/ffr-net_amd/csrc/conv.cpp
+++ b/ffr-net_amd/csrc/conv.cpp
@@ -127,7 +127,7 @@
         const int cpp = 4, nph = f.nkc / cpp;
         fprintf(stderr, "[wf trace] %dx%d cin %d cout %d (input transform in the kernel, %d-channel blocks%s): %d live blocks of %d | per block (wave 0): "
                         "prologue %.0f loop %.0f = %d phases x (transform %.0f + barrier %.0f + %d K chunks of %.0f) epilogue %.0f cyc | "
-                        "block ends spread over %.1f us\n", c.H, c.W, L.cin_pad, L.cout_pad, p.half_n ? 32 : 64, "", cnt, nb,
+                        "block ends spread over %.1f us\n", c.H, c.W, L.cin_pad, L.cout_pad, p.half_n ? 32 : 64, p.split ? ", split-operand K loop" : "", cnt, nb,
                 pro / cnt, loop / cnt, nph, ep[0] / cnt, ep[1] / cnt, cpp, (loop / cnt / nph - ep[0] / cnt - ep[1] / cnt) / cpp, epi / cnt,
                 (double)(r1 - r0) / 100.0);
     }
@@ -208,6 +208,7 @@
     f.Vc = p.phased ? nullptr : c.winoV; f.x = c.x; f.in_pitch = c.in_pitch; f.pad_mode = L.pad_mode;
     f.x_bytes = p.phased ? (unsigned)(4.0 * c.N * c.H * c.W * c.in_pitch) : 0u;
     f.map_v = p.phased ? 2 : 1; f.half_n = p.half_n ? 1 : 0;
+    f.U3 = p.split ? L.wu3 : nullptr;
     f.Uc = L.wuc; f.bias = L.bias; f.slope = L.slope; f.resid = c.resid; f.out = c.out; f.tile_sums = c.tile_sums;
     f.N = c.N; f.H = c.H; f.W = c.W; f.nkc = L.cin_pad / 8;
     f.cout_pad = L.cout_pad; f.cout_store = c.cout_store; f.out_pitch = c.out_pitch; f.out_coff = c.out_coff;
@@ -218,6 +219,7 @@
 #endif
     Scope s(h, st, FFR_KC_WINO_FUSED, flops, bytes, fexec, flops / 4.0);
     HIPCK(h, launch_wino_fused(f, st));
+    if (p.split) ++h->wf_split_launches;
     return FFR_OK;
 }
 
@@ -289,7 +291,7 @@
     if (p.path == ConvPlan::Fused && !p.n_main) return conv_fused(h, L, c, p, flops, bytes, st);
     if (p.path == ConvPlan::Fused) {
         ConvCall c1 = c, c2 = c;
-        c1.N = p.n_main; c1.force = p.half_n ? ConvForce::FusedHalf : ConvForce::Fused;
+        c1.N = p.n_main; c1.force = p.half_n ? ConvForce::FusedHalf : p.split ? ConvForce::FusedSplit : ConvForce::Fused;
         c2.N = c.N - p.n_main; c2.force = ConvForce::Unfused;
         const size_t px = (size_t)p.n_main * c.H * c.W;
         c2.x = c.x + px * c.in_pitch;
diff --git a/ffr-net_amd/csrc/engine.cpp b/ffr-net_amd/csrc/engine.cpp
--- a/ffr-net_amd/csrc/engine.cpp
+++ b/ffr-net_amd/csrc/engine.cpp
@@ -113,6 +113,18 @@
     out->recnet_load_seconds = h->rec_load_s;
     out->mixed_tile_pack_seconds = h->mixed_pack_s;
     out->split_weight_bytes = h->split_weight_bytes;
+    out->wf_split_weight_bytes = h->wf_split_weight_bytes;
+    out->wf_split_launches = h->wf_split_launches;
+    return FFR_OK;
+}
+
+int ffr_split_planes_host(const double* w, long long n, unsigned short* planes) {
+    if (!w || !planes || n < 0) return FFR_ERR_ARG;
+    for (long long i = 0; i < n; ++i) {
+        unsigned short q[3];
+        split_bf16x3(w[i], q);
+        for (int p = 0; p < 3; ++p) planes[(size_t)p * n + i] = q[p];
+    }
     return FFR_OK;
 }
 
@@ -527,7 +539,7 @@
     {"wf_phased_maxk", &Options::wf_phased_maxk, nullptr, 0, 1 << 20}, {"wf_minblocks", nullptr, &Options::wf_minblocks, 0, 1LL << 40},
     {"se_maxtiles", &Options::se_maxtiles, nullptr, 0, 1 << 20}, {"wf_tailsplit", &Options::wf_tailsplit, nullptr, 0, 1},
     {"gemm_stream", &Options::gemm_stream, nullptr, 0, 1}, {"sk_minunits", &Options::sk_minunits, nullptr, 1, 1 << 20},
-    {"combine_v", &Options::combine_v, nullptr, 0, 1}, {"wf_mixed", &Options::wf_mixed, nullptr, 0, 1},
+    {"combine_v", &Options::combine_v, nullptr, 0, 1}, {"wf_split", &Options::wf_split, nullptr, 0, 1}, {"wf_mixed", &Options::wf_mixed, nullptr, 0, 1},
     {"channel_rows", &Options::channel_rows, nullptr, 0, 4}, {"igemm_split", &Options::igemm_split, nullptr, 0, 1},
     {"wf_trace", &Options::wf_trace, nullptr, 0, 1}, {"igemm_trace", &Options::igemm_trace, nullptr, 0, 1},
 };
@@ -651,7 +663,7 @@
     FFR_DEVICE_SCOPE(h); RC(check_fwd(h, false, false, N));
     if (!x || !w_host || !bias_host || !out || cin % 32 || cout % 4 || cin <= 0 || cout <= 0)
         return fail(h, FFR_ERR_ARG, "ffr_op_conv3x3: bad arguments (cin %% 32, cout %% 4)");
-    if (use_wino < 0 || use_wino > 4) return fail(h, FFR_ERR_ARG, "ffr_op_conv3x3: use_wino must be 0..4");
+    if (use_wino < 0 || use_wino > 5) return fail(h, FFR_ERR_ARG, "ffr_op_conv3x3: use_wino must be 0..5");
     hipStream_t st = (hipStream_t)stream;
     Work w;
     RC(ensure_arena(h, N > 8 ? N : 8, 112, 112, &w));
@@ -662,6 +674,8 @@
     ConvW L;
     int rc = pack_conv(h, own, w_host, cout, cin, 3, 3, nullptr, &ob, slope_host, 1, 1, pad_mode, &L);
     if (rc == FFR_OK && use_wino && !L.wu) rc = fail(h, FFR_ERR_UNSUPPORTED, "layer not eligible for the Winograd path (cin < FFR_WINO_MINCIN)");
+    if (rc == FFR_OK && use_wino == 5 && !L.wu3)
+        rc = fail(h, FFR_ERR_UNSUPPORTED, "the split-operand fused form needs cin <= wf_phased_maxk (%d) and room for its weight planes", h->opt.wf_phased_maxk);
     if (rc == FFR_OK && use_wino == 4) {
         if (!wino_mixed_eligible(h, L, N, H, W, cin, w.wino_cap, ConvForce::Mixed)) rc = fail(h, FFR_ERR_UNSUPPORTED, "layer / map not eligible for the mixed-tile path");
         else rc = ensure_mixed_weights(h, L, own, true);
diff --git a/ffr-net_amd/csrc/engine_internal.h b/ffr-net_amd/csrc/engine_internal.h
--- a/ffr-net_amd/csrc/engine_internal.h
+++ b/ffr-net_amd/csrc/engine_internal.h
@@ -32,6 +32,7 @@
     float* wum[4] = {nullptr, nullptr, nullptr, nullptr};
     bool wum_gave_up = false;
     unsigned short* w3 = nullptr;
+    unsigned short* wu3 = nullptr;
     float* wuc = nullptr;
     bool direct = false;
     double sensitivity = -1.0;
@@ -58,6 +59,7 @@
     int wf_mixed = 1;
     int channel_rows = 0;
     int igemm_split = 1;
+    int wf_split = 1;
     int combine_v = 1;
     int wf_trace = 0, igemm_trace = 0;
 };
@@ -84,6 +86,8 @@
     size_t mixed_weight_bytes = 0;
     double enc_load_s = 0.0, rec_load_s = 0.0, mixed_pack_s = 0.0;
     size_t split_weight_bytes = 0;
+    size_t wf_split_weight_bytes = 0;
+    long long wf_split_launches = 0;
     bool mixed_gave_up_logged = false, split_gave_up_logged = false;
     int mixed_ready_n = 0, mixed_ready_h = 0, mixed_ready_w = 0;
     float *stem_w = nullptr, *stem_b = nullptr, *stem_s = nullptr;
@@ -186,6 +190,8 @@
 int upload(ffr_handle* h, std::vector<void*>& owner, const std::vector<float>& v, float** out);
 int pack_conv(ffr_handle* h, std::vector<void*>& owner, const float* W, int cout, int cin, int R, int S,
               const BNFold* in_bn, const BNFold* out_bn, const float* slope, int stride, int pad, int pad_mode, ConvW* L);
+void split_bf16x3(double w, unsigned short out[3]);
+void pack_wino_split(const double* ud, int cout_pad, int cin_pad, unsigned short* pl);
 void free_list(std::vector<void*>& v);
 int ensure_mixed_weights(ffr_handle* h, ConvW& L, std::vector<void*>& owner, bool strict);
 int prepare_mixed_weights(ffr_handle* h, int N, int H, int W, size_t wino_cap);
@@ -193,7 +199,7 @@
 extern const RecLayer REC_LAYERS[15];
 inline ConvW& rec_conv(ffr_handle* h, int i) { return i < 9 ? h->sp[i] : i < 12 ? h->fm[i - 9] : h->mg[i - 12]; }
 
-enum class ConvForce { Auto = -1, Direct = 0, Fused = 1, Unfused = 2, FusedHalf = 3, Mixed = 4 };
+enum class ConvForce { Auto = -1, Direct = 0, Fused = 1, Unfused = 2, FusedHalf = 3, Mixed = 4, FusedSplit = 5 };
 
 struct ConvCall {
     const float* x; int N, H, W, in_pitch;
@@ -214,6 +220,7 @@
     enum Path { Direct, Mixed, Fused, Unfused } path = Direct;
     bool half_n = false;
     bool phased = false;
+    bool split = false;
     int n_main = 0;
     hipStream_t side = nullptr;
     bool takes_v = false;
diff --git a/ffr-net_amd/csrc/ffr_kernels.h b/ffr-net_amd/csrc/ffr_kernels.h
--- a/ffr-net_amd/csrc/ffr_kernels.h
+++ b/ffr-net_amd/csrc/ffr_kernels.h
@@ -9,6 +9,12 @@
 #endif
 
 namespace ffr {
+
+__device__ __forceinline__ unsigned cvt_pk_bf16(float lo, float hi) {
+    unsigned r;
+    asm("v_cvt_pk_bf16_f32 %0, %1, %2" : "=v"(r) : "v"(lo), "v"(hi));
+    return r;
+}
 
 struct IgemmArgs {
     const float* x;
@@ -74,7 +80,9 @@
     int th, tw, mbn, nbn;
     long long T;
     unsigned long long* trace;
+    const unsigned short* U3;
 };
+inline size_t wino_split_u_elems(int cout_pad, int cin_pad) { return (size_t)(cout_pad / 64) * (cin_pad / 16) * 36 * 2 * 3 * 64 * 8; }
 bool combine_in_c_supported(int H, int W, int C);
 hipError_t launch_combine_in_c(const float* res, const float* scale, const float* sh, float* out, float* Vc, int N, int H,
                                int W, int C, hipStream_t stream);
diff --git a/ffr-net_amd/csrc/igemm.hip b/ffr-net_amd/csrc/igemm.hip
--- a/ffr-net_amd/csrc/igemm.hip
+++ b/ffr-net_amd/csrc/igemm.hip
@@ -11,12 +11,6 @@
 
 #define LDS_PTR(p) ((__attribute__((address_space(3))) void*)(p))
 #define GLB_PTR(p) ((const __attribute__((address_space(1))) void*)(p))
-
-__device__ __forceinline__ unsigned cvt_pk_bf16(float lo, float hi) {
-    unsigned r;
-    asm("v_cvt_pk_bf16_f32 %0, %1, %2" : "=v"(r) : "v"(lo), "v"(hi));
-    return r;
-}
 
 template <int BM, int BN, int WARPS_M, int WARPS_N, int PAD_MODE, bool SPLIT = false>
 __global__ __launch_bounds__(256) void k_igemm(const IgemmArgs a) {
diff --git a/ffr-net_amd/csrc/pack.cpp b/ffr-net_amd/csrc/pack.cpp
--- a/ffr-net_amd/csrc/pack.cpp
+++ b/ffr-net_amd/csrc/pack.cpp
@@ -50,21 +50,48 @@
     return std::nearbyint(std::ldexp(d, -q)) * std::ldexp(1.0, q);
 }
 
+void split_bf16x3(double w, unsigned short out[3]) {
+    for (int p = 0; p < 3; ++p) {
+        const double b = round_bf16(w);
+        const float bf = (float)b;
+        unsigned u;
+        memcpy(&u, &bf, 4);
+        out[p] = (unsigned short)(u >> 16);
+        w -= b;
+    }
+}
+
+static int upload_planes(ffr_handle* h, std::vector<void*>& owner, const std::vector<unsigned short>& pl, size_t* counter, unsigned short** out);
+
 int upload_split(ffr_handle* h, std::vector<void*>& owner, const std::vector<double>& wd, unsigned short** out) {
-    *out = nullptr;
     const size_t n = wd.size();
     std::vector<unsigned short> pl(3 * n);
     for (size_t i = 0; i < n; ++i) {
-        double r = wd[i];
-        for (int p = 0; p < 3; ++p) {
-            const double b = round_bf16(r);
-            const float bf = (float)b;
-            unsigned u;
-            memcpy(&u, &bf, 4);
-            pl[(size_t)p * n + i] = (unsigned short)(u >> 16);
-            r -= b;
-        }
-    }
+        unsigned short q[3];
+        split_bf16x3(wd[i], q);
+        for (int p = 0; p < 3; ++p) pl[(size_t)p * n + i] = q[p];
+    }
+    return upload_planes(h, owner, pl, &h->split_weight_bytes, out);
+}
+
+void pack_wino_split(const double* ud, int cout_pad, int cin_pad, unsigned short* pl) {
+    const int nst = cin_pad / 16;
+    for (int nb = 0; nb < cout_pad / 64; ++nb)
+        for (int s = 0; s < nst; ++s)
+            for (int xi = 0; xi < 36; ++xi)
+                for (int nt = 0; nt < 2; ++nt)
+                    for (int lane = 0; lane < 64; ++lane)
+                        for (int i = 0; i < 8; ++i) {
+                            const int co = nb * 64 + nt * 32 + (lane & 31), ci = 16 * s + 8 * (lane >> 5) + i;
+                            unsigned short q[3];
+                            split_bf16x3(ud[((size_t)xi * cout_pad + co) * cin_pad + ci], q);
+                            const size_t base = ((((size_t)nb * nst + s) * 36 + xi) * 2 + nt) * 3;
+                            for (int p = 0; p < 3; ++p) pl[((base + p) * 64 + lane) * 8 + i] = q[p];
+                        }
+}
+
+static int upload_planes(ffr_handle* h, std::vector<void*>& owner, const std::vector<unsigned short>& pl, size_t* counter, unsigned short** out) {
+    *out = nullptr;
     void* p = nullptr;
     const size_t bytes = pl.size() * sizeof(unsigned short);
     hipError_t e = hipMalloc(&p, bytes);
@@ -80,7 +107,7 @@
         return FFR_OK;
     }
     owner.push_back(p);
-    if (&owner == &h->enc_allocs) { h->enc_weight_bytes += bytes; h->split_weight_bytes += bytes; }
+    if (&owner == &h->enc_allocs) { h->enc_weight_bytes += bytes; *counter += bytes; }
     if (&owner == &h->rec_allocs) h->rec_weight_bytes += bytes;
     *out = (unsigned short*)p;
     return FFR_OK;
@@ -140,6 +167,7 @@
     if (!wino) RC(upload_split(h, owner, wd, &L->w3));
     L->wu = nullptr;
     L->wuc = nullptr;
+    L->wu3 = nullptr;
     for (int tau = 0; tau < 4; ++tau) L->wum[tau] = nullptr;
     L->direct = false;
     L->sensitivity = -1.0;
@@ -147,6 +175,9 @@
         static const double G[6][3] = {{0.25, 0, 0}, {-1.0 / 6, -1.0 / 6, -1.0 / 6}, {-1.0 / 6, 1.0 / 6, -1.0 / 6},
                                        {1.0 / 24, 1.0 / 12, 1.0 / 6}, {1.0 / 24, -1.0 / 12, 1.0 / 6}, {0, 0, 1}};
         std::vector<float> wu((size_t)36 * L->cout_pad * L->cin_pad, 0.f);
+        const bool split = L->cin_pad <= h->opt.wf_phased_maxk && L->cin_pad % 32 == 0;
+        std::vector<double> wud;
+        if (split) wud.assign(wu.size(), 0.0);
         for (int co = 0; co < cout; ++co) {
             const double g = out_bn ? out_bn->s[co] : 1.0;
             for (int ci = 0; ci < cin; ++ci) {
@@ -159,6 +190,7 @@
                     for (int j = 0; j < 6; ++j) {
                         const double u = tmp[i][0] * G[j][0] + tmp[i][1] * G[j][1] + tmp[i][2] * G[j][2];
                         wu[((size_t)(i * 6 + j) * L->cout_pad + co) * L->cin_pad + ci] = (float)(u * sc);
+                        if (split) wud[((size_t)(i * 6 + j) * L->cout_pad + co) * L->cin_pad + ci] = u * sc;
                     }
             }
         }
@@ -176,6 +208,11 @@
                             for (int e = 0; e < 4; ++e) dst[e] = src[e];
                         }
         RC(upload(h, owner, wuc, &L->wuc));
+        if (split) {
+            std::vector<unsigned short> pl(wino_split_u_elems(L->cout_pad, L->cin_pad));
+            pack_wino_split(wud.data(), L->cout_pad, L->cin_pad, pl.data());
+            RC(upload_planes(h, owner, pl, &h->wf_split_weight_bytes, &L->wu3));
+        }
     }
     L->slope = nullptr;
     if (slope) {
@@ -276,7 +313,7 @@
     free_list(h->enc_allocs);
     ++h->generation;
     h->enc_loaded = false;
-    h->mixed_ready_n = 0; h->mixed_weight_bytes = 0; h->enc_weight_bytes = 0; h->mixed_pack_s = 0.0; h->split_weight_bytes = 0;
+    h->mixed_ready_n = 0; h->mixed_weight_bytes = 0; h->enc_weight_bytes = 0; h->mixed_pack_s = 0.0; h->split_weight_bytes = 0; h->wf_split_weight_bytes = 0;
     const auto load_t0 = std::chrono::steady_clock::now();
     SD sd; sd.h = h;
     for (int i = 0; i < n; ++i) if (t[i].name) sd.m[t[i].name] = &t[i];
diff --git a/ffr-net_amd/csrc/plan.cpp b/ffr-net_amd/csrc/plan.cpp
--- a/ffr-net_amd/csrc/plan.cpp
+++ b/ffr-net_amd/csrc/plan.cpp
@@ -13,6 +13,7 @@
 
 ConvForce wino_fused_form(const ffr_handle* h, int cin_pad, int cout_pad, long long T, double x_bytes, ConvForce ask) {
     if (!h->opt.wino_fused || ask == ConvForce::Direct || ask == ConvForce::Unfused) return ConvForce::Unfused;
+    if (ask == ConvForce::FusedSplit) return ConvForce::Fused;
     if (ask == ConvForce::Fused || ask == ConvForce::FusedHalf) return ask;
     const long long min_blocks = h->opt.wf_minblocks;
     const long long mbn = (T + 31) / 32;
@@ -65,6 +66,8 @@
         p.path = ConvPlan::Fused;
         p.phased = phased;
         p.half_n = form == ConvForce::FusedHalf;
+        p.split = L.wu3 && phased && !p.half_n && (f == ConvForce::FusedSplit || (f == ConvForce::Auto && h->opt.wf_split != 0));
+        if (f == ConvForce::FusedSplit && !p.split) { p = ConvPlan{}; p.refused = "the split-operand fused form was asked for a layer or launch that cannot run it"; return p; }
         const int nbn = L.cout_pad / (p.half_n ? 32 : 64);
         const long long block_tiles = (T + 31) / 32 * nbn;
         if (f == ConvForce::Auto && short_last_round(h, block_tiles)) {
@@ -79,7 +82,8 @@
         p.takes_v = !phased && p.n_main == 0 && L.pad_mode == 0 && c.in_pitch == L.cin_pad;
         return p;
     }
-    if (L.wu == L.wuc) p.refused = "Winograd weights exist in the fused kernel's order only, but this launch cannot run fused";
+    if (f == ConvForce::FusedSplit) p.refused = "the split-operand fused form was asked for a launch that cannot run fused";
+    else if (L.wu == L.wuc) p.refused = "Winograd weights exist in the fused kernel's order only, but this launch cannot run fused";
     else if ((size_t)36 * T * L.cin_pad <= c.wino_cap && (size_t)36 * T * L.cout_pad <= c.wino_cap && T < 0x7fffffffLL) p.path = ConvPlan::Unfused;
     return p;
 }
diff --git a/ffr-net_amd/csrc/wino_fused.hip b/ffr-net_amd/csrc/wino_fused.hip
--- a/ffr-net_amd/csrc/wino_fused.hip
+++ b/ffr-net_amd/csrc/wino_fused.hip
@@ -2,6 +2,9 @@
 #include "wino_math.h"
 
 namespace ffr {
+
+typedef unsigned u32x4 __attribute__((ext_vector_type(4)));
+typedef __bf16 bf16x8 __attribute__((ext_vector_type(8)));
 
 template <int PAD_MODE>
 __global__ __launch_bounds__(256) void k_wino_in_c(const float* __restrict__ x, float* __restrict__ Vc, int H, int W, int pitch,
@@ -165,11 +168,13 @@
 }
 
 constexpr int WF_EPI_FLOATS = 36 * 32 * 32;
+constexpr int WF_U3_STEP = 2 * 3 * 64 * 16;
 constexpr int WF_LDS_BYTES = (WF_EPI_FLOATS + 9 * 64 + 32 * 8 + 32 * 12) * 4;
 
-template <int MODE, int NT>
+template <int MODE, int NT, bool SPLIT = false>
 __global__ __launch_bounds__(256, 1) void k_wino_fused(const WinoFusedArgs a) {
     constexpr bool PHASED = MODE != 0;
+    static_assert(!SPLIT || (MODE == 1 && NT == 2), "the split-operand form exists for the in-kernel transform with 32 x 64 blocks");
     extern __shared__ __attribute__((aligned(16))) float smem[];
     const int wave = __builtin_amdgcn_readfirstlane(threadIdx.x >> 6);
     const int lane = threadIdx.x & 63;
@@ -241,10 +246,13 @@
 
     const __amdgpu_buffer_rsrc_t vrs = __builtin_amdgcn_make_buffer_rsrc((void*)(PHASED ? a.Uc : a.Vc + (size_t)mb * nkc * 36 * 256), 0,
                                                                          PHASED ? 0u : (unsigned)nkc * 36u * 1024u, 0x00020000);
-    const __amdgpu_buffer_rsrc_t urs = __builtin_amdgcn_make_buffer_rsrc((void*)a.Uc, 0, (unsigned)((size_t)a.cout_pad * nkc * 8 * 36 * 4), 0x00020000);
+    const __amdgpu_buffer_rsrc_t urs = SPLIT
+        ? __builtin_amdgcn_make_buffer_rsrc((void*)a.U3, 0, (unsigned)((size_t)(a.cout_pad >> 6) * (nkc >> 1) * 36 * WF_U3_STEP), 0x00020000)
+        : __builtin_amdgcn_make_buffer_rsrc((void*)a.Uc, 0, (unsigned)((size_t)a.cout_pad * nkc * 8 * 36 * 4), 0x00020000);
     const unsigned lane16 = (unsigned)lane * 16u;
     unsigned vp = (unsigned)(9 * wave) * 1024u;
-    unsigned up = NT == 2 ? (unsigned)(nb * nkc * 36 + 9 * wave) * 2048u
+    unsigned up = SPLIT ? (unsigned)(nb * (nkc >> 1) * 36 + 9 * wave) * (unsigned)WF_U3_STEP
+                : NT == 2 ? (unsigned)(nb * nkc * 36 + 9 * wave) * 2048u
                           : (unsigned)((nb >> 1) * nkc * 36 + 9 * wave) * 2048u + (unsigned)(nb & 1) * 1024u;
     auto ldfrag = [&](const __amdgpu_buffer_rsrc_t& rs, unsigned so) {
         return __builtin_bit_cast(f32x4, __builtin_amdgcn_raw_buffer_load_b128(rs, lane16, so, 0));
@@ -315,6 +323,44 @@
     for (int c = 0; c < 4; ++c) aoff[c] = ((lane & 32) + (lane & 24) + ((lane + 2 * c + (lane >> 5)) & 7)) * 4;
     auto reada = [&](int buf, int c, int j) {
         af[buf] = *reinterpret_cast<const f32x4*>(smem + (c * 36 + 9 * wave + j) * 256 + aoff[c]);
+    };
+    constexpr int NS = 3;
+    constexpr int PU[6] = {2, 0, 1, 1, 0, 0}, PV[6] = {0, 2, 1, 0, 1, 0};
+    u32x4 fu3[SPLIT ? NS : 1][NT][3], pv[2][3];
+    f32x4 vraw[2];
+    int voff[2][2];
+#pragma unroll
+    for (int s = 0; s < 2; ++s)
+#pragma unroll
+        for (int hh = 0; hh < 2; ++hh) {
+            const int c = 2 * s + (lane >> 5);
+            voff[s][hh] = c * 36 * 256 + (32 * hh + (lane & 24) + ((lane + 2 * c + hh) & 7)) * 4;
+        }
+    auto loadu3 = [&](int slot, int k, unsigned u) {
+#pragma unroll
+        for (int nt = 0; nt < NT; ++nt)
+#pragma unroll
+            for (int p = 0; p < 3; ++p)
+                fu3[slot][nt][p] = __builtin_bit_cast(u32x4, __builtin_amdgcn_raw_buffer_load_b128(
+                    urs, lane16, u + (unsigned)((k / 9) * 36 + k % 9) * (unsigned)WF_U3_STEP + (unsigned)(nt * 3 + p) * 1024u, 0));
+    };
+    auto loadu3_one = [&](int slot, int k, int m, unsigned u) {
+        fu3[slot][m / 3][m % 3] = __builtin_bit_cast(u32x4, __builtin_amdgcn_raw_buffer_load_b128(
+            urs, lane16, u + (unsigned)((k / 9) * 36 + k % 9) * (unsigned)WF_U3_STEP + (unsigned)m * 1024u, 0));
+    };
+    auto readv = [&](int k) {
+#pragma unroll
+        for (int hh = 0; hh < 2; ++hh) vraw[hh] = *reinterpret_cast<const f32x4*>(smem + (9 * wave + k % 9) * 256 + voff[k / 9][hh]);
+    };
+    auto split_unit = [&](int slot, int u) __attribute__((always_inline)) {
+        const int e2 = u / 2, v = e2 / 2, e = 2 * (e2 % 2);
+        float lo = vraw[v][e], hi = vraw[v][e + 1];
+        const unsigned w = cvt_pk_bf16(lo, hi);
+        pv[slot][u % 2][e2] = w;
+        lo -= __builtin_bit_cast(float, w << 16);
+        hi -= __builtin_bit_cast(float, w & 0xffff0000u);
+        if (u % 2) pv[slot][2][e2] = cvt_pk_bf16(lo, hi);
+        else { vraw[v][e] = lo; vraw[v][e + 1] = hi; }
     };
     __syncthreads();
     constexpr unsigned OOB = 0x40000000u;
@@ -367,7 +413,9 @@
             bt6t(d[i], v);
 #pragma unroll
             for (int j = 0; j < 6; ++j) *reinterpret_cast<f32x4*>(vout + (i * 6 + j) * 256) = v[j];
-            if (i >= 2) {
+            if constexpr (SPLIT) {
+                if (i >= 6 - NS) loadu3(i - (6 - NS), i - (6 - NS), up);
+            } else if (i >= 2) {
 #pragma unroll
                 for (int q = 0; q < 2; ++q)
 #pragma unroll
@@ -378,6 +426,35 @@
         if (FFR_TRACE_ON(a.trace)) se[0] += __builtin_amdgcn_s_memtime() - tp0;
         __syncthreads();
         if (FFR_TRACE_ON(a.trace)) se[1] += __builtin_amdgcn_s_memtime() - tp0;
+        if constexpr (SPLIT) {
+        readv(0);
+#pragma unroll
+        for (int u = 0; u < 8; ++u) split_unit(0, u);
+        FFR_PIN;
+#pragma unroll
+        for (int k = 0; k < 18; ++k) {
+            const int j = k % 9, cur = k & 1, slot = k % NS;
+#pragma unroll
+            for (int g = 0; g < 6 * NT; ++g) {
+                const int q = g / NT, nt = g % NT;
+                if (j < 8) acc[j][nt] = __builtin_amdgcn_mfma_f32_32x32x16_bf16(__builtin_bit_cast(bf16x8, fu3[slot][nt][PU[q]]),
+                                                                              __builtin_bit_cast(bf16x8, pv[cur][PV[q]]), acc[j][nt], 0, 0, 0);
+                else asm volatile("s_nop 1\n\tv_mfma_f32_32x32x16_bf16 %0, %1, %2, %0" : "+v"(accv[nt]) : "v"(fu3[slot][nt][PU[q]]), "v"(pv[cur][PV[q]]));
+                if (g == 0) {
+                    if (k == 9) offsets();
+                    if (k < 17) readv(k + 1);
+                }
+                if (g >= 1 && g <= 3 * NT && k >= 1 && k - 1 + NS < 18) loadu3_one((k - 1) % NS, k - 1 + NS, g - 1, up);
+                if (k >= 10 && (g == 3 * NT + 1 || g == 3 * NT + 2)) {
+                    const int idx = 2 * (k - 10) + (g - 3 * NT - 1);
+                    pre[idx] = load_px(idx, soff_next);
+                }
+                if (k < 17 && g >= 4 && g < 12) split_unit(cur ^ 1, g - 4);
+                FFR_PIN;
+            }
+        }
+        up += 2u * 36u * (unsigned)WF_U3_STEP;
+        } else {
         reada(0, 0, 0);
 #pragma unroll
         for (int c = 0; c < 4; ++c) {
@@ -408,6 +485,7 @@
                 }
             }
             up += 36 * 2048u;
+        }
         }
         __syncthreads();
     }
@@ -554,8 +632,8 @@
 }
 
 hipError_t wino_fused_init() {
-    const void* fns[4] = {(const void*)k_wino_fused<0, 2>, (const void*)k_wino_fused<1, 2>,
-                          (const void*)k_wino_fused<0, 1>, (const void*)k_wino_fused<1, 1>};
+    const void* fns[5] = {(const void*)k_wino_fused<0, 2>, (const void*)k_wino_fused<1, 2>, (const void*)k_wino_fused<0, 1>,
+                          (const void*)k_wino_fused<1, 1>, (const void*)k_wino_fused<1, 2, true>};
     for (const void* f : fns) {
         hipError_t e = hipFuncSetAttribute(f, hipFuncAttributeMaxDynamicSharedMemorySize, WF_LDS_BYTES);
         if (e != hipSuccess) return e;
@@ -584,11 +662,14 @@
     a.nbn = a.cout_pad / (a.half_n ? 32 : 64);
     const dim3 grid(wf_grid(a.mbn, a.nbn, a.map_v));
     if (a.Vc) {
+        if (a.U3) return hipErrorInvalidValue;
         if (a.half_n) hipLaunchKernelGGL((k_wino_fused<0, 1>), grid, dim3(256), WF_LDS_BYTES, stream, a);
         else hipLaunchKernelGGL((k_wino_fused<0, 2>), grid, dim3(256), WF_LDS_BYTES, stream, a);
     } else {
         if (!a.x || a.nkc % 4 || a.x_bytes == 0 || a.x_bytes > 0x40000000u) return hipErrorInvalidValue;
+        if (a.U3 && a.half_n) return hipErrorInvalidValue;
         if (a.half_n) hipLaunchKernelGGL((k_wino_fused<1, 1>), grid, dim3(256), WF_LDS_BYTES, stream, a);
+        else if (a.U3) hipLaunchKernelGGL((k_wino_fused<1, 2, true>), grid, dim3(256), WF_LDS_BYTES, stream, a);
         else hipLaunchKernelGGL((k_wino_fused<1, 2>), grid, dim3(256), WF_LDS_BYTES, stream, a);
     }
     return hipGetLastError();
diff --git a/ffr-net_amd/native.py b/ffr-net_amd/native.py
--- a/ffr-net_amd/native.py
+++ b/ffr-net_amd/native.py
@@ -25,7 +25,8 @@
 class MemStats(C.Structure):
     _fields_ = [('encoder_weight_bytes', C.c_size_t), ('recnet_weight_bytes', C.c_size_t), ('mixed_tile_weight_bytes', C.c_size_t),
                 ('workspace_bytes', C.c_size_t), ('encoder_load_seconds', C.c_double), ('recnet_load_seconds', C.c_double),
-                ('mixed_tile_pack_seconds', C.c_double), ('split_weight_bytes', C.c_size_t)]
+                ('mixed_tile_pack_seconds', C.c_double), ('split_weight_bytes', C.c_size_t),
+                ('wf_split_weight_bytes', C.c_size_t), ('wf_split_launches', C.c_longlong)]
 
 
 class KClassStat(C.Structure):
@@ -104,6 +105,7 @@
     ('ffr_layer_set_arith', C.c_int, [_P, C.c_int, C.c_int]),
     ('ffr_calibrate', C.c_int, [_P, _P, _P, C.c_int, C.c_int, C.c_int, C.c_double, C.POINTER(C.c_double), _P]),
     ('ffr_memory_stats', C.c_int, [_P, _P]),
+    ('ffr_split_planes_host', C.c_int, [_P, C.c_longlong, _P]),
     ('ffr_set_option', C.c_int, [_P, C.c_char_p, C.c_longlong]),
     ('ffr_get_option', C.c_int, [_P, C.c_char_p, C.POINTER(C.c_longlong)]),
     ('ffr_probe_mfma_peak', C.c_int, [_P, C.c_int, C.POINTER(C.c_double), C.POINTER(C.c_double), _P]),
diff --git a/include/ffrnet.h b/include/ffrnet.h
--- a/include/ffrnet.h
+++ b/include/ffrnet.h
@@ -124,8 +124,11 @@
     size_t encoder_weight_bytes, recnet_weight_bytes, mixed_tile_weight_bytes, workspace_bytes;
     double encoder_load_seconds, recnet_load_seconds, mixed_tile_pack_seconds;
     size_t split_weight_bytes;
+    size_t wf_split_weight_bytes;
+    long long wf_split_launches;
 } ffr_mem_stats;
 int ffr_memory_stats(const ffr_handle* h, ffr_mem_stats* out);
+int ffr_split_planes_host(const double* w, long long n, unsigned short* planes);
 int ffr_probe_mfma_peak(ffr_handle* h, int iters, double* tflops, double* clock_ghz, void* stream);
 int ffr_profile_read(ffr_handle* h, ffr_kclass_stat* out );
 
```

New measurement: 17030 embeddings/s (median of 6 runs). 1.03x the previous value.
